# IST-DASLab/gptq-gguf-toolkit

Measured on AMD Instinct MI355X. Metric: Mparams/s GPTQ-quantized, higher is better.
Workload: dtype f32; 1 GPU; llama3-8b-block-q4k: 7 Linears of one block (218.1 M params), 128x2048-token calibration fed per sequence through the package's BlockSchedule, block_size 128, rel_damp 0.01, nstep 20; calib_seqs_per_rank=128, parallelism=calib-dp1+matrix-fanout, owners=rank0

## Files before the change

### gptq-gguf-toolkit_amd/_cabi.py

```python
import ctypes
import os
import subprocess

_HERE = os.path.dirname(os.path.abspath(__file__))
CSRC = os.path.join(_HERE, "csrc")
SO_PATH = os.environ.get("GQ_SO_PATH") or os.path.join(CSRC, "libgptqgguf_hip.so")

ABI_VERSION = 6
F32, F16, BF16 = 0, 1, 2
WS_H_ACCUMULATE, WS_H_PREPARE, WS_GPTQ_QUANTIZE, WS_CHOL_GEMM = 1, 2, 3, 4

EXPORTS = (
    "gq_abi_version", "gq_last_error", "gq_option_count", "gq_option_name", "gq_option_get", "gq_option_default", "gq_option_set", "gq_type_info", "gq_workspace_bytes", "gq_h_accumulate", "gq_h_accumulate_grouped", "gq_h_accumulate_segments", "gq_h_stage", "gq_h_stage_many", "gq_h_prepare", "gq_w_prepare", "gq_h_pack_upper", "gq_h_unpack_upper",
    "gq_scale_search", "gq_group_search", "gq_gptq_quantize", "gq_gptq_quantize_stacked", "gq_gptq_quantize_slice", "gq_gptq_quantize_perm", "gq_gptq_uses_helper_stream", "gq_far_helper_enable", "gq_obq_h_prepare", "gq_obq_quantize", "gq_rtn_quantize", "gq_dequantize", "gq_pack", "gq_unpack", "gq_dequantize_blocks", "gq_trailing_update", "gq_chol_gemm", "gq_stage_to_host", "gq_fwd_rmsnorm", "gq_fwd_rmsnorm_ordered", "gq_fwd_rope", "gq_fwd_silu_mul",
    "gq_eval_nll", "gq_eval_kl", "gq_eval_kl_sparse",
    "gq_prof_enable", "gq_prof_ntags", "gq_prof_name", "gq_prof_collect", "gq_prof_collect2",
)
EXPORTS_ERREST = ("gq_quad_form_workspace_bytes", "gq_quad_form")
EXPORTS_SEARCH = ("gq_level_switch",)
SWITCH_MAX_JOBS = 64
EXPORTS_LEVELS = ("gq_gptq_quantize_bands",)
BANDS_MAX = 64
EXPORTS_LEVELPACK = ("gq_pack_bands",)
PACK_BANDS_ALIGN = 16
EXPORTS_Q8 = ("gq_quantize_q8_0",)
Q8_0 = 8
IQ4_NL, IQ4_XS = 20, 23
EXPORTS_IQ4_ENCODE = ("gq_quantize_iq4",)
EXPORTS_IQ4_GPTQ = ("gq_gptq_quantize_iq4", "gq_pack_iq4")
EXPORTS_QGEMM = ("gq_linear_packed",)
EXPORTS_QGEMV = ("gq_gemv_packed",)
GEMV_MAX_T = 16
EXPORTS_SAMPLE = ("gq_sample_logits",)
SAMPLE_MAX_K = 1024
EXPORTS_MOE = ("gq_gemv_packed_experts",)
MOE_MAX_PAIRS = 64
EXPORTS_MOE_GEMM = ("gq_moe_route", "gq_linear_packed_experts")
MOE_ROUTE_MAX_EXPERTS = 256
MOE_ROUTE_MAX_PAIRS = 131072
EXPORTS_MOE_CALIB = ("gq_fwd_moe_combine",)
MOE_COMBINE_MAX_K = 8
EXPORTS_MOE_SEARCH = ("gq_level_switch_experts",)
SWITCH_EXPERTS_MAX_JOBS = 71


class GQError(RuntimeError):
    pass


class TypeInfo(ctypes.Structure):
    _fields_ = [(n, ctypes.c_int) for n in
                ("bits", "qmin", "qmax", "scale_maxq", "group", "is_signed", "k_search", "type_size")]


class Search(ctypes.Structure):
    _fields_ = [("rmin", ctypes.c_double), ("rdelta", ctypes.c_double), ("nstep", ctypes.c_int),
                ("quant_scale", ctypes.c_int), ("grid", ctypes.c_int), ("maxshrink", ctypes.c_double)]


class SwitchJob(ctypes.Structure):
    _fields_ = [("src", ctypes.c_void_p), ("dst", ctypes.c_void_p), ("row_src", ctypes.c_void_p),
                ("R", ctypes.c_int64), ("C", ctypes.c_int64), ("kind", ctypes.c_int32), ("out_dtype", ctypes.c_int32)]


class SwitchExpertsJob(ctypes.Structure):
    _fields_ = [("src", ctypes.c_void_p), ("dst", ctypes.c_void_p), ("E", ctypes.c_int64), ("R", ctypes.c_int64),
                ("C", ctypes.c_int64), ("dst_expert_stride", ctypes.c_int64), ("kind", ctypes.c_int32),
                ("out_dtype", ctypes.c_int32)]


class Band(ctypes.Structure):
    _fields_ = [("row_end", ctypes.c_int64), ("q_type", ctypes.c_int32)]


def build(force: bool = False) -> str:
    args = ["make", "-C", CSRC, "-s", "-j8"]
    if force:
        args.append("-B")
    subprocess.check_call(args)
    return SO_PATH


_lib = None


def lib():
    global _lib
    if _lib is not None:
        return _lib
    if not os.path.exists(SO_PATH):
        raise GQError(
            f"{SO_PATH} not found: the HIP extension is not built. Run `python -c 'import __graft_entry__ as g; "
            f"g.build()'` (or `make -C {CSRC}`). There is no CPU fallback.")
    import torch
    L = ctypes.CDLL(SO_PATH)
    vp, i64, ci, cf, sz = ctypes.c_void_p, ctypes.c_int64, ctypes.c_int, ctypes.c_float, ctypes.c_size_t
    sp = ctypes.POINTER(Search)
    L.gq_abi_version.restype = ci
    if L.gq_abi_version() != ABI_VERSION:
        raise GQError(f"{SO_PATH} has ABI version {L.gq_abi_version()}, this package binds version {ABI_VERSION}: rebuild "
                      f"(`make -C {CSRC}`)")
    L.gq_last_error.restype = ctypes.c_char_p
    L.gq_option_name.restype = ctypes.c_char_p
    L.gq_option_name.argtypes = [ci]
    L.gq_option_get.argtypes = [ctypes.c_char_p, ctypes.POINTER(i64)]
    L.gq_option_default.argtypes = [ctypes.c_char_p, ctypes.POINTER(i64)]
    L.gq_option_set.argtypes = [ctypes.c_char_p, i64, ctypes.POINTER(i64)]
    L.gq_type_info.argtypes = [ci, ctypes.POINTER(TypeInfo)]
    L.gq_workspace_bytes.argtypes = [ci, i64, i64, i64, ci]
    L.gq_workspace_bytes.restype = sz
    L.gq_h_accumulate.argtypes = [vp, vp, ci, i64, i64, cf, cf, vp, sz, vp]
    L.gq_h_accumulate_grouped.argtypes = [ci, vp, vp, vp, vp, vp, vp, ci, vp, sz, vp]
    L.gq_h_accumulate_segments.argtypes = [ci, vp, vp, vp, vp, vp, vp, vp, ci, vp, sz, vp]
    L.gq_h_stage.argtypes = [vp, vp, i64, vp]
    L.gq_h_stage_many.argtypes = [vp, vp, vp, ci, vp, sz, vp]
    L.gq_h_prepare.argtypes = [vp, vp, i64, i64, cf, vp, vp, vp, vp, sz, vp]
    L.gq_w_prepare.argtypes = [vp, vp, i64, i64, vp, vp]
    L.gq_h_pack_upper.argtypes = [vp, i64, vp, vp]
    L.gq_h_unpack_upper.argtypes = [vp, i64, vp, vp]
    L.gq_scale_search.argtypes = [vp, i64, i64, ci, sp, vp, i64, vp, i64, vp, i64, vp, i64, vp]
    L.gq_group_search.argtypes = [vp, ci, i64, i64, ci, sp, vp, vp, vp, vp, vp, vp, vp]
    L.gq_gptq_quantize.argtypes = [vp, vp, i64, i64, ci, ci, ci, sp, vp, vp, vp, vp, vp, vp, sz, vp]
    L.gq_gptq_quantize_stacked.argtypes = [vp, vp, i64, i64, ci, ci, ci, sp, vp, vp, vp, vp, vp, vp, ci, vp, sz, vp]
    L.gq_gptq_quantize_slice.argtypes = [vp, vp, i64, i64, ci, ci, ci, sp, vp, vp, vp, vp, vp, vp, vp, sz, vp]
    L.gq_gptq_quantize_perm.argtypes = [vp, vp, i64, i64, ci, ci, vp, vp, vp, vp, vp, vp, vp, sz, vp]
    L.gq_gptq_uses_helper_stream.argtypes = [i64, i64, ci]
    L.gq_far_helper_enable.argtypes = [ci]
    L.gq_obq_h_prepare.argtypes = L.gq_h_prepare.argtypes
    L.gq_obq_quantize.argtypes = [vp, vp, i64, i64, ci, ci, ci, ci, vp, vp, vp, vp, sz, vp]
    L.gq_rtn_quantize.argtypes = [vp, ci, i64, i64, ci, sp, vp, vp, vp, vp, vp, vp]
    L.gq_dequantize.argtypes = [ci, vp, vp, vp, vp, vp, i64, i64, vp, ci, vp]
    L.gq_pack.argtypes = [ci, vp, vp, vp, vp, vp, i64, i64, vp, vp]
    L.gq_unpack.argtypes = [ci, vp, i64, i64, vp, vp, vp, vp, vp, vp]
    L.gq_dequantize_blocks.argtypes = [ci, vp, i64, i64, vp, vp, ci, vp]
    L.gq_trailing_update.argtypes = [vp, i64, vp, i64, vp, i64, i64, i64, i64, vp]
    L.gq_chol_gemm.argtypes = [vp, i64, vp, i64, vp, i64, i64, i64, i64, ci, ci, ci, ci, ci, vp, sz, vp]
    L.gq_stage_to_host.argtypes = [vp, vp, i64, vp]
    L.gq_fwd_rmsnorm.argtypes = [vp, vp, vp, i64, i64, cf, ci, vp]
    L.gq_fwd_rmsnorm_ordered.argtypes = [vp, vp, vp, i64, i64, cf, ci, vp, vp]
    L.gq_fwd_rope.argtypes = [vp, vp, vp, vp, i64, ci, ci, ci, vp]
    L.gq_fwd_silu_mul.argtypes = [vp, vp, vp, i64, ci, vp]
    L.gq_eval_nll.argtypes = [vp, ci, i64, i64, i64, vp, i64, vp, vp, vp]
    L.gq_eval_kl.argtypes = [vp, ci, vp, ci, i64, i64, i64, i64, vp, vp]
    L.gq_eval_kl_sparse.argtypes = [vp, ci, i64, i64, i64, vp, ci, vp, i64, vp, vp]
    L.gq_quad_form_workspace_bytes.argtypes = [i64, i64]
    L.gq_quad_form_workspace_bytes.restype = sz
    L.gq_quad_form.argtypes = [vp, ci, i64, vp, ci, i64, vp, i64, i64, vp, vp, sz, vp]
    L.gq_level_switch.argtypes = [ctypes.POINTER(SwitchJob), ci, vp]
    L.gq_gptq_quantize_bands.argtypes = [vp, vp, i64, i64, ctypes.POINTER(Band), ci, ci, sp, vp, vp, vp, vp, vp, vp, sz, vp]
    L.gq_pack_bands.argtypes = [vp, vp, vp, vp, vp, i64, i64, ctypes.POINTER(Band), ci, ctypes.POINTER(vp), ctypes.POINTER(vp), vp]
    L.gq_quantize_q8_0.argtypes = [vp, ci, i64, i64, vp, vp, vp]
    L.gq_quantize_iq4.argtypes = [vp, ci, i64, i64, ci, vp, vp, vp, vp]
    L.gq_gptq_quantize_iq4.argtypes = [vp, vp, i64, i64, ci, ci, vp, vp, vp, vp, vp, vp, vp, sz, vp]
    L.gq_pack_iq4.argtypes = [ci, i64, i64, vp, vp, vp, vp, vp, vp]
    L.gq_linear_packed.argtypes = [ci, vp, vp, i64, i64, vp, i64, ci, vp, vp]
    L.gq_gemv_packed.argtypes = [ci, vp, vp, i64, i64, vp, i64, ci, vp, vp]
    L.gq_sample_logits.argtypes = [vp, ci, i64, i64, i64, ci, cf, cf, vp, vp, vp]
    L.gq_gemv_packed_experts.argtypes = [ci, vp, i64, i64, i64, vp, i64, vp, i64, i64, ci, vp, vp]
    L.gq_moe_route.argtypes = [vp, i64, i64, vp, vp, vp]
    L.gq_linear_packed_experts.argtypes = [ci, vp, i64, i64, i64, vp, i64, i64, vp, vp, i64, ci, vp, vp]
    L.gq_fwd_moe_combine.argtypes = [vp, vp, vp, vp, vp, ci, i64, i64, i64, i64, ci, vp, vp]
    L.gq_level_switch_experts.argtypes = [ctypes.POINTER(SwitchExpertsJob), ci, vp]
    L.gq_prof_enable.argtypes = [ctypes.c_uint]
    L.gq_prof_enable.restype = None
    L.gq_prof_name.argtypes = [ci]
    L.gq_prof_name.restype = ctypes.c_char_p
    L.gq_prof_collect.argtypes = [ctypes.POINTER(ctypes.c_double), ctypes.POINTER(ctypes.c_long)]
    L.gq_prof_collect2.argtypes = [ctypes.POINTER(ctypes.c_double), ctypes.POINTER(ctypes.c_long),
                                   ctypes.POINTER(ctypes.c_double)]
    for name in (EXPORTS + EXPORTS_ERREST + EXPORTS_SEARCH + EXPORTS_LEVELS + EXPORTS_LEVELPACK + EXPORTS_Q8 + EXPORTS_IQ4_ENCODE + EXPORTS_IQ4_GPTQ + EXPORTS_QGEMM +
                 EXPORTS_QGEMV + EXPORTS_SAMPLE + EXPORTS_MOE + EXPORTS_MOE_GEMM + EXPORTS_MOE_CALIB + EXPORTS_MOE_SEARCH):
        getattr(L, name)
    _lib = L
    return L


def check(rc: int, what: str):
    if rc != 0:
        msg = lib().gq_last_error().decode(errors="replace")
        raise GQError(f"{what} failed (status {rc}): {msg}")


def type_info(q_type: int) -> dict:
    t = TypeInfo()
    check(lib().gq_type_info(int(q_type), ctypes.byref(t)), "gq_type_info")
    return {n: getattr(t, n) for n, _ in TypeInfo._fields_}


def prof_enable(tags=None):
    L = lib()
    names = [L.gq_prof_name(i).decode() for i in range(L.gq_prof_ntags())]
    mask = 0
    for i, n in enumerate(names):
        if tags is None or n in tags:
            mask |= 1 << i
    L.gq_prof_enable(mask)
    return names


def prof_collect(busy: bool = False) -> dict:
    L = lib()
    n = L.gq_prof_ntags()
    ms = (ctypes.c_double * n)()
    cnt = (ctypes.c_long * n)()
    bz = (ctypes.c_double * n)()
    check(L.gq_prof_collect2(ms, cnt, bz), "gq_prof_collect2")
    if busy:
        return {L.gq_prof_name(i).decode(): (ms[i], cnt[i], bz[i]) for i in range(n) if cnt[i]}
    return {L.gq_prof_name(i).decode(): (ms[i], cnt[i]) for i in range(n) if cnt[i]}


def option_names():
    L = lib()
    return [L.gq_option_name(i).decode() for i in range(L.gq_option_count())]


def option_get(name: str) -> int:
    v = ctypes.c_int64()
    check(lib().gq_option_get(name.encode(), ctypes.byref(v)), "gq_option_get")
    return int(v.value)


def option_default(name: str) -> int:
    v = ctypes.c_int64()
    check(lib().gq_option_default(name.encode(), ctypes.byref(v)), "gq_option_default")
    return int(v.value)


def option_set(name: str, value: int) -> int:
    prev = ctypes.c_int64()
    check(lib().gq_option_set(name.encode(), int(value), ctypes.byref(prev)), "gq_option_set")
    return int(prev.value)


class options:

    def __init__(self, **kv):
        self.kv, self.prev = kv, {}

    def __enter__(self):
        for k, v in self.kv.items():
            self.prev[k] = option_set(k, option_default(k) if v is None else v)
        return self

    def __exit__(self, *exc):
        for k, v in self.prev.items():
            option_set(k, v)
        return False
```

### gptq-gguf-toolkit_amd/block_schedule.py

```python
import contextlib
import os
import sys
import time
from typing import Any, Callable, Dict, List, Optional, Tuple

import torch
import torch.nn as nn

from . import dist_utils
from . import ops as _ops
from .gptq import GPTQ
from .model_utils import ForwardInterrupt
from .quant_utils import GGML_QUANT_SIZES
from .quant_utils import GGMLQuantizationType, dequantize_linear_weight

_stream_pool: Dict[Any, List["torch.cuda.Stream"]] = {}


def _chain_streams(device, n: int):
    if n <= 0 or torch.device(device).type != "cuda":
        return []
    pool = _stream_pool.setdefault(torch.device(device), [])
    while len(pool) < n:
        pool.append(torch.cuda.Stream(device))
    return pool[:n]


class _Lane:

    def __init__(self, stream, main):
        self.stream, self.main = stream, main

    def wait(self, event):
        if self.stream is not None and event is not None:
            self.stream.wait_event(event)

    def run(self):
        return torch.cuda.stream(self.stream) if self.stream is not None else contextlib.nullcontext()

    def join(self, tensors=()):
        if self.stream is None:
            return
        ev = torch.cuda.Event()
        ev.record(self.stream)
        self.main.wait_event(ev)
        for t in tensors:
            if t is not None and t.is_cuda:
                t.record_stream(self.main)


def _zero_columns(w: torch.Tensor) -> torch.Tensor:
    return (w.detach().reshape(w.shape[0], -1) == 0).all(dim=0)


def _owner_cost(h: GPTQ) -> float:
    return float(h.d_row) * h.d_col * (h.d_col + 128)


def _chain_order_key(hs: List[GPTQ]):
    return (not any(h._row_split_active() for h in hs), -sum(float(h.d_row) * h.d_col ** 2 for h in hs))


def _lane_load(hs: List[GPTQ]) -> float:
    return sum(float(h.d_row) * h.d_col ** 2 + float(h.d_col) ** 3 / 3 for h in hs)


def _plan_lanes(cost: List[float], lanes: int) -> Tuple[List[int], List[int]]:
    n = len(cost)
    lane_of, load = [0] * n, [0.0] * max(lanes, 1)
    for k in range(n):
        lane_of[k] = min(range(lanes), key=lambda i: (load[i], i)) if lanes else 0
        load[lane_of[k]] += cost[k]
    enq = list(range(n))
    if lanes >= 4 and n > 2 * lanes:
        per = [[k for k in range(n) if lane_of[k] == i] for i in range(lanes)]
        for i in range(lanes // 2, lanes):
            per[i].reverse()
        enq = [per[i][j] for j in range(max(len(x) for x in per)) for i in range(lanes) if j < len(per[i])]
    return lane_of, enq


@contextlib.contextmanager
def _far_helper_lease(on: bool):
    was = _ops.far_helper_enable(on)
    try:
        yield
    finally:
        _ops.far_helper_enable(was)


class _Call:

    def __init__(self, qtypes, writeback, extra, own: Dict[str, bool], world: int, rank: int):
        self.qtypes, self.writeback, self.extra, self.own, self.world, self.rank = qtypes, writeback, extra, own, world, rank
        self.results: Dict[str, tuple] = {}
        self.deq: Dict[str, torch.Tensor] = {}


class BlockSchedule:
    unverified: List[torch.Tensor] = []

    def __init__(self, layers: Dict[str, nn.Module], make_handle: Callable[[nn.Module, str], GPTQ],
                 n_streams: Optional[int] = None, verbose: bool = False):
        self.handles: Dict[str, GPTQ] = {n: make_handle(l, n) for n, l in layers.items()}
        self._zero_cols = {n: _zero_columns(l.weight) for n, l in layers.items()}
        self._sharing = None
        for h in self.handles.values():
            h._scheduled = True
        self._seen: Dict[Any, Any] = {}
        self._fired: List[str] = []
        self._last_fired: Optional[str] = None
        self._other_after = False
        self._n_samples = 0
        self.n_streams = int(os.environ.get("GQ_CHAIN_STREAMS", 4)) if n_streams is None else n_streams
        self.stack = os.environ.get("GQ_STACK", "1") != "0"
        self.verbose = verbose
        self.stats = {"syrk_launches": 0, "allreduce_bytes": 0, "reused_U": 0, "own_U": 0, "refactorised": 0}
        self.owners: Dict[str, Any] = {}

    def hook(self, name: str):
        def _hook(_, inp, out):
            self.feed(name, inp[0])
        return _hook

    def pre_hook(self, name: str, interrupt: bool = True):
        def _hook(_, inp):
            self.feed(name, inp[0])
            self._fired.append(name)
            self._other_after = False
            if interrupt and name == self._last_fired and self._all_fired_once():
                self.stats["forward1_interrupts"] = self.stats.get("forward1_interrupts", 0) + 1
                raise ForwardInterrupt
        return _hook

    def _all_fired_once(self) -> bool:
        return len(self._fired) == len(self.handles) and len(set(self._fired)) == len(self._fired)

    def other_pre_hook(self):
        def _hook(_, inp):
            if self._n_samples == 0:
                self._other_after = True
        return _hook

    def feed(self, name: str, x: torch.Tensor) -> None:
        h = self.handles[name]
        key = (x.data_ptr(), tuple(x.shape), tuple(x.stride()), x.dtype, x._version)
        hit = self._seen.get(key)
        if hit is not None and hit[0].d_col == h.d_col and hit[0] is not h:
            leader = hit[0]
            assert h.shared_H_with in (None, leader), "input sharing pattern changed between samples"
            assert h.H is None, "handle switched from own Hessian to a shared one"
            h.shared_H_with = leader
            leader._has_followers = True
        else:
            assert h.shared_H_with is None, "input sharing pattern changed between samples"
            self._seen[key] = (h, x)
        h.update(x)

    def sample_done(self) -> None:
        self._seen.clear()
        if self._n_samples == 0 and self._all_fired_once() and not self._other_after:
            self._last_fired = self._fired[-1]
        self._n_samples += 1
        self._fired = []
        if self._sharing is None:
            self._publish_sharing()
        due = [h for h in self.leaders() if h._fill >= h.flush_tokens]
        if due:
            self.flush(only=due)

    def _publish_sharing(self) -> None:
        name_of = {id(h): n for n, h in self.handles.items()}
        followers = [n for n, h in self.handles.items() if h.shared_H_with is not None]
        host = ev = None
        if followers:
            neq = torch.stack([(self._zero_cols[n] != self._zero_cols[name_of[id(self.handles[n].shared_H_with)]]).any()
                               for n in followers])
            if neq.is_cuda:
                host = torch.empty(len(followers), dtype=torch.bool, pin_memory=True)
                host.copy_(neq, non_blocking=True)
                ev = torch.cuda.Event()
                ev.record(torch.cuda.current_stream(neq.device))
            else:
                host = neq
        self._sharing = (followers, host, ev)

    def _needs_own_factorisation(self) -> Dict[str, bool]:
        if self._sharing is None or not self._sharing[0]:
            return {}
        followers, host, ev = self._sharing
        if ev is not None:
            ev.synchronize()
        return dict(zip(followers, host.tolist()))

    _staged_checks: List[Any] = []

    @classmethod
    def stage_verify(cls) -> None:
        flags, cls.unverified = cls.unverified, []
        if not flags:
            return
        anyf = torch.stack([f.reshape(()) for f in flags]).any().reshape(1)
        if anyf.is_cuda:
            host = torch.empty(1, dtype=torch.bool, pin_memory=True)
            host.copy_(anyf, non_blocking=True)
            ev = torch.cuda.Event()
            ev.record(torch.cuda.current_stream(anyf.device))
            cls._staged_checks.append((host, ev))
        else:
            cls._staged_checks.append((anyf, None))

    @classmethod
    def verify(cls, wait: bool = True) -> None:
        cls.stage_verify()
        keep = []
        for host, ev in cls._staged_checks:
            if ev is not None and not wait and not ev.query():
                keep.append((host, ev))
                continue
            if ev is not None:
                ev.synchronize()
            if bool(host.item()):
                cls._staged_checks = []
                raise RuntimeError("a Linear reused its leader's Cholesky factor although their dead / zero-column sets "
                                   "differ (gq_w_prepare flag)")
        cls._staged_checks = keep

    @classmethod
    def discard_checks(cls) -> None:
        cls.unverified = []
        cls._staged_checks = []

    def leaders(self) -> List[GPTQ]:
        return [h for h in self.handles.values() if h.shared_H_with is None]

    def _fold(self, grids: List[List[GPTQ]]) -> None:
        for grp in grids:
            args = [h._flush_args() for h in grp]
            _ops.h_accumulate_grouped([a[0] for a in args], [a[1] for a in args], [a[2] for a in args],
                                      [a[3] for a in args])
            self.stats["syrk_launches"] += 1
            for h in grp:
                h._flush_done()

    def flush(self, only: Optional[List[GPTQ]] = None) -> None:
        todo = [h for h in self.leaders() if h._fill > 0 and (only is None or any(h is o for o in only))]
        if not todo:
            return
        todo.sort(key=lambda h: (-h.d_col, id(h)))
        grids: List[List[GPTQ]] = []
        if 1 < len(todo) <= 8 and len({(h._pending_dtype(), h._pending_device()) for h in todo}) == 1:
            rest, grids_tail = todo, []
        elif len(todo) > 1 and todo[0].d_col > todo[1].d_col:
            rest, grids_tail = todo[1:], [[todo[0]]]
        else:
            rest, grids_tail = todo, []
        by_kind: Dict[Any, List[GPTQ]] = {}
        for h in rest:
            by_kind.setdefault((h._pending_dtype(), h._pending_device()), []).append(h)
        for grp in by_kind.values():
            grids += [grp[i:i + 8] for i in range(0, len(grp), 8)]
        grids += grids_tail
        self._fold(grids)

    def _agree_on_sharing(self) -> None:
        names = list(self.handles)
        idx = {id(self.handles[n]): i for i, n in enumerate(names)}
        dev = next(iter(self.handles.values())).W_device
        v = torch.full((len(names),), -1, dtype=torch.int64, device=dev)
        for i, n in enumerate(names):
            h = self.handles[n]
            if h.shared_H_with is not None:
                v[i] = idx[id(h.shared_H_with)]
            elif h.H is not None or h._fill > 0:
                v[i] = i
        mine = v.clone()
        dist_utils.collective_calls["small_all_reduce"] += 1
        dist_utils.collective_bytes["small_all_reduce"] += v.numel() * 8
        torch.distributed.all_reduce(v, op=torch.distributed.ReduceOp.MAX)
        got, mine = v.tolist(), mine.tolist()
        for i, n in enumerate(names):
            h = self.handles[n]
            assert mine[i] in (-1, got[i]), f"{n}: ranks observed different input sharing ({mine[i]} vs {got[i]})"
            if mine[i] == -1 and got[i] not in (-1, i):
                leader = self.handles[names[got[i]]]
                h.shared_H_with = leader
                leader._has_followers = True

    @torch.no_grad()
    def quantize(self, qtypes: Dict[str, GGMLQuantizationType], writeback: bool = True,
                 extra: Optional[Callable[[str, GPTQ, tuple], Any]] = None) -> Dict[str, Tuple[torch.Tensor, ...]]:
        handles = self.handles
        world, rank = dist_utils.get_world_size(), dist_utils.get_rank()
        for n, h in handles.items():
            if qtypes[n] == GGMLQuantizationType.Q3_K:
                h.act_order = False
        if world > 1:
            self._assign_ranks(world)
        dev = next(iter(handles.values())).W_device
        on_gpu = torch.device(dev).type == "cuda"
        main = torch.cuda.current_stream(dev) if on_gpu else None
        ready, start = self._reduce_hessians(world, main)

        order = self._chains(rank)
        call = _Call(qtypes, writeback, extra, self._needs_own_factorisation(), world, rank)
        on_main = 1
        lent = 1 if on_gpu and 2 < self.n_streams and len(order) <= self.n_streams and any(
            _ops.uses_helper_stream(h.d_row, h.d_col, h.block_size) for h in handles.values()
            if h.owner_rank == rank and not h._row_split_active()) else 0
        streams = [None] * on_main + _chain_streams(dev, min(self.n_streams - lent, len(order)) - on_main)
        trace = "sched" in os.environ.get("GQ_TRACE", "")
        t_host = time.perf_counter()
        lane_of, enq = _plan_lanes([_lane_load([handles[n] for n in names]) for names in order], len(streams))
        with _far_helper_lease(bool(lent)) if on_gpu else contextlib.nullcontext():
            lanes = []
            for k in enq:
                if trace:
                    print(f"  [sched] +{1e3 * (time.perf_counter() - t_host):7.2f} ms: enqueue chain {k} {order[k]} on lane {lane_of[k]}",
                          file=sys.stderr)
                lane = _Lane(streams[lane_of[k]], main)
                lead = handles[order[k][0]].shared_H_with or handles[order[k][0]]
                lane.wait(ready.get(id(lead), start))
                lanes.append((lane, self._run_chain(call, order[k], lane)))
            for lane, born in lanes:
                lane.join(born)
        if trace:
            print(f"  [sched] +{1e3 * (time.perf_counter() - t_host):7.2f} ms: all chains enqueued", file=sys.stderr)
        self._settle_late_followers(call)
        self.stats["own_U"] = len(call.results) - self.stats["reused_U"]
        return self._exchange_and_write_back(call)

    @torch.no_grad()
    def quantize_levels(self, levels, propagate: Optional[GGMLQuantizationType],
                        extra: Optional[Callable[[str, GPTQ, dict], Any]] = None,
                        pack: Optional[Callable[[tuple, list, list], Any]] = None,
                        before: Optional[Callable[[str, GPTQ], Any]] = None) -> Dict[str, Dict[Any, Tuple[torch.Tensor, ...]]]:
        handles = self.handles
        levels = [GGMLQuantizationType(t) for t in levels]
        if not levels or len(set(levels)) != len(levels):
            raise ValueError("quantize_levels needs a non-empty list of distinct levels")
        if propagate is not None:
            propagate = GGMLQuantizationType(propagate)
            if propagate not in levels:
                raise ValueError(f"propagate={propagate.name} is not one of the levels {[t.name for t in levels]}")
        if dist_utils.get_world_size() > 1:
            raise NotImplementedError("quantize_levels runs on one rank (multi-rank level builds are not built)")
        for n, h in handles.items():
            if h.act_order or h.static_groups:
                raise ValueError(f"{n}: act_order / static_groups handles have no level build")
        dev = next(iter(handles.values())).W_device
        on_gpu = torch.device(dev).type == "cuda"
        main = torch.cuda.current_stream(dev) if on_gpu else None
        ready, start = self._reduce_hessians(1, main)
        order = self._chains(0)
        own = self._needs_own_factorisation()
        lent = 1 if on_gpu and 2 < self.n_streams and len(order) <= self.n_streams and any(
            _ops.uses_helper_stream(len(levels) * h.d_row, h.d_col, h.block_size) for h in handles.values()) else 0
        streams = [None] + _chain_streams(dev, min(self.n_streams - lent, len(order)) - 1)
        lane_of, enq = _plan_lanes([_lane_load([handles[n] for n in names]) for names in order], len(streams))
        results: Dict[str, Dict[Any, tuple]] = {}
        deq: Dict[str, torch.Tensor] = {}
        with _far_helper_lease(bool(lent)) if on_gpu else contextlib.nullcontext():
            lanes = []
            for k in enq:
                lane = _Lane(streams[lane_of[k]], main)
                lane.wait(start)
                lanes.append((lane, self._run_level_chain(order[k], levels, propagate, own, extra, results, deq, lane, pack,
                                                          before)))
            for lane, born in lanes:
                lane.join(born)
        self.stats["own_U"] = len(results) - self.stats["reused_U"]
        for n, h in handles.items():
            if propagate is not None:
                h.layer.weight.data = deq[n]
            h.reset()
        return {n: results[n] for n in handles}

    def _run_level_chain(self, names: List[str], levels, propagate, own: Dict[str, bool], extra, results, deq,
                         lane: _Lane, pack=None, before=None) -> List[torch.Tensor]:
        handles = self.handles
        born: List[torch.Tensor] = []
        names = sorted(names, key=lambda n: handles[n].shared_H_with is not None)
        together = [n for n in names if handles[n].shared_H_with is None or (n in own and not own[n])]
        alone = [n for n in names if n not in together]
        walks = [] if pack is not None else None
        name_of = {handles[n]: n for n in names}
        with lane.run():
            for n in names if before is not None else ():
                out = before(n, handles[n])
                born.extend(t for t in (out if isinstance(out, (tuple, list)) else (out,)) if torch.is_tensor(t))
            for grp in ([together] if self.stack else [[n] for n in together]):
                if not grp:
                    continue
                if self.verbose:
                    print(f"[rank 0] Quantizing {grp} with {[t.name for t in levels]}.")
                hs = [handles[n] for n in grp]
                if len(grp) > 1:
                    self.stats["stacked"] = self.stats.get("stacked", 0) + len(grp)
                res = GPTQ.compute_levels(hs, levels, defer_check=True, walks=walks)
                for n, h in zip(grp, hs):
                    if h._pending_mismatch is not None:
                        BlockSchedule.unverified.append(h._pending_mismatch)
                        h._pending_mismatch = None
                        self.stats["reused_U"] += 1
                    results[n] = res[h]
            for n in alone:
                h = handles[n]
                self.stats["refactorised"] += 1
                results[n] = GPTQ.compute_levels([h], levels, own_U=True, walks=walks)[h]
            for n in names:
                h = handles[n]
                for res in results[n].values():
                    born.extend(res)
                born.extend(t for t in (h._last_U, h._last_cf) if torch.is_tensor(t))
                if propagate is not None:
                    deq[n] = dequantize_linear_weight(propagate, *results[n][propagate], out_dtype=h.layer.weight.data.dtype)
                    born.append(deq[n])
                if extra is not None:
                    out = extra(n, h, results[n])
                    born.extend(t for t in (out if isinstance(out, (tuple, list)) else (out,)) if torch.is_tensor(t))
            for stacked, bands, members in walks or ():
                out = pack(stacked, bands, [None if mem is None else (name_of[mem[0]], mem[1]) for mem in members])
                born.extend(t for t in (out if isinstance(out, (tuple, list)) else (out,)) if torch.is_tensor(t))
        return born

    def _assign_ranks(self, world: int) -> None:
        handles = self.handles
        costs = {n: _owner_cost(h) for n, h in handles.items()}
        split = {n for n in dist_utils.row_split_names(costs, world) if not handles[n].act_order}
        for n in split:
            handles[n].row_split = True
        for n, r in dist_utils.assign_owners({n: c for n, c in costs.items() if n not in split}, world).items():
            handles[n].owner_rank = r
        if any(h.allow_no_samples for h in handles.values()):
            self._agree_on_sharing()
        self.owners = {n: (f"rows/{world}" if h._row_split_active() else h.owner_rank) for n, h in handles.items()}
        need: Dict[int, set] = {}
        for n, h in handles.items():
            lead = h.shared_H_with or h
            need.setdefault(id(lead), set()).update(range(world) if h._row_split_active() else (h.owner_rank,))
        for h in self.leaders():
            ranks = need.get(id(h), set())
            h.reduce_to = next(iter(ranks)) if len(ranks) == 1 else None

    def _reduce_hessians(self, world: int, main):
        ready: Dict[int, Any] = {}
        self.flush()
        for h in sorted(self.leaders(), key=lambda h: -h.d_col):
            h.sync_hessian()
            if world > 1:
                self.stats["allreduce_bytes"] += dist_utils.hessian_payload_bytes(h.d_col)
                if main is not None:
                    ready[id(h)] = torch.cuda.Event()
                    ready[id(h)].record(main)
        for h in self.handles.values():
            h.sync_hessian()
        start = None
        if main is not None and world == 1:
            start = torch.cuda.Event()
            start.record(main)
        return ready, start

    def _chains(self, rank: int) -> List[List[str]]:
        chains: Dict[int, List[str]] = {}
        for n, h in self.handles.items():
            if h.owner_rank == rank or h._row_split_active():
                chains.setdefault(id(h.shared_H_with or h), []).append(n)
        return sorted(chains.values(), key=lambda ns: _chain_order_key([self.handles[n] for n in ns]))

    def _run_chain(self, call: _Call, names: List[str], lane: _Lane) -> List[torch.Tensor]:
        handles, qtypes = self.handles, call.qtypes
        born: List[torch.Tensor] = []
        with lane.run():
            for grp in self._stack_groups(sorted(names, key=lambda n: handles[n].shared_H_with is not None), qtypes, call.own):
                if self.verbose:
                    for n in grp:
                        print(f"[rank {call.rank}] Quantizing {n} with {qtypes[n].name}.")
                if len(grp) > 1:
                    hs = [handles[n] for n in grp]
                    self.stats["stacked"] = self.stats.get("stacked", 0) + len(grp)
                    for n, h, res in zip(grp, hs, GPTQ.compute_stacked(hs, qtypes[grp[0]])):
                        self._computed(call, born, n, h, res)
                    continue
                n = grp[0]
                h = handles[n]
                h.make_working_copy()
                self._computed(call, born, n, h, h.compute(qtypes[n], defer_check=True, own_U=call.own.get(n, False)))
        return born

    def _computed(self, call: _Call, born: List[torch.Tensor], n: str, h: GPTQ, res: tuple) -> None:
        if n in call.own and h._pending_mismatch is not None:
            BlockSchedule.unverified.append(h._pending_mismatch)
            h._pending_mismatch = None
            self.stats["reused_U"] += 1
        elif call.own.get(n, False):
            self.stats["refactorised"] += 1
        call.results[n] = res
        born.extend(res)
        born.extend(t for t in (h._last_U, h._last_cf, getattr(h, "_researches", None), h.W) if torch.is_tensor(t))
        if call.world == 1 and call.writeback:
            call.deq[n] = dequantize_linear_weight(call.qtypes[n], *res, out_dtype=h.layer.weight.data.dtype)
            born.append(call.deq[n])
        if call.extra is not None:
            out = call.extra(n, h, res)
            born.extend(t for t in (out if isinstance(out, (tuple, list)) else (out,)) if torch.is_tensor(t))

    def _settle_late_followers(self, call: _Call) -> None:
        handles = self.handles
        pending = [(n, handles[n]._pending_mismatch) for n in call.results if handles[n]._pending_mismatch is not None]
        if pending:
            flags = torch.cat([f.reshape(1) for _, f in pending]).tolist()
            for (n, _), bad in zip(pending, flags):
                h = handles[n]
                h._pending_mismatch = None
                if bad:
                    self.stats["refactorised"] += 1
                    h.make_working_copy()
                    call.results[n] = h.compute(call.qtypes[n], own_U=True)
                    call.deq.pop(n, None)
                else:
                    self.stats["reused_U"] += 1

    def _exchange_and_write_back(self, call: _Call) -> Dict[str, Tuple[torch.Tensor, ...]]:
        handles, qtypes = self.handles, call.qtypes
        if call.world > 1:
            out = self._exchange_block(handles, qtypes, call.results, call.world, call.rank)
        else:
            out = {n: call.results[n] for n in handles}
        for n, h in handles.items():
            if call.writeback:
                w = call.deq.get(n)
                if w is None:
                    w = dequantize_linear_weight(qtypes[n], *out[n], out_dtype=h.layer.weight.data.dtype)
                h.layer.weight.data = w
            h.reset()
        return out

    def _stack_groups(self, names: List[str], qtypes, own: Dict[str, bool]) -> List[List[str]]:
        if not self.stack:
            return [[n] for n in names]
        groups: List[List[str]] = []
        open_: Dict[Any, List[str]] = {}
        for n in names:
            h = self.handles[n]
            key = h.stack_key(qtypes[n])
            known = (h.shared_H_with is None and h._has_followers) or (n in own and not own[n])
            if key is None or not known:
                groups.append([n])
                continue
            g = open_.get(key)
            if g is None or len(g) >= 8:
                g = open_[key] = []
                groups.append(g)
            g.append(n)
        return groups

    @staticmethod
    def _piece_layout(q_type, rows: int, cols: int):
        bits, clamp, scale_maxq, group_size, supergroup_size, sz_dtype, q_dtype = GGML_QUANT_SIZES[q_type]
        shapes = ((q_dtype, (rows, cols)), (torch.float16, (rows, cols // supergroup_size)),
                  (sz_dtype, (rows, cols // group_size)), (torch.float16, (rows, cols // supergroup_size)),
                  (sz_dtype, (rows, cols // group_size)))
        lay, off = [], 0
        for dt, shp in shapes:
            n = shp[0] * shp[1] * torch.empty(0, dtype=dt).element_size()
            lay.append((dt, shp, off, n))
            off += (n + 255) & ~255
        return lay, off

    def _exchange_block(self, handles, qtypes, results, world: int, rank: int):
        per_rank: List[List[Tuple[str, int, int]]] = [[] for _ in range(world)]
        for n, h in handles.items():
            if h._row_split_active():
                for r in range(world):
                    r0, r1, _ = dist_utils.row_slice(h.d_row, r, world)
                    if r1 > r0:
                        per_rank[r].append((n, r0, r1))
            else:
                per_rank[h.owner_rank].append((n, 0, h.d_row))
        layouts = [[(n, r0, r1) + self._piece_layout(qtypes[n], r1 - r0, handles[n].d_col) for n, r0, r1 in lst]
                   for lst in per_rank]
        sizes = [sum(x[4] for x in lst) for lst in layouts]
        split = [n for n, h in handles.items() if h._row_split_active()]
        tail = (4 * len(split) + 255) & ~255 if split else 0
        body = max(max(sizes), 256)
        nbytes = body + tail
        dev = next(iter(handles.values())).W_device
        buf = torch.empty(nbytes, dtype=torch.uint8, device=dev)
        off = 0
        for n, r0, r1, lay, tot in layouts[rank]:
            for t, (dt, shp, o, k) in zip(results[n], lay):
                buf[off + o:off + o + k].view(dt).view(shp).copy_(t)
            off += tot
        if split:
            buf[body:body + 4 * len(split)].view(torch.int32).copy_(torch.cat([handles[n]._researches for n in split]))
        gathered = dist_utils.all_gather_bytes(buf, nbytes)
        self.stats["allgather_bytes"] = self.stats.get("allgather_bytes", 0) + nbytes
        redo = []
        if split:
            counts = gathered[:, body:body + 4 * len(split)].view(torch.int32).reshape(world, len(split)).sum(dim=0).tolist()
            redo = [n for n, c in zip(split, counts) if c != 0]
        parts: Dict[str, List[List[torch.Tensor]]] = {n: [] for n in handles}
        for r in range(world):
            off = 0
            for n, r0, r1, lay, tot in layouts[r]:
                parts[n].append([gathered[r, off + o:off + o + k].view(dt).view(shp) for dt, shp, o, k in lay])
                off += tot
        out: Dict[str, tuple] = {}
        for n in handles:
            ps = parts[n]
            if n in redo:
                self.stats["row_split_redone"] = self.stats.get("row_split_redone", 0) + 1
                handles[n].row_split_redone = True
                out[n] = handles[n].recompute_whole(qtypes[n])
                continue
            out[n] = tuple(ps[0]) if len(ps) == 1 else tuple(torch.cat([p[i] for p in ps], dim=0) for i in range(5))
        return out
```

### gptq-gguf-toolkit_amd/csrc/gq_cholesky.hip

```cpp
#include <atomic>
#include <stdlib.h>

#include "gq_common.hpp"
#include "gq_gemm32.hpp"
#include "gq_gemm3b.hpp"
#include "gq_gemm3p.hpp"

#include <map>
#include <memory>
#include <mutex>

namespace gq {

constexpr int NB = 128;

__global__ __launch_bounds__(256) void col_flags_kernel(const float* __restrict__ H, const float* __restrict__ W,
                                                        int64_t R, int64_t C, uint8_t* __restrict__ dead,
                                                        uint8_t* __restrict__ zc) {
    const int64_t j = (int64_t)blockIdx.x * 64 + (threadIdx.x & 63);
    const int ty = threadIdx.x >> 6;
    __shared__ int nz[4][64];
    int any = 0;
    if (j < C)
        for (int64_t r = ty; r < R; r += 4) any |= (W[r * C + j] != 0.0f);
    nz[ty][threadIdx.x & 63] = any;
    __syncthreads();
    if (ty == 0 && j < C) {
        int a = nz[0][threadIdx.x] | nz[1][threadIdx.x] | nz[2][threadIdx.x] | nz[3][threadIdx.x];
        uint8_t dd = H[j * C + j] == 0.0f;
        dead[j] = dd;
        zc[j] = dd || !a;
    }
}

__global__ __launch_bounds__(256) void zero_dead_cols_kernel(float* __restrict__ W, int64_t R, int64_t C,
                                                             const uint8_t* __restrict__ dead) {
    const int64_t j = (int64_t)blockIdx.x * 64 + (threadIdx.x & 63);
    const bool dd = j < C && dead[j];
    if (!__syncthreads_or(dd)) return;
    if (dd)
        for (int64_t r = threadIdx.x >> 6; r < R; r += 4) W[r * C + j] = 0.0f;
}

__global__ __launch_bounds__(256) void w_prepare_kernel(float* __restrict__ W, int64_t R, int64_t C,
                                                        const uint8_t* __restrict__ dead,
                                                        const uint8_t* __restrict__ zc, int* __restrict__ mismatch) {
    const int64_t j = (int64_t)blockIdx.x * 64 + (threadIdx.x & 63);
    const int ty = threadIdx.x >> 6;
    __shared__ int nz[4][64];
    int any = 0;
    if (j < C) {
        const bool dd = dead[j];
        for (int64_t r = ty; r < R; r += 4) {
            if (dd) W[r * C + j] = 0.0f;
            else any |= (W[r * C + j] != 0.0f);
        }
    }
    nz[ty][threadIdx.x & 63] = any;
    __syncthreads();
    if (ty == 0 && j < C) {
        int a = nz[0][threadIdx.x] | nz[1][threadIdx.x] | nz[2][threadIdx.x] | nz[3][threadIdx.x];
        uint8_t mine = dead[j] || !a;
        if (mine != zc[j]) atomicOr(mismatch, 1);
    }
}

__global__ __launch_bounds__(256) void col_flags4_kernel(const float* __restrict__ H, const float* __restrict__ W,
                                                         int64_t R, int64_t C, uint8_t* __restrict__ dead,
                                                         uint8_t* __restrict__ zc) {
    const int tx = threadIdx.x & 15, ty = threadIdx.x >> 4;
    const int64_t j = (int64_t)blockIdx.x * 64 + 4 * tx;
    __shared__ int nz[16][64];
    int a0 = 0, a1 = 0, a2 = 0, a3 = 0;
    if (j < C) {
#pragma unroll 8
        for (int64_t r = ty; r < R; r += 16) {
            const float4 v = *reinterpret_cast<const float4*>(W + r * C + j);
            a0 |= (v.x != 0.0f); a1 |= (v.y != 0.0f); a2 |= (v.z != 0.0f); a3 |= (v.w != 0.0f);
        }
    }
    nz[ty][4 * tx] = a0; nz[ty][4 * tx + 1] = a1; nz[ty][4 * tx + 2] = a2; nz[ty][4 * tx + 3] = a3;
    __syncthreads();
    const int64_t jc = (int64_t)blockIdx.x * 64 + threadIdx.x;
    if (threadIdx.x < 64 && jc < C) {
        int a = 0;
#pragma unroll
        for (int t = 0; t < 16; ++t) a |= nz[t][threadIdx.x];
        const uint8_t dd = H[jc * C + jc] == 0.0f;
        dead[jc] = dd;
        zc[jc] = dd || !a;
    }
}
__global__ __launch_bounds__(256) void w_prepare4_kernel(float* __restrict__ W, int64_t R, int64_t C,
                                                         const uint8_t* __restrict__ dead,
                                                         const uint8_t* __restrict__ zc, int* __restrict__ mismatch) {
    const int tx = threadIdx.x & 15, ty = threadIdx.x >> 4;
    const int64_t j = (int64_t)blockIdx.x * 64 + 4 * tx;
    __shared__ int nz[16][64];
    int a0 = 0, a1 = 0, a2 = 0, a3 = 0;
    if (j < C) {
        const bool d0 = dead[j], d1 = dead[j + 1], d2 = dead[j + 2], d3 = dead[j + 3];
        const bool anyd = d0 | d1 | d2 | d3;
#pragma unroll 8
        for (int64_t r = ty; r < R; r += 16) {
            float4 v = *reinterpret_cast<const float4*>(W + r * C + j);
            if (anyd) {
                if (d0) v.x = 0.0f;
                if (d1) v.y = 0.0f;
                if (d2) v.z = 0.0f;
                if (d3) v.w = 0.0f;
                *reinterpret_cast<float4*>(W + r * C + j) = v;
            }
            a0 |= (v.x != 0.0f); a1 |= (v.y != 0.0f); a2 |= (v.z != 0.0f); a3 |= (v.w != 0.0f);
        }
    }
    nz[ty][4 * tx] = a0; nz[ty][4 * tx + 1] = a1; nz[ty][4 * tx + 2] = a2; nz[ty][4 * tx + 3] = a3;
    __syncthreads();
    const int64_t jc = (int64_t)blockIdx.x * 64 + threadIdx.x;
    if (threadIdx.x < 64 && jc < C) {
        int a = 0;
#pragma unroll
        for (int t = 0; t < 16; ++t) a |= nz[t][threadIdx.x];
        const uint8_t mine = dead[jc] || !a;
        if (mine != zc[jc]) atomicOr(mismatch, 1);
    }
}

__global__ __launch_bounds__(256) void mask_h_kernel(float* __restrict__ H, int64_t C, const uint8_t* __restrict__ zc) {
    __shared__ int flagged[64];
    const int64_t i0 = (int64_t)blockIdx.x * 64;
    if (threadIdx.x < 64) flagged[threadIdx.x] = (i0 + threadIdx.x < C) && zc[i0 + threadIdx.x];
    __syncthreads();
    for (int t = 0; t < 64; ++t) {
        if (!flagged[t]) continue;
        const int64_t i = i0 + t;
        for (int64_t j = threadIdx.x; j < C; j += blockDim.x) {
            const float v = (i == j) ? 1.0f : 0.0f;
            H[i * C + j] = v;
            H[j * C + i] = v;
        }
    }
}

__global__ __launch_bounds__(256) void dead_diag_kernel(float* __restrict__ H, int64_t C, const uint8_t* __restrict__ dead) {
    const int64_t j = (int64_t)blockIdx.x * blockDim.x + threadIdx.x;
    if (j < C && dead[j]) H[j * C + j] = 1.0f;
}

__global__ __launch_bounds__(1024) void damp_kernel(float* __restrict__ H, int64_t C, float rel_damp) {
    __shared__ double part[1024];
    double acc = 0.0;
    for (int64_t i = threadIdx.x; i < C; i += 1024) acc += (double)H[i * C + i];
    part[threadIdx.x] = acc;
    __syncthreads();
    for (int o = 512; o > 0; o >>= 1) {
        if ((int)threadIdx.x < o) part[threadIdx.x] += part[threadIdx.x + o];
        __syncthreads();
    }
    const float damp = rel_damp * (float)(part[0] / (double)C);
    for (int64_t i = threadIdx.x; i < C; i += 1024) H[i * C + i] += damp;
}

__global__ __launch_bounds__(256) void equil_kernel(const float* __restrict__ H, int64_t n, float* __restrict__ s) {
    const int64_t j = (int64_t)blockIdx.x * blockDim.x + threadIdx.x;
    if (j >= n) return;
    const float h = H[j * n + j];
    float v = 1.0f;
    if (h > 0.0f && h < 3.0e38f) {
        int e;
        (void)frexpf(h, &e);
        const int half = (e >= 0 ? e : e - 1) / 2;
        v = ldexpf(1.0f, -half);
    }
    s[j] = v;
}
__global__ __launch_bounds__(256) void reverse_copy_kernel(float* __restrict__ A, const float* __restrict__ H,
                                                           int64_t n, const float* __restrict__ s) {
    const int64_t i = blockIdx.x, r = n - 1 - i;
    const int64_t jend = (i / 128 + 1) * 128;
    const float si = s ? s[r] : 1.0f;
    for (int64_t j = 4 * (int64_t)threadIdx.x; j < jend; j += 4 * 256) {
        const float4 h = *reinterpret_cast<const float4*>(H + r * n + (n - 4 - j));
        float4 a = make_float4(h.w, h.z, h.y, h.x);
        if (s) {
            const float4 sc = *reinterpret_cast<const float4*>(s + (n - 4 - j));
            a.x *= si * sc.w; a.y *= si * sc.z; a.z *= si * sc.y; a.w *= si * sc.x;
        }
        *reinterpret_cast<float4*>(A + i * n + j) = a;
    }
}

__global__ __launch_bounds__(256) void finish_u_kernel(float* __restrict__ U, const float* __restrict__ X, int64_t n,
                                                       const int* __restrict__ flag, const float* __restrict__ s) {
    const int64_t i = blockIdx.x, r = n - 1 - i;
    const bool bad = *flag != 0;
    for (int64_t j = 4 * (int64_t)threadIdx.x; j < n; j += 4 * 256) {
        float4 u = make_float4(0.f, 0.f, 0.f, 0.f);
        if (bad) {
            u.x = (j == i) ? 1.0f : 0.0f; u.y = (j + 1 == i) ? 1.0f : 0.0f;
            u.z = (j + 2 == i) ? 1.0f : 0.0f; u.w = (j + 3 == i) ? 1.0f : 0.0f;
        } else if (j + 3 >= i) {
            const float4 x = *reinterpret_cast<const float4*>(X + r * n + (n - 4 - j));
            float4 sc = make_float4(1.f, 1.f, 1.f, 1.f);
            if (s) sc = *reinterpret_cast<const float4*>(s + j);
            u.x = (j >= i) ? x.w * sc.x : 0.0f;
            u.y = (j + 1 >= i) ? x.z * sc.y : 0.0f;
            u.z = (j + 2 >= i) ? x.y * sc.z : 0.0f;
            u.w = x.x * sc.w;
        }
        *reinterpret_cast<float4*>(U + i * n + j) = u;
    }
}

constexpr int LDP = NB + 4;

__global__ __launch_bounds__(256) void diag_potrf_inv_kernel(float* __restrict__ A, int64_t lda,
                                                             float* __restrict__ Xout, int64_t ldx,
                                                             int* __restrict__ flag) {
    extern __shared__ __attribute__((aligned(16))) float smem[];
    float* S = smem;
    float* XT = smem + NB * LDP;
    float* dg = XT + NB * LDP;
    const int tid = threadIdx.x;
    for (int idx = tid; idx < NB * NB; idx += 256) {
        int i = idx / NB, j = idx % NB;
        float v = (j <= i) ? A[i * lda + j] : 0.0f;
        S[i * LDP + j] = v;
        XT[i * LDP + j] = 0.0f;
        if (i == j) dg[i] = v;
    }
    __syncthreads();
    const bool fac = tid < NB;
    const int i = tid & (NB - 1);
    for (int j = 0; j <= NB; ++j) {
        if (fac) {
            if (j < NB && i >= j) {
                const float4* ri = reinterpret_cast<const float4*>(S + i * LDP);
                const float4* rj = reinterpret_cast<const float4*>(S + j * LDP);
                float a0 = 0.f, a1 = 0.f, a2 = 0.f, a3 = 0.f, q0 = 0.f, q1 = 0.f, q2 = 0.f, q3 = 0.f;
                const int n4 = j >> 2;
                int p4 = 0;
                for (; p4 + 4 <= n4; p4 += 4) {
                    float4 a[4], b[4];
#pragma unroll
                    for (int u = 0; u < 4; ++u) { a[u] = ri[p4 + u]; b[u] = rj[p4 + u]; }
#pragma unroll
                    for (int u = 0; u < 4; ++u) {
                        a0 = fmaf(a[u].x, b[u].x, a0); a1 = fmaf(a[u].y, b[u].y, a1);
                        a2 = fmaf(a[u].z, b[u].z, a2); a3 = fmaf(a[u].w, b[u].w, a3);
                        q0 = fmaf(b[u].x, b[u].x, q0); q1 = fmaf(b[u].y, b[u].y, q1);
                        q2 = fmaf(b[u].z, b[u].z, q2); q3 = fmaf(b[u].w, b[u].w, q3);
                    }
                }
                for (; p4 < n4; ++p4) {
                    const float4 a = ri[p4], b = rj[p4];
                    a0 = fmaf(a.x, b.x, a0); a1 = fmaf(a.y, b.y, a1); a2 = fmaf(a.z, b.z, a2); a3 = fmaf(a.w, b.w, a3);
                    q0 = fmaf(b.x, b.x, q0); q1 = fmaf(b.y, b.y, q1); q2 = fmaf(b.z, b.z, q2); q3 = fmaf(b.w, b.w, q3);
                }
                float acc = (a0 + a1) + (a2 + a3), accp = (q0 + q1) + (q2 + q3);
                for (int p = p4 * 4; p < j; ++p) {
                    const float a = S[i * LDP + p], b = S[j * LDP + p];
                    acc = fmaf(a, b, acc);
                    accp = fmaf(b, b, accp);
                }
                float piv = dg[j] - accp;
                const bool bad = !(piv > 0.0f);
                if (bad) piv = 1.0f;
                const float ljj = sqrtf(piv);
                if (i == j) {
                    S[j * LDP + j] = ljj;
                    if (bad) *flag = 1;
                } else {
                    S[i * LDP + j] = (S[i * LDP + j] - acc) / ljj;
                }
            }
        } else if (j >= 1) {
            const int r = j - 1, c = i;
            if (c == r) {
                XT[c * LDP + r] = 1.0f / S[r * LDP + r];
            } else if (c < r) {
                const float4* lr = reinterpret_cast<const float4*>(S + r * LDP);
                const float4* xc = reinterpret_cast<const float4*>(XT + c * LDP);
                float a0 = 0.f, a1 = 0.f, a2 = 0.f, a3 = 0.f;
                int p4 = c >> 2;
                const int e4 = r >> 2;
                for (; p4 + 3 <= e4; p4 += 4) {
                    float4 a[4], b[4];
#pragma unroll
                    for (int u = 0; u < 4; ++u) { a[u] = lr[p4 + u]; b[u] = xc[p4 + u]; }
#pragma unroll
                    for (int u = 0; u < 4; ++u) {
                        a0 = fmaf(a[u].x, b[u].x, a0); a1 = fmaf(a[u].y, b[u].y, a1);
                        a2 = fmaf(a[u].z, b[u].z, a2); a3 = fmaf(a[u].w, b[u].w, a3);
                    }
                }
                for (; p4 <= e4; ++p4) {
                    const float4 a = lr[p4], b = xc[p4];
                    a0 = fmaf(a.x, b.x, a0); a1 = fmaf(a.y, b.y, a1); a2 = fmaf(a.z, b.z, a2); a3 = fmaf(a.w, b.w, a3);
                }
                const float acc = (a0 + a1) + (a2 + a3);
                XT[c * LDP + r] = -acc / S[r * LDP + r];
            }
        }
        __syncthreads();
    }
    for (int idx = tid; idx < NB * NB; idx += 256) {
        int r = idx / NB, c = idx % NB;
        if (c <= r) A[r * lda + c] = S[r * LDP + c];
        Xout[r * ldx + c] = XT[c * LDP + r];
    }
}

constexpr int LDQ = NB + 1;
constexpr int TQ = 33;

__device__ __forceinline__ float rdlane(float v, int l) {
    return __builtin_bit_cast(float, __builtin_amdgcn_readlane(__builtin_bit_cast(int, v), l));
}

template <int C>
__device__ __forceinline__ void d_upd4(float (&a)[32], float aj) {
    int t0, t1, t2, t3;
    asm volatile(
        "v_readlane_b32 %4, %8, %9\n\tv_readlane_b32 %5, %8, %10\n\tv_readlane_b32 %6, %8, %11\n\t"
        "v_readlane_b32 %7, %8, %12\n\t"
        "v_fma_f32 %0, -%8, %4, %0\n\tv_fma_f32 %1, -%8, %5, %1\n\tv_fma_f32 %2, -%8, %6, %2\n\tv_fma_f32 %3, -%8, %7, %3"
        : "+v"(a[C]), "+v"(a[C + 1]), "+v"(a[C + 2]), "+v"(a[C + 3]), "=&s"(t0), "=&s"(t1), "=&s"(t2), "=&s"(t3)
        : "v"(aj), "n"(C), "n"(C + 1), "n"(C + 2), "n"(C + 3));
}
template <int C>
__device__ __forceinline__ void d_upd8(float (&a)[32], float aj) {
    int t0, t1, t2, t3, t4, t5, t6, t7;
    asm volatile(
        "v_readlane_b32 %8, %16, %17\n\tv_readlane_b32 %9, %16, %18\n\tv_readlane_b32 %10, %16, %19\n\t"
        "v_readlane_b32 %11, %16, %20\n\tv_readlane_b32 %12, %16, %21\n\tv_readlane_b32 %13, %16, %22\n\t"
        "v_readlane_b32 %14, %16, %23\n\tv_readlane_b32 %15, %16, %24\n\t"
        "v_fma_f32 %0, -%16, %8, %0\n\tv_fma_f32 %1, -%16, %9, %1\n\tv_fma_f32 %2, -%16, %10, %2\n\t"
        "v_fma_f32 %3, -%16, %11, %3\n\tv_fma_f32 %4, -%16, %12, %4\n\tv_fma_f32 %5, -%16, %13, %5\n\t"
        "v_fma_f32 %6, -%16, %14, %6\n\tv_fma_f32 %7, -%16, %15, %7"
        : "+v"(a[C]), "+v"(a[C + 1]), "+v"(a[C + 2]), "+v"(a[C + 3]), "+v"(a[C + 4]), "+v"(a[C + 5]), "+v"(a[C + 6]),
          "+v"(a[C + 7]), "=&s"(t0), "=&s"(t1), "=&s"(t2), "=&s"(t3), "=&s"(t4), "=&s"(t5), "=&s"(t6), "=&s"(t7)
        : "v"(aj), "n"(C), "n"(C + 1), "n"(C + 2), "n"(C + 3), "n"(C + 4), "n"(C + 5), "n"(C + 6), "n"(C + 7));
}
template <int C>
__device__ __forceinline__ void d_upd1(float (&a)[32], float aj) {
    int t0;
    asm volatile("v_readlane_b32 %1, %2, %3\n\ts_nop 1\n\tv_fma_f32 %0, -%2, %1, %0" : "+v"(a[C]), "=&s"(t0) : "v"(aj), "n"(C));
}
template <int C>
__device__ __forceinline__ void d_updates(float (&a)[32], float aj) {
    if constexpr (C + 7 <= 31) {
        d_upd8<C>(a, aj);
        d_updates<C + 8>(a, aj);
    } else if constexpr (C + 3 <= 31) {
        d_upd4<C>(a, aj);
        d_updates<C + 4>(a, aj);
    } else if constexpr (C <= 31) {
        d_upd1<C>(a, aj);
        d_updates<C + 1>(a, aj);
    }
}
template <int J>
__device__ __forceinline__ void d_factor(float (&a)[32], int i, float& myinv, bool& bad) {
    asm volatile("s_nop 1" : "+v"(a[J]));
    float pj = rdlane(a[J], J);
    if (!(pj > 0.0f)) {
        bad = true;
        pj = 1.0f;
    }
    float inv = __builtin_amdgcn_rsqf(pj);
    inv = fmaf(inv, fmaf(-0.5f * pj * inv, inv, 0.5f), inv);
    const float ljj = pj * inv;
    int ii = i;
    asm volatile("" : "+v"(ii));
    const bool mine = ii == J;
    if (mine) myinv = inv;
    a[J] = mine ? ljj : a[J] * inv;
    asm volatile("s_nop 1" : "+v"(a[J]));
    d_updates<J + 1>(a, a[J]);
    if constexpr (J < 31) d_factor<J + 1>(a, i, myinv, bad);
}
template <int R, int P>
__device__ __forceinline__ void d_dot4(const float (&a)[32], const float (&x)[32], float (&acc)[4]) {
    int t0, t1, t2, t3;
    asm volatile(
        "v_readlane_b32 %4, %8, %16\n\tv_readlane_b32 %5, %9, %16\n\tv_readlane_b32 %6, %10, %16\n\t"
        "v_readlane_b32 %7, %11, %16\n\t"
        "v_fma_f32 %0, %4, %12, %0\n\tv_fma_f32 %1, %5, %13, %1\n\tv_fma_f32 %2, %6, %14, %2\n\tv_fma_f32 %3, %7, %15, %3"
        : "+v"(acc[0]), "+v"(acc[1]), "+v"(acc[2]), "+v"(acc[3]), "=&s"(t0), "=&s"(t1), "=&s"(t2), "=&s"(t3)
        : "v"(a[P]), "v"(a[P + 1]), "v"(a[P + 2]), "v"(a[P + 3]), "v"(x[P]), "v"(x[P + 1]), "v"(x[P + 2]), "v"(x[P + 3]),
          "n"(R));
}
template <int R, int P>
__device__ __forceinline__ void d_dot8(const float (&a)[32], const float (&x)[32], float (&acc)[4]) {
    int t0, t1, t2, t3, t4, t5, t6, t7;
    asm volatile(
        "v_readlane_b32 %4, %12, %28\n\tv_readlane_b32 %5, %13, %28\n\tv_readlane_b32 %6, %14, %28\n\t"
        "v_readlane_b32 %7, %15, %28\n\tv_readlane_b32 %8, %16, %28\n\tv_readlane_b32 %9, %17, %28\n\t"
        "v_readlane_b32 %10, %18, %28\n\tv_readlane_b32 %11, %19, %28\n\t"
        "v_fma_f32 %0, %4, %20, %0\n\tv_fma_f32 %1, %5, %21, %1\n\tv_fma_f32 %2, %6, %22, %2\n\t"
        "v_fma_f32 %3, %7, %23, %3\n\tv_fma_f32 %0, %8, %24, %0\n\tv_fma_f32 %1, %9, %25, %1\n\t"
        "v_fma_f32 %2, %10, %26, %2\n\tv_fma_f32 %3, %11, %27, %3"
        : "+v"(acc[0]), "+v"(acc[1]), "+v"(acc[2]), "+v"(acc[3]), "=&s"(t0), "=&s"(t1), "=&s"(t2), "=&s"(t3), "=&s"(t4),
          "=&s"(t5), "=&s"(t6), "=&s"(t7)
        : "v"(a[P]), "v"(a[P + 1]), "v"(a[P + 2]), "v"(a[P + 3]), "v"(a[P + 4]), "v"(a[P + 5]), "v"(a[P + 6]), "v"(a[P + 7]),
          "v"(x[P]), "v"(x[P + 1]), "v"(x[P + 2]), "v"(x[P + 3]), "v"(x[P + 4]), "v"(x[P + 5]), "v"(x[P + 6]), "v"(x[P + 7]),
          "n"(R));
}
template <int R, int P>
__device__ __forceinline__ void d_dot1(const float (&a)[32], const float (&x)[32], float& acc) {
    int t0;
    asm volatile("v_readlane_b32 %1, %2, %4\n\ts_nop 1\n\tv_fma_f32 %0, %1, %3, %0" : "+v"(acc), "=&s"(t0) : "v"(a[P]), "v"(x[P]), "n"(R));
}
template <int R, int P>
__device__ __forceinline__ void d_dot(const float (&a)[32], const float (&x)[32], float (&acc)[4]) {
    if constexpr (P + 7 < R) {
        d_dot8<R, P>(a, x, acc);
        d_dot<R, P + 8>(a, x, acc);
    } else if constexpr (P + 3 < R) {
        d_dot4<R, P>(a, x, acc);
        d_dot<R, P + 4>(a, x, acc);
    } else if constexpr (P < R) {
        d_dot1<R, P>(a, x, acc[P & 3]);
        d_dot<R, P + 1>(a, x, acc);
    }
}
template <int R>
__device__ __forceinline__ void d_inverse(const float (&a)[32], float (&x)[32], int i, float myinv) {
    const float irr = rdlane(myinv, R);
    float acc[4] = {0.0f, 0.0f, 0.0f, 0.0f};
    d_dot<R, 0>(a, x, acc);
    const float dot = (acc[0] + acc[1]) + (acc[2] + acc[3]);
    int ii = i;
    asm volatile("" : "+v"(ii));
    x[R] = (R < ii) ? 0.0f : ((R == ii) ? irr : -dot * irr);
    if constexpr (R < 31) d_inverse<R + 1>(a, x, i, myinv);
}

__device__ __forceinline__ f32x16 mfma_nt_32(const float* Ap, int lda_, const float* Bp, int ldb_, int lane) {
    f32x16 acc;
#pragma unroll
    for (int e = 0; e < 16; ++e) acc[e] = 0.0f;
    const int li = lane & 31, lk = lane >> 5;
    float av[16], bv[16];
#pragma unroll
    for (int p = 0; p < 16; ++p) {
        av[p] = Ap[li * lda_ + 2 * p + lk];
        bv[p] = Bp[li * ldb_ + 2 * p + lk];
    }
#pragma unroll
    for (int p = 0; p < 16; ++p) acc = __builtin_amdgcn_mfma_f32_32x32x2f32(av[p], bv[p], acc, 0, 0, 0);
    return acc;
}


}
#include "gq_diag5.hpp"
namespace gq {

static int64_t p3_min() { return opt(OPT_chol_3p_min); }
static int p3_planes() { return opt(OPT_chol_planes) == 3 ? 3 : 2; }
static inline bool p3_node(int64_t n1, int64_t n2) {
    return p3_min() > 0 && n1 >= p3_min() && n2 >= p3_min() && n1 % 256 == 0 && n2 % 256 == 0;
}
constexpr int P3_MAX_SLOTS = 1024;
struct P3Gemm {
    size_t table_at, rlist_at;
    int n_reduce;
};
struct P3Plans {
    std::vector<uint32_t> words;
    std::vector<P3Gemm> gemms;
};
static void p3_collect(P3Plans& pl, int64_t lo, int64_t hi) {
    if (hi - lo == 1) return;
    const int64_t mid = (lo + hi) / 2;
    const int64_t n1 = (mid - lo) * NB, n2 = (hi - mid) * NB;
    p3_collect(pl, lo, mid);
    const bool big = p3_node(n1, n2);
    const int gran = p3_planes() == 3 ? 2 : 4;
    auto add = [&](const std::vector<p3::GemmShape>& shs) {
        p3::Plan p = p3::make_plan(shs, gran, P3_MAX_SLOTS);
        P3Gemm g;
        while (pl.words.size() % 4) pl.words.push_back(0u);
        g.table_at = pl.words.size();
        pl.words.insert(pl.words.end(), p.table.begin(), p.table.end());
        g.rlist_at = pl.words.size();
        pl.words.insert(pl.words.end(), p.rlist.begin(), p.rlist.end());
        g.n_reduce = (int)(p.rlist.size() / 2);
        if (p.nslots < 0) fprintf(stderr, "gq: image GEMM plan needs more than %d partial slots\n", P3_MAX_SLOTS), abort();
        pl.gemms.push_back(g);
    };
    if (big) {
        const int t1 = (int)(n1 / 256), t2 = (int)(n2 / 256), k1 = (int)(n1 / 32);
        add({{t2, t1, k1, 1, false}});
        add({{t2, t2, k1, 0, true}, {t2, t1, k1, 2, false}});
    }
    p3_collect(pl, mid, hi);
    if (big) add({{(int)(n2 / 256), (int)(n1 / 256), (int)(n2 / 32), 3, false}});
}
static std::shared_ptr<const P3Plans> p3_plans_for(int64_t nblk) {
    static std::mutex mu;
    static std::map<std::pair<int64_t, int64_t>, std::shared_ptr<const P3Plans>> cache;
    std::lock_guard<std::mutex> lk(mu);
    const std::pair<int64_t, int64_t> key{nblk, p3_min() * 4 + p3_planes()};
    auto it = cache.find(key);
    if (it != cache.end()) return it->second;
    auto pl = std::make_shared<P3Plans>();
    p3_collect(*pl, 0, nblk);
    cache[key] = pl;
    return pl;
}
struct P3Run {
    const P3Plans* plans = nullptr;
    const uint32_t* words_dev = nullptr;
    size_t next = 0;
    unsigned char* img[2] = {nullptr, nullptr};
    float* partial = nullptr;
    unsigned* rmax = nullptr;
    float* inv_scale = nullptr;
};
static size_t p3_image_bytes(int64_t C) { return (size_t)(C / 2) * (size_t)(C / 2) * 2 * (size_t)p3_planes(); }
static bool p3_used(int64_t C) {
    const int64_t nblk = C / NB, mid = nblk / 2;
    return nblk >= 2 && p3_node(mid * NB, (nblk - mid) * NB);
}

size_t h_prepare_workspace_bytes(int64_t R, int64_t C) {
    (void)R;
    const size_t n2 = (size_t)C * (size_t)C * sizeof(float);
    size_t extra = 0;
    if (p3_used(C)) {
        auto pl = p3_plans_for(C / NB);
        extra = 2 * (p3_image_bytes(C) + 256) + (size_t)P3_MAX_SLOTS * p3::TILE * p3::TILE * 4 + pl->words.size() * 4 +
                4 * (size_t)C * 4 + 2048;
    }
    return 2 * n2 + 2 * (size_t)C + 4 * (size_t)C + 1024 + extra;
}

template <int NP>
static p3::Problem p3_problem(P3Run& run, const unsigned char* Aimg, int64_t Ka, const unsigned char* Bimg, int64_t Kb,
                              float* Cm, int64_t ldc, int mode, const float* rs, const float* cs) {
    return p3::Problem{Aimg, Bimg, (uint32_t)(Ka / 32 * NP * p3::BLK), (uint32_t)(Kb / 32 * NP * p3::BLK), Cm, ldc, mode,
                       rs, cs, run.partial};
}
template <int NP>
static int p3_gemm(P3Run& run, const p3::Problem& p0, const p3::Problem* p1, hipStream_t st) {
    const P3Gemm& gm = run.plans->gemms[run.next++];
    p3::Group g;
    g.p[0] = p0;
    g.p[1] = p1 ? *p1 : p0;
    g.table = run.words_dev + gm.table_at;
    return p3::launch_gemm<NP>(g, gm.n_reduce, run.words_dev + gm.rlist_at, st);
}

static int chol_inv_rec(float* A, float* X, float* Tmp, int* flag, int64_t n, int64_t lo, int64_t hi, size_t diag_lds,
                        hipStream_t st, P3Run& run);

template <int NP>
static int chol_node_p3(float* A, float* X, float* Tmp, int* flag, int64_t n, int64_t lo, int64_t mid, int64_t hi,
                        size_t diag_lds, hipStream_t st, P3Run& run) {
    const int64_t n1 = (mid - lo) * NB, n2 = (hi - mid) * NB;
    const int64_t o21 = (mid * NB) * n + lo * NB, o11 = (lo * NB) * n + lo * NB, o22 = (mid * NB) * n + mid * NB;
    unsigned* rm0 = run.rmax, *rm1 = run.rmax ? run.rmax + n / 2 : nullptr;
    float* is0 = run.inv_scale, *is1 = run.inv_scale ? run.inv_scale + n / 2 : nullptr;
    const float* s0 = NP == 2 ? is0 : nullptr;
    const float* s1 = NP == 2 ? is1 : nullptr;
    int rc;
    {
        ProfScope ps(PT_CHOL_GEMM, st);
        if ((rc = p3::launch_split<NP>(false, A + o21, n, n2, n1, 0, 0, run.img[0], rm0, is0, st))) return rc;
        if ((rc = p3::launch_split<NP>(false, X + o11, n, n1, n1, 1, 0, run.img[1], rm1, is1, st))) return rc;
        const p3::Problem g1 = p3_problem<NP>(run, run.img[0], n1, run.img[1], n1, Tmp + o21, n, 1, s0, s1);
        if ((rc = p3_gemm<NP>(run, g1, nullptr, st))) return rc;
        if ((rc = p3::launch_split<NP>(false, Tmp + o21, n, n2, n1, 0, 1, run.img[0], rm0, is0, st))) return rc;
        if ((rc = p3::launch_split<NP>(true, X + o11, n, n1, n1, 2, 1, run.img[1], rm1, is1, st))) return rc;
        const p3::Problem g2 = p3_problem<NP>(run, run.img[0], n1, run.img[0], n1, A + o22, n, 0, s0, s0);
        const p3::Problem g3 = p3_problem<NP>(run, run.img[0], n1, run.img[1], n1, A + o21, n, 1, s0, s1);
        if ((rc = p3_gemm<NP>(run, g2, &g3, st))) return rc;
    }
    if ((rc = chol_inv_rec(A, X, Tmp, flag, n, mid, hi, diag_lds, st, run))) return rc;
    ProfScope ps(PT_TRTRI_GEMM, st);
    if ((rc = p3::launch_split<NP>(false, X + o22, n, n2, n2, 1, 0, run.img[0], rm0, is0, st))) return rc;
    if ((rc = p3::launch_split<NP>(true, A + o21, n, n1, n2, 0, 0, run.img[1], rm1, is1, st))) return rc;
    const p3::Problem g4 = p3_problem<NP>(run, run.img[0], n2, run.img[1], n2, X + o21, n, 2, s0, s1);
    return p3_gemm<NP>(run, g4, nullptr, st);
}

static int chol_inv_rec(float* A, float* X, float* Tmp, int* flag, int64_t n, int64_t lo, int64_t hi, size_t diag_lds,
                        hipStream_t st, P3Run& run) {
    if (hi - lo == 1) {
        ProfScope ps(PT_DIAG_POTRF, st);
        const int64_t o = (lo * NB) * n + lo * NB;
        if (diag_lds == DIAG5_LDS)
            hipLaunchKernelGGL(diag_blk5_kernel, dim3(1), dim3(320), diag_lds, st, A + o, n, X + o, n, flag);
        else
            hipLaunchKernelGGL(diag_potrf_inv_kernel, dim3(1), dim3(256), diag_lds, st, A + o, n, X + o, n, flag);
        GQ_LAUNCH_CHECK();
        return GQ_OK;
    }
    const int64_t mid = (lo + hi) / 2;
    int rc;
    if ((rc = chol_inv_rec(A, X, Tmp, flag, n, lo, mid, diag_lds, st, run))) return rc;
    const int64_t n1 = (mid - lo) * NB, n2 = (hi - mid) * NB;
    if (run.plans && p3_node(n1, n2))
        return p3_planes() == 3 ? chol_node_p3<3>(A, X, Tmp, flag, n, lo, mid, hi, diag_lds, st, run)
                                : chol_node_p3<2>(A, X, Tmp, flag, n, lo, mid, hi, diag_lds, st, run);
    const int64_t o21 = (mid * NB) * n + lo * NB, o11 = (lo * NB) * n + lo * NB, o22 = (mid * NB) * n + mid * NB;
    const int64_t min3b = opt(OPT_chol_fp32) ? (int64_t)1 << 40 : opt(OPT_chol_3b_min);
    const bool big = n1 >= min3b && n2 >= min3b;
#define GQ_CHOL_GEMM(TB, MODE, LOW, KRV, ...) \
    (big ? launch_gemm3b<TB, MODE, LOW, KRV>(__VA_ARGS__) : launch_gemm32<TB, MODE, LOW, KRV>(__VA_ARGS__))
    const bool pair = !big && !opt(OPT_chol_no_pair) && n % 4 == 0 && gemm32_uses_64_full(n2, n2, n1, true) &&
                      gemm32_uses_64_full(n2, n1, n1, false);
    {
        ProfScope ps(PT_CHOL_GEMM, st);
        if ((rc = GQ_CHOL_GEMM(true, 1, false, 1, Tmp + o21, n, A + o21, n, X + o11, n, n2, n1, n1, st))) return rc;
        if (pair) {
            if ((rc = launch_gemm32_pair(A + o22, Tmp + o21, n2, n1, A + o21, Tmp + o21, X + o11, n2, n1, n1, n, st))) return rc;
        } else if ((rc = GQ_CHOL_GEMM(true, 0, true, 0, A + o22, n, Tmp + o21, n, Tmp + o21, n, n2, n2, n1, st))) return rc;
    }
    if ((rc = chol_inv_rec(A, X, Tmp, flag, n, mid, hi, diag_lds, st, run))) return rc;
    ProfScope ps(PT_TRTRI_GEMM, st);
    if (!pair && (rc = GQ_CHOL_GEMM(false, 1, false, 2, A + o21, n, Tmp + o21, n, X + o11, n, n2, n1, n1, st))) return rc;
    return GQ_CHOL_GEMM(false, 2, false, 3, X + o21, n, X + o22, n, A + o21, n, n2, n1, n2, st);
#undef GQ_CHOL_GEMM
}

int w_prepare(const uint8_t* flags, float* W, int64_t R, int64_t C, int* mismatch, hipStream_t st) {
    if (!flags || !W || !mismatch) GQ_FAIL(GQ_E_NULL, "gq_w_prepare: null pointer");
    if (R <= 0 || C <= 0) GQ_FAIL(GQ_E_BAD_SHAPE, "gq_w_prepare: R=%ld C=%ld", (long)R, (long)C);
    GQ_HIP(hipMemsetAsync(mismatch, 0, sizeof(int), st));
    ProfScope ps(PT_PREP_ELEM, st);
    if (C % 4 == 0 && (uintptr_t)W % 16 == 0)
        hipLaunchKernelGGL(w_prepare4_kernel, dim3((unsigned)((C + 63) / 64)), dim3(256), 0, st, W, R, C, flags, flags + C,
                           mismatch);
    else
        hipLaunchKernelGGL(w_prepare_kernel, dim3((unsigned)((C + 63) / 64)), dim3(256), 0, st, W, R, C, flags, flags + C,
                           mismatch);
    GQ_LAUNCH_CHECK();
    return GQ_OK;
}

int h_prepare(float* H, float* W, int64_t R, int64_t C, float rel_damp, float* U, int* not_invertible,
              uint8_t* col_flags_out, void* ws, size_t ws_bytes, hipStream_t st, bool obq_order) {
    if (!H || !W || !U || !not_invertible) GQ_FAIL(GQ_E_NULL, "gq_h_prepare: null pointer");
    if (R <= 0 || C <= 0 || C % NB) GQ_FAIL(GQ_E_BAD_SHAPE, "gq_h_prepare: R=%ld C=%ld (C %% 128 != 0)", (long)R, (long)C);
    const size_t need = h_prepare_workspace_bytes(R, C);
    if (!ws || ws_bytes < need) GQ_FAIL(GQ_E_WORKSPACE, "gq_h_prepare: workspace %zu < %zu bytes", ws_bytes, need);
    const int64_t n = C, nblk = C / NB;
    float* A = reinterpret_cast<float*>(((uintptr_t)ws + 255) & ~(uintptr_t)255);
    float* X = A + (size_t)n * n;
    uint8_t* dead = reinterpret_cast<uint8_t*>(X + (size_t)n * n);
    uint8_t* zc = dead + n;
    int rc;

    P3Run run;
    std::shared_ptr<const P3Plans> plans;
    if (p3_used(C)) {
        plans = p3_plans_for(nblk);
        unsigned char* p = reinterpret_cast<unsigned char*>(zc + n);
        p = reinterpret_cast<unsigned char*>(((uintptr_t)p + 255) & ~(uintptr_t)255) + (((size_t)n * 4 + 255) & ~(size_t)255);
        run.img[0] = p; p += (p3_image_bytes(C) + 255) & ~(size_t)255;
        run.img[1] = p; p += (p3_image_bytes(C) + 255) & ~(size_t)255;
        run.partial = reinterpret_cast<float*>(p); p += (size_t)P3_MAX_SLOTS * p3::TILE * p3::TILE * 4;
        if (p3_planes() == 2) {
            run.rmax = reinterpret_cast<unsigned*>(p); p += (size_t)n * 4;
            run.inv_scale = reinterpret_cast<float*>(p); p += (size_t)n * 4;
        } else {
            p += 2 * (size_t)n * 4;
        }
        p = reinterpret_cast<unsigned char*>(((uintptr_t)p + 255) & ~(uintptr_t)255);
        if (p + plans->words.size() * 4 > reinterpret_cast<unsigned char*>(ws) + ws_bytes)
            GQ_FAIL(GQ_E_WORKSPACE, "gq_h_prepare: workspace too small for the image GEMMs");
        GQ_HIP(hipMemcpyAsync(p, plans->words.data(), plans->words.size() * 4, hipMemcpyHostToDevice, st));
        run.words_dev = reinterpret_cast<const uint32_t*>(p);
        run.plans = plans.get();
    }
    GQ_HIP(hipMemsetAsync(not_invertible, 0, sizeof(int), st));
    float* eq_s = nullptr;
    {
    ProfScope ps(PT_PREP_ELEM, st);
    if ((uintptr_t)W % 16 == 0)
        hipLaunchKernelGGL(col_flags4_kernel, dim3((unsigned)((C + 63) / 64)), dim3(256), 0, st, H, W, R, C, dead, zc);
    else
        hipLaunchKernelGGL(col_flags_kernel, dim3((unsigned)((C + 63) / 64)), dim3(256), 0, st, H, W, R, C, dead, zc);
    GQ_LAUNCH_CHECK();
    hipLaunchKernelGGL(zero_dead_cols_kernel, dim3((unsigned)((C + 63) / 64)), dim3(256), 0, st, W, R, C, dead);
    GQ_LAUNCH_CHECK();
    if (col_flags_out) GQ_HIP(hipMemcpyAsync(col_flags_out, dead, 2 * (size_t)C, hipMemcpyDeviceToDevice, st));
    if (obq_order) {
        hipLaunchKernelGGL(dead_diag_kernel, dim3((unsigned)((C + 255) / 256)), dim3(256), 0, st, H, C, dead);
        hipLaunchKernelGGL(damp_kernel, dim3(1), dim3(1024), 0, st, H, C, rel_damp);
        hipLaunchKernelGGL(mask_h_kernel, dim3((unsigned)((C + 63) / 64)), dim3(256), 0, st, H, C, zc);
    } else {
        hipLaunchKernelGGL(mask_h_kernel, dim3((unsigned)((C + 63) / 64)), dim3(256), 0, st, H, C, zc);
        hipLaunchKernelGGL(damp_kernel, dim3(1), dim3(1024), 0, st, H, C, rel_damp);
    }
    GQ_LAUNCH_CHECK();
    const bool equil = !opt(OPT_chol_no_equil);
    if (equil) {
        eq_s = reinterpret_cast<float*>(((uintptr_t)(zc + n) + 255) & ~(uintptr_t)255);
        hipLaunchKernelGGL(equil_kernel, dim3((unsigned)((n + 255) / 256)), dim3(256), 0, st, H, n, eq_s);
    }
    if (opt(OPT_chol_poison)) GQ_HIP(hipMemsetAsync(A, 0xff, 2 * (size_t)n * n * sizeof(float), st));
    hipLaunchKernelGGL(reverse_copy_kernel, dim3((unsigned)n), dim3(256), 0, st, A, H, n, eq_s);
    GQ_LAUNCH_CHECK();
    }
    static std::atomic<bool> attr_set{false};
    const bool use_ref = opt(OPT_diag_ref) != 0;
    const size_t diag_lds = use_ref ? (2 * NB * LDP + NB) * sizeof(float) : DIAG5_LDS;
    if (!attr_set) {
        GQ_HIP(hipFuncSetAttribute((const void*)diag_potrf_inv_kernel, hipFuncAttributeMaxDynamicSharedMemorySize,
                                   (int)((2 * NB * LDP + NB) * sizeof(float))));
        GQ_HIP(hipFuncSetAttribute((const void*)diag_blk5_kernel, hipFuncAttributeMaxDynamicSharedMemorySize,
                                   (int)DIAG5_LDS));
        attr_set = true;
    }
    if ((rc = chol_inv_rec(A, X, U, not_invertible, n, 0, nblk, diag_lds, st, run))) return rc;
    ProfScope ps(PT_PREP_ELEM, st);
    hipLaunchKernelGGL(finish_u_kernel, dim3((unsigned)n), dim3(256), 0, st, U, X, n, not_invertible, eq_s);
    GQ_LAUNCH_CHECK();
    return GQ_OK;
}

size_t chol_gemm_workspace_bytes(int64_t M, int64_t N, int64_t K) {
    const size_t img = (size_t)3 * 2 * (size_t)K;
    return img * (size_t)M + img * (size_t)N + (size_t)P3_MAX_SLOTS * p3::TILE * p3::TILE * 4 + 2 * (size_t)(M + N) * 4 +
           ((size_t)(M / 256 + 1) * (size_t)(N / 256 + 1) * 6 * 4 + 64) * 4 + 4096;
}
template <int NP>
static int chol_gemm_np(float* Cm, int64_t ldc, const float* A, int64_t lda, const float* B, int64_t ldb, int64_t M, int64_t N,
                        int64_t K, int trans_b, int mode, int kr, int lower, unsigned char* p, unsigned char* end,
                        hipStream_t st) {
    auto take = [&](size_t bytes) {
        unsigned char* q = p;
        p += (bytes + 255) & ~(size_t)255;
        return q;
    };
    unsigned char* ia = take((size_t)NP * 2 * M * K);
    unsigned char* ib = take((size_t)NP * 2 * N * K);
    float* partial = reinterpret_cast<float*>(take((size_t)P3_MAX_SLOTS * p3::TILE * p3::TILE * 4));
    unsigned* rma = reinterpret_cast<unsigned*>(take((size_t)M * 4));
    unsigned* rmb = reinterpret_cast<unsigned*>(take((size_t)N * 4));
    float* isa = reinterpret_cast<float*>(take((size_t)M * 4));
    float* isb = reinterpret_cast<float*>(take((size_t)N * 4));
    const p3::GemmShape sh{(int)(M / 256), (int)(N / 256), (int)(K / 32), kr, lower != 0};
    const p3::Plan pl = p3::make_plan({sh}, NP == 3 ? 2 : 4, P3_MAX_SLOTS);
    if (pl.nslots < 0) GQ_FAIL(GQ_E_UNSUPPORTED, "gq_chol_gemm: the schedule needs more than %d partial slots", P3_MAX_SLOTS);
    std::vector<uint32_t> words(pl.table);
    const size_t rl_at = words.size();
    words.insert(words.end(), pl.rlist.begin(), pl.rlist.end());
    uint32_t* wd = reinterpret_cast<uint32_t*>(take(words.size() * 4));
    if (p > end) GQ_FAIL(GQ_E_WORKSPACE, "gq_chol_gemm: workspace too small");
    GQ_HIP(hipMemcpyAsync(wd, words.data(), words.size() * 4, hipMemcpyHostToDevice, st));
    const int rev = kr == 2;
    int rc;
    if ((rc = p3::launch_split<NP>(false, A, lda, M, K, kr == 3 ? 1 : 0, rev, ia, rma, isa, st))) return rc;
    if (!(lower && A == B && trans_b)) {
        if ((rc = p3::launch_split<NP>(!trans_b, B, ldb, N, K, kr == 1 ? 1 : (kr == 2 ? 2 : 0), rev, ib, rmb, isb, st))) return rc;
    } else {
        ib = ia;
        isb = isa;
    }
    p3::Group g;
    g.p[0] = p3::Problem{ia, ib, (uint32_t)(K / 32 * NP * p3::BLK), (uint32_t)(K / 32 * NP * p3::BLK), Cm, ldc, mode,
                         NP == 2 ? isa : nullptr, NP == 2 ? isb : nullptr, partial};
    g.p[1] = g.p[0];
    g.table = wd;
    return p3::launch_gemm<NP>(g, (int)(pl.rlist.size() / 2), wd + rl_at, st);
}
int chol_gemm(float* Cm, int64_t ldc, const float* A, int64_t lda, const float* B, int64_t ldb, int64_t M, int64_t N, int64_t K,
              int trans_b, int mode, int kr, int lower, int planes, void* ws, size_t ws_bytes, hipStream_t st) {
    if (!Cm || !A || !B || !ws) GQ_FAIL(GQ_E_NULL, "gq_chol_gemm: null pointer");
    if (M <= 0 || N <= 0 || K <= 0 || M % 256 || N % 256 || K % 128 || lda % 4 || ldb % 4 || ldc % 4)
        GQ_FAIL(GQ_E_BAD_SHAPE, "gq_chol_gemm: M=%ld N=%ld (multiples of 256) K=%ld (of 128), ld %% 4 == 0", (long)M, (long)N, (long)K);
    if (mode < 0 || mode > 2 || kr < 0 || kr > 3 || (planes != 2 && planes != 3) || (kr == 1 && !trans_b) || (kr == 2 && trans_b))
        GQ_FAIL(GQ_E_UNSUPPORTED, "gq_chol_gemm: mode=%d kr=%d planes=%d trans_b=%d", mode, kr, planes, trans_b);
    unsigned char* p = reinterpret_cast<unsigned char*>(((uintptr_t)ws + 255) & ~(uintptr_t)255);
    unsigned char* end = reinterpret_cast<unsigned char*>(ws) + ws_bytes;
    return planes == 3 ? chol_gemm_np<3>(Cm, ldc, A, lda, B, ldb, M, N, K, trans_b, mode, kr, lower, p, end, st)
                       : chol_gemm_np<2>(Cm, ldc, A, lda, B, ldb, M, N, K, trans_b, mode, kr, lower, p, end, st);
}

}
```

### gptq-gguf-toolkit_amd/csrc/gq_diag5.hpp

```cpp
#pragma once

namespace gq {

constexpr int D5_ISPLIT = 29;
constexpr int LR5 = 36;
constexpr size_t DIAG5_LDS = (size_t)(2 * NB * LDQ + 5 * 32 * TQ + 32 * 32 + 32 * LR5 + 32 + 4) * sizeof(float);
typedef float d5_f4 __attribute__((ext_vector_type(4)));

template <int OFF>
__device__ __forceinline__ void d5_st(unsigned addr, float v) {
    asm volatile("ds_write_b32 %0, %1 offset:%2" ::"v"(addr), "v"(v), "n"(OFF) : "memory");
}
__device__ __forceinline__ void d5_sti(unsigned addr, int v) { asm volatile("ds_write_b32 %0, %1" ::"v"(addr), "v"(v) : "memory"); }

template <int VOFF>
__device__ __forceinline__ void d5_read_col(unsigned vbase, d5_f4 (&v)[8]) {
    asm volatile("ds_read_b128 %0, %1 offset:%2" : "=v"(v[0]) : "v"(vbase), "n"(VOFF + 0) : "memory");
    asm volatile("ds_read_b128 %0, %1 offset:%2" : "=v"(v[1]) : "v"(vbase), "n"(VOFF + 16) : "memory");
    asm volatile("ds_read_b128 %0, %1 offset:%2" : "=v"(v[2]) : "v"(vbase), "n"(VOFF + 32) : "memory");
    asm volatile("ds_read_b128 %0, %1 offset:%2" : "=v"(v[3]) : "v"(vbase), "n"(VOFF + 48) : "memory");
    asm volatile("ds_read_b128 %0, %1 offset:%2" : "=v"(v[4]) : "v"(vbase), "n"(VOFF + 64) : "memory");
    asm volatile("ds_read_b128 %0, %1 offset:%2" : "=v"(v[5]) : "v"(vbase), "n"(VOFF + 80) : "memory");
    asm volatile("ds_read_b128 %0, %1 offset:%2" : "=v"(v[6]) : "v"(vbase), "n"(VOFF + 96) : "memory");
    asm volatile("ds_read_b128 %0, %1 offset:%2" : "=v"(v[7]) : "v"(vbase), "n"(VOFF + 112) : "memory");
}
template <int VOFF, int Q0>
__device__ __forceinline__ void d5_read_col_from(unsigned vbase, d5_f4 (&v)[8]) {
    if constexpr (Q0 <= 0) asm volatile("ds_read_b128 %0, %1 offset:%2" : "=v"(v[0]) : "v"(vbase), "n"(VOFF + 0) : "memory");
    if constexpr (Q0 <= 1) asm volatile("ds_read_b128 %0, %1 offset:%2" : "=v"(v[1]) : "v"(vbase), "n"(VOFF + 16) : "memory");
    if constexpr (Q0 <= 2) asm volatile("ds_read_b128 %0, %1 offset:%2" : "=v"(v[2]) : "v"(vbase), "n"(VOFF + 32) : "memory");
    if constexpr (Q0 <= 3) asm volatile("ds_read_b128 %0, %1 offset:%2" : "=v"(v[3]) : "v"(vbase), "n"(VOFF + 48) : "memory");
    if constexpr (Q0 <= 4) asm volatile("ds_read_b128 %0, %1 offset:%2" : "=v"(v[4]) : "v"(vbase), "n"(VOFF + 64) : "memory");
    if constexpr (Q0 <= 5) asm volatile("ds_read_b128 %0, %1 offset:%2" : "=v"(v[5]) : "v"(vbase), "n"(VOFF + 80) : "memory");
    if constexpr (Q0 <= 6) asm volatile("ds_read_b128 %0, %1 offset:%2" : "=v"(v[6]) : "v"(vbase), "n"(VOFF + 96) : "memory");
    asm volatile("ds_read_b128 %0, %1 offset:%2" : "=v"(v[7]) : "v"(vbase), "n"(VOFF + 112) : "memory");
}
__device__ __forceinline__ void d5_wait_col(d5_f4 (&v)[8]) {
    asm volatile("s_waitcnt lgkmcnt(0)"
                 : "+v"(v[0]), "+v"(v[1]), "+v"(v[2]), "+v"(v[3]), "+v"(v[4]), "+v"(v[5]), "+v"(v[6]), "+v"(v[7])
                 :: "memory");
}

typedef float d5_f2 __attribute__((ext_vector_type(2)));
template <int C0>
__device__ __forceinline__ void d5_update_from(float (&a)[32], float p, const d5_f4 (&L)[8]) {
    if constexpr (C0 < 32 && (C0 & 1)) {
        a[C0] = fmaf(-p, L[C0 >> 2][C0 & 3], a[C0]);
        asm volatile("" : "+v"(a[C0]));
    }
    const d5_f2 np = {-p, -p};
#pragma unroll
    for (int c = (C0 + 1) & ~1; c < 32; c += 2) {
        d5_f2 t = {a[c], a[c + 1]};
        const d5_f2 l = {L[c >> 2][c & 3], L[c >> 2][(c & 3) + 1]};
        t = __builtin_elementwise_fma(np, l, t);
        asm volatile("" : "+v"(t));
        a[c] = t.x;
        a[c + 1] = t.y;
    }
}

template <int J>
__device__ __forceinline__ void d5_factor(float (&a)[32], int i, bool& bad, unsigned lcol, unsigned lcolb, unsigned lrow,
                                          unsigned invs, unsigned flag, int base, int lane, d5_f4 (&Lp)[8]) {
    asm volatile("s_nop 1" : "+v"(a[J]));
    float pj = rdlane(a[J], J);
    if (!(pj > 0.0f)) {
        bad = true;
        pj = 1.0f;
    }
    float inv = __builtin_amdgcn_rsqf(pj);
    inv = fmaf(inv, fmaf(-0.5f * pj * inv, inv, 0.5f), inv);
    a[J] = a[J] * inv;
    d5_st<J * 32 * 4>(lcol, a[J]);
    d5_st<J * 4>(lrow, a[J]);
    d5_st<J * 4>(invs, inv);
    d5_sti(flag, base + J + 1);
    if constexpr (J < 31) {
        asm volatile("s_nop 1" : "+v"(a[J]));
        const float l = rdlane(a[J], J + 1);
        a[J + 1] = fmaf(-a[J], l, a[J + 1]);
        asm volatile("" : "+v"(a[J + 1]));
    }
    if constexpr (J >= 1 && J < 31) {
        d5_wait_col(Lp);
        d5_update_from<J + 1>(a, a[J - 1], Lp);
    }
    if constexpr (J < 30) {
        d5_read_col_from<J * 32 * 4, (J + 2) / 4>(lcolb, Lp);
        d5_factor<J + 1>(a, i, bad, lcol, lcolb, lrow, invs, flag, base, lane, Lp);
    } else if constexpr (J == 30) {
        d5_factor<J + 1>(a, i, bad, lcol, lcolb, lrow, invs, flag, base, lane, Lp);
    }
}

__device__ __forceinline__ void d5_need(unsigned flag, int need, int& avail) {
    while (avail < need) {
        int f;
        asm volatile("ds_read_b32 %0, %1\n\ts_waitcnt lgkmcnt(0)" : "=v"(f) : "v"(flag) : "memory");
        avail = __builtin_amdgcn_readfirstlane(f);
        if (avail < need) __builtin_amdgcn_s_sleep(2);
    }
}
template <int OFF>
__device__ __forceinline__ void d5_read_f32(unsigned base, float& v) {
    asm volatile("ds_read_b32 %0, %1 offset:%2" : "=v"(v) : "v"(base), "n"(OFF) : "memory");
}
__device__ __forceinline__ void d5_wait_col1(d5_f4 (&v)[8], float& sc) {
    asm volatile("s_waitcnt lgkmcnt(0)"
                 : "+v"(sc), "+v"(v[0]), "+v"(v[1]), "+v"(v[2]), "+v"(v[3]), "+v"(v[4]), "+v"(v[5]), "+v"(v[6]), "+v"(v[7])
                 :: "memory");
}

template <int J>
__device__ __forceinline__ void d5_panel(float (&a)[32], unsigned lcolb, unsigned invs, unsigned flag, int base, int& avail,
                                         d5_f4 (&Lc)[8], float invj, d5_f4 (&Ln)[8]) {
    const float p = a[J] * invj;
    a[J] = p;
    float invn = 0.0f;
    if constexpr (J < 31) {
        d5_need(flag, base + J + 2, avail);
        d5_read_f32<(J + 1) * 4>(invs, invn);
        d5_read_col_from<(J + 1) * 32 * 4, (J + 2) / 4>(lcolb, Ln);
    }
    d5_update_from<J + 1>(a, p, Lc);
    if constexpr (J < 31) {
        d5_wait_col1(Ln, invn);
        d5_panel<J + 1>(a, lcolb, invs, flag, base, avail, Ln, invn, Lc);
    }
}

template <int R, int REND>
__device__ __forceinline__ void d5_inverse(float (&x)[32], int i, unsigned lrowb, unsigned invs, unsigned flag, int base,
                                           int& avail, d5_f4 (&Lc)[8], float irr, d5_f4 (&Ln)[8], float& irr_out) {
    float irn = 0.0f;
    if constexpr (R < 31) {
        d5_need(flag, base + R + 2, avail);
        d5_read_f32<(R + 1) * 4>(invs, irn);
        d5_read_col<(R + 1) * LR5 * 4>(lrowb, Ln);
    }
    d5_f2 acc2[2] = {{0.0f, 0.0f}, {0.0f, 0.0f}};
#pragma unroll
    for (int p = 0; p + 1 < R; p += 2) {
        const d5_f2 l = {Lc[p >> 2][p & 3], Lc[p >> 2][(p & 3) + 1]};
        const d5_f2 xx = {x[p], x[p + 1]};
        acc2[(p >> 1) & 1] = __builtin_elementwise_fma(l, xx, acc2[(p >> 1) & 1]);
    }
    float tail = 0.0f;
    if constexpr (R & 1) tail = Lc[(R - 1) >> 2][(R - 1) & 3] * x[R - 1];
    const float dot = ((acc2[0].x + acc2[0].y) + (acc2[1].x + acc2[1].y)) + tail;
    int ii = i;
    asm volatile("" : "+v"(ii));
    x[R] = (R < ii) ? 0.0f : ((R == ii) ? irr : -dot * irr);
    asm volatile("" : "+v"(x[R]));
    if constexpr (R < 31) {
        d5_wait_col1(Ln, irn);
        if constexpr (R + 1 < REND) d5_inverse<R + 1, REND>(x, i, lrowb, invs, flag, base, avail, Ln, irn, Lc, irr_out);
        else irr_out = irn;
    }
}

#define D5_STAMP(k) (void)0

__global__ __launch_bounds__(320) void diag_blk5_kernel(float* __restrict__ A, int64_t lda, float* __restrict__ Xout,
                                                        int64_t ldx, int* __restrict__ flag_out) {
    extern __shared__ __attribute__((aligned(16))) float smem[];
    float* S = smem;
    float* X = smem + NB * LDQ;
    float* Tw0 = X + NB * LDQ;
    float* Lcol = Tw0 + 5 * 32 * TQ;
    float* Lrow = Lcol + 32 * 32;
    float* Invs = Lrow + 32 * LR5;
    int* Step = reinterpret_cast<int*>(Invs + 32);
    const int tid = threadIdx.x, lane = tid & 63, wid = tid >> 6;
    float* Tw = Tw0 + wid * 32 * TQ;
    if (tid == 0) *Step = 0;
    if (wid == 0) D5_STAMP(0);
    if (tid < 256) {
        float4 v[NB * NB / 4 / 256];
#pragma unroll
        for (int q = 0; q < NB * NB / 4 / 256; ++q) {
            const int idx = tid + q * 256, r = idx / (NB / 4), c = (idx % (NB / 4)) * 4;
            v[q] = (c <= r) ? *reinterpret_cast<const float4*>(A + r * lda + c) : make_float4(0.f, 0.f, 0.f, 0.f);
        }
#pragma unroll
        for (int q = 0; q < NB * NB / 4 / 256; ++q) {
            const int idx = tid + q * 256, r = idx / (NB / 4), c = (idx % (NB / 4)) * 4;
            S[r * LDQ + c + 0] = (c + 0 <= r) ? v[q].x : 0.0f;
            S[r * LDQ + c + 1] = (c + 1 <= r) ? v[q].y : 0.0f;
            S[r * LDQ + c + 2] = (c + 2 <= r) ? v[q].z : 0.0f;
            S[r * LDQ + c + 3] = (c + 3 <= r) ? v[q].w : 0.0f;
        }
    }
    __syncthreads();
    if (wid == 0) D5_STAMP(1);
    const unsigned lcol_b = (unsigned)(uintptr_t)Lcol, lrow_b = (unsigned)(uintptr_t)Lrow;
    const unsigned invs_b = (unsigned)(uintptr_t)Invs, step_b = (unsigned)(uintptr_t)Step;
    const int lc = lane & 31, lh = lane >> 5;
    const int i = lane & 31;
    float xinv[32];
    d5_f4 xL0[8], xL1[8];
    float xirr = 0.0f;
    for (int sb = 0; sb < 4; ++sb) {
        const int c0 = 32 * sb, base = 32 * sb;
        if (wid == sb) {
            float a[32];
#pragma unroll
            for (int c = 0; c < 32; ++c) a[c] = S[(c0 + i) * LDQ + c0 + c];
            bool bad = false;
            d5_f4 Lp[8];
            d5_factor<0>(a, i, bad, lcol_b + (unsigned)(i * 4), lcol_b, lrow_b + (unsigned)(i * LR5 * 4), invs_b, step_b, base, lane, Lp);
            if (lane < 32) {
#pragma unroll
                for (int c = 0; c < 32; ++c) {
                    int ii = i;
                    asm volatile("" : "+v"(ii));
                    S[(c0 + i) * LDQ + c0 + c] = (c <= ii) ? a[c] : 0.0f;
                }
                if (bad && lane == 0) *flag_out = 1;
            }
        } else if (wid > sb && wid < 4) {
            float a[32];
#pragma unroll
            for (int c = 0; c < 32; ++c) a[c] = S[(32 * wid + i) * LDQ + c0 + c];
            int avail = 0;
            d5_f4 L0[8], L1[8];
            float inv0;
            d5_need(step_b, base + 1, avail);
            d5_read_f32<0>(invs_b, inv0);
            d5_read_col<0>(lcol_b, L0);
            d5_wait_col1(L0, inv0);
            d5_panel<0>(a, lcol_b, invs_b, step_b, base, avail, L0, inv0, L1);
            if (lane < 32) {
#pragma unroll
                for (int c = 0; c < 32; ++c) S[(32 * wid + i) * LDQ + c0 + c] = a[c];
            }
        } else if (wid == 4) {
            int avail = 0;
            float inv0;
            d5_need(step_b, base + 1, avail);
            d5_read_f32<0>(invs_b, inv0);
            d5_read_col<0>(lrow_b, xL0);
            d5_wait_col1(xL0, inv0);
            d5_inverse<0, D5_ISPLIT>(xinv, i, lrow_b, invs_b, step_b, base, avail, xL0, inv0, xL1, xirr);
        }
        D5_STAMP(16 + 8 * sb + wid);
        __syncthreads();
        if (wid == 0) D5_STAMP(2 + 2 * sb);
        if (wid == 4) {
            int avail = base + 32;
            d5_inverse<D5_ISPLIT, 32>(xinv, i, lrow_b, invs_b, step_b, base, avail, (D5_ISPLIT & 1) ? xL1 : xL0, xirr,
                                      (D5_ISPLIT & 1) ? xL0 : xL1, xirr);
            if (lane < 32) {
#pragma unroll
                for (int c = 0; c < 32; ++c) X[(c0 + c) * LDQ + c0 + i] = xinv[c];
            }
        }
        int t = 0;
        for (int bi = sb + 1; bi < 4; ++bi)
            for (int bj = sb + 1; bj <= bi; ++bj, ++t) {
                if ((t & 3) != wid) continue;
                f32x16 acc = mfma_nt_32(S + (32 * bi) * LDQ + c0, LDQ, S + (32 * bj) * LDQ + c0, LDQ, lane);
#pragma unroll
                for (int e = 0; e < 16; ++e) {
                    float* p = S + (32 * bi + (e & 3) + 8 * (e >> 2) + 4 * lh) * LDQ + 32 * bj + lc;
                    *p = *p - acc[e];
                }
            }
        __syncthreads();
        if (wid == 0) D5_STAMP(3 + 2 * sb);
    }
    {
        const int li = lane & 31, lk = lane >> 5;
        auto prod = [&](f32x16& acc, const float* PA, int lda_, int ar, int ak, const float* PB, int ldb_, int bk, int bc) {
            float av[16], bv[16];
#pragma unroll
            for (int p = 0; p < 16; ++p) {
                av[p] = PA[(ar + li) * lda_ + ak + 2 * p + lk];
                bv[p] = PB[(bk + 2 * p + lk) * ldb_ + bc + li];
            }
#pragma unroll
            for (int p = 0; p < 16; ++p) acc = __builtin_amdgcn_mfma_f32_32x32x2f32(av[p], bv[p], acc, 0, 0, 0);
        };
        auto zero = [](f32x16& acc) {
#pragma unroll
            for (int e = 0; e < 16; ++e) acc[e] = 0.0f;
        };
        auto put = [&](float* P, int ld_, int r0, int c0_, const f32x16& acc, float sgn) {
#pragma unroll
            for (int e = 0; e < 16; ++e) P[(r0 + (e & 3) + 8 * (e >> 2) + 4 * lh) * ld_ + c0_ + lc] = sgn * acc[e];
        };
        if (wid < 2) {
            const int bi = 2 * wid + 1, bj = 2 * wid;
            f32x16 acc;
            zero(acc);
            prod(acc, S, LDQ, 32 * bi, 32 * bj, X, LDQ, 32 * bj, 32 * bj);
            put(Tw, TQ, 0, 0, acc, 1.0f);
            zero(acc);
            prod(acc, X, LDQ, 32 * bi, 32 * bi, Tw, TQ, 0, 0);
            put(X, LDQ, 32 * bi, 32 * bj, acc, -1.0f);
        }
        __syncthreads();
        const int r = (wid >> 1) & 1, c = wid & 1;
        if (wid < 4) {
            f32x16 acc;
            zero(acc);
            for (int k = c; k < 2; ++k) prod(acc, S, LDQ, 32 * (2 + r), 32 * k, X, LDQ, 32 * k, 32 * c);
            put(Tw, TQ, 0, 0, acc, 1.0f);
        }
        __syncthreads();
        if (wid < 4) {
            f32x16 acc;
            zero(acc);
            for (int k = 0; k <= r; ++k) prod(acc, X, LDQ, 32 * (2 + r), 32 * (2 + k), Tw0 + (2 * k + c) * 32 * TQ, TQ, 0, 0);
            put(X, LDQ, 32 * (2 + r), 32 * c, acc, -1.0f);
        }
        __syncthreads();
    }
    if (wid == 0) D5_STAMP(10);
    for (int idx = tid; idx < NB * NB / 4; idx += 320) {
        const int r = idx / (NB / 4), c = (idx % (NB / 4)) * 4;
        const float* sr = S + r * LDQ + c;
        const float* xr = X + r * LDQ + c;
        *reinterpret_cast<float4*>(Xout + r * ldx + c) =
            (c >> 5) > (r >> 5) ? make_float4(0.f, 0.f, 0.f, 0.f) : make_float4(xr[0], xr[1], xr[2], xr[3]);
        (void)sr;
    }
    if (wid == 0) D5_STAMP(11);
}

}
```

### gptq-gguf-toolkit_amd/csrc/gq_gemm32.hpp

```cpp
#pragma once
#include <atomic>
#include <stdlib.h>

#include <type_traits>

#include "gq_common.hpp"

namespace gq {

typedef float f32x16 __attribute__((ext_vector_type(16)));
constexpr int TM = 128, TN = 128, TK = 32;
constexpr int LDA_S = TK + 1;
constexpr int LDBT_S = TK + 1;
template <int TS> struct G32 {
    static constexpr int NV = TS / 32;
    static constexpr int LDB = TS + 4;
    static constexpr int A_FLOATS = TS * LDA_S;
    static constexpr int B_FLOATS = (TK * LDB > TS * LDBT_S) ? TK * LDB : TS * LDBT_S;
    static constexpr int STAGE_FLOATS = A_FLOATS + B_FLOATS;
    static constexpr int LDS_BYTES = 2 * STAGE_FLOATS * 4;
};
constexpr int LDB_S = G32<128>::LDB;
constexpr int G32_LDS_BYTES = G32<128>::LDS_BYTES;

// ... 488 lines not shown
        by = (id & 7) * (nby / 8) + j / nbx;
        bx = j % nbx;
    } else {
        by = id / nbx;
        bx = id % nbx;
    }
    const int64_t m0 = (int64_t)by * 64, n0 = (int64_t)bx * 64;
    const unsigned lds0 = (unsigned)(uintptr_t)g32_smem;
    const int wm = wid >> 1, wn = wid & 1;
    const int li = lane & 31, lk = lane >> 5;
    f32x16 cv;
    float* cp = Cmat + (m0 + wm * 32 + 4 * lk) * ldc + n0 + wn * 32 + li;
#define GQ_N_DL(vo, sp, ldsaddr) \
    asm volatile("s_mov_b32 m0, %2\n\ts_nop 0\n\tglobal_load_lds_dwordx4 %0, %1" ::"v"(vo), "s"(sp), "s"(ldsaddr) : "memory")
    {
        const float* bp = B + n0;
        const unsigned bvo = (unsigned)(((lane >> 4) * ldb + (lane & 15) * 4) * 4);
        const int arow = lane >> 4;
        const float* ap = A + m0 * lda;
#define GQ_N_QUARTER(q)                                                                                               \
    do {                                                                                                              \
        _Pragma("unroll") for (int r = 0; r < 4; ++r) {                                                               \
            const int j = (q) * 16 + wid * 4 + r;              \
            const float* sp_ = bp + (int64_t)(4 * j) * ldb;                                                           \
            GQ_N_DL(bvo, sp_, lds0 + NEAR_A_BYTES + (unsigned)j * 1024u);                                             \
        }                                                                                                             \
        _Pragma("unroll") for (int r = 0; r < 4; ++r) {                                                               \
            const int row0 = wid * 16 + 4 * r;                      \
            const unsigned avo = (unsigned)((arow * lda + (q) * 64 + (((lane & 15) ^ (4 * r + arow)) << 2)) * 4);     \
            const float* sp_ = ap + (int64_t)row0 * lda;                                                              \
            GQ_N_DL(avo, sp_, lds0 + (unsigned)((q) * 16384 + row0 * 256));                                           \
        }                                                                                                             \
    } while (0)
        GQ_N_QUARTER(0);
#pragma unroll
        for (int e = 0; e < 16; ++e) cv[e] = cp[((e & 3) + 8 * (e >> 2)) * ldc];
        GQ_N_QUARTER(1);
        GQ_N_QUARTER(2);
        GQ_N_QUARTER(3);
#undef GQ_N_QUARTER
    }
#undef GQ_N_DL
    unsigned aaddr[16];
    {
        const int row = wm * 32 + li;
#pragma unroll
        for (int u = 0; u < 16; ++u) aaddr[u] = lds0 + (unsigned)(row * 256 + ((u ^ (row & 15)) << 4));
    }
    const unsigned bbase = lds0 + NEAR_A_BYTES + (unsigned)(lk * 64 + wn * 32 + li) * 4u;
    g32_u32x4 fa[3];
    float fb0[3], fb1[3];
#define GQ_N_READS(g, s)                                                                                              \
    do {                                                                                                              \
        asm volatile("ds_read_b128 %0, %1 offset:%2" : "=v"(fa[s]) : "v"(aaddr[(g) & 15]), "n"(((g) >> 4) * 16384) : "memory"); \
        asm volatile("ds_read_b32 %0, %1 offset:%2" : "=v"(fb0[s]) : "v"(bbase), "n"((g) * 1024) : "memory");         \
        asm volatile("ds_read_b32 %0, %1 offset:%2" : "=v"(fb1[s]) : "v"(bbase), "n"((g) * 1024 + 512) : "memory");   \
    } while (0)
    asm volatile("s_waitcnt vmcnt(40)" ::: "memory");
    __builtin_amdgcn_s_barrier();
    GQ_N_READS(0, 0);
    GQ_N_READS(1, 1);
    const f32x16 zero = {0.f, 0.f, 0.f, 0.f, 0.f, 0.f, 0.f, 0.f, 0.f, 0.f, 0.f, 0.f, 0.f, 0.f, 0.f, 0.f};
    f32x16 acc = zero;
#define GQ_N_GROUP(g)                                                                                            \
    do {                                                                                                         \
        constexpr int s_ = (g) % 3;                                                                              \
        if ((g) % 16 == 14 && (g) < 48) {                                                                        \
            if ((g) == 14) asm volatile("s_waitcnt vmcnt(16)" ::: "memory");                                     \
            else if ((g) == 30) asm volatile("s_waitcnt vmcnt(8)" ::: "memory");                                 \
            else asm volatile("s_waitcnt vmcnt(0)" ::: "memory");                                                \
            __builtin_amdgcn_s_barrier();                                                                        \
        }                                                                                                        \
        if ((g) + 2 < NEAR_K / 4) {                                                                              \
            GQ_N_READS(((g) + 2 < NEAR_K / 4) ? (g) + 2 : 0, ((g) + 2) % 3);                                     \
            asm volatile("s_waitcnt lgkmcnt(6)" : "+v"(fa[s_]), "+v"(fb0[s_]), "+v"(fb1[s_])::"memory");         \
        } else if ((g) + 1 < NEAR_K / 4) {                                                                       \
            asm volatile("s_waitcnt lgkmcnt(3)" : "+v"(fa[s_]), "+v"(fb0[s_]), "+v"(fb1[s_])::"memory");         \
        } else {                                                                                                 \
            asm volatile("s_waitcnt lgkmcnt(0)" : "+v"(fa[s_]), "+v"(fb0[s_]), "+v"(fb1[s_])::"memory");         \
        }                                                                                                        \
        const float a0_ = __builtin_bit_cast(float, lk ? fa[s_].y : fa[s_].x);                                   \
        const float a1_ = __builtin_bit_cast(float, lk ? fa[s_].w : fa[s_].z);                                   \
        acc = __builtin_amdgcn_mfma_f32_32x32x2f32(a0_, fb0[s_], ((g) % 32 == 0) ? zero : acc, 0, 0, 0);         \
        acc = __builtin_amdgcn_mfma_f32_32x32x2f32(a1_, fb1[s_], acc, 0, 0, 0);                                  \
        if ((g) % 32 == 31) {                                                                                    \
            _Pragma("unroll") for (int e = 0; e < 16; ++e) cv[e] = cv[e] - acc[e];                               \
        }                                                                                                        \
    } while (0)
#define GQ_N_G8(g) GQ_N_GROUP(g); GQ_N_GROUP((g) + 1); GQ_N_GROUP((g) + 2); GQ_N_GROUP((g) + 3); \
                   GQ_N_GROUP((g) + 4); GQ_N_GROUP((g) + 5); GQ_N_GROUP((g) + 6); GQ_N_GROUP((g) + 7)
    GQ_N_G8(0); GQ_N_G8(8); GQ_N_G8(16); GQ_N_G8(24); GQ_N_G8(32); GQ_N_G8(40); GQ_N_G8(48); GQ_N_G8(56);
#undef GQ_N_G8
#undef GQ_N_GROUP
#undef GQ_N_READS
#pragma unroll
    for (int e = 0; e < 16; ++e) cp[((e & 3) + 8 * (e >> 2)) * ldc] = cv[e];
}

inline int launch_gemm32_near256(float* Cmat, int64_t ldc, const float* A, int64_t lda, const float* B, int64_t ldb, int64_t M,
                                 int64_t N, hipStream_t st) {
    static std::atomic<bool> attr_set{false};
    if (!attr_set) {
        GQ_HIP(hipFuncSetAttribute((const void*)gemm32_near256_kernel<128>, hipFuncAttributeMaxDynamicSharedMemorySize, NEAR_LDS_BYTES));
        attr_set = true;
    }
    const unsigned nbx = (unsigned)(N / 64), nby = (unsigned)(M / 64);
    hipLaunchKernelGGL(gemm32_near256_kernel<128>, dim3(nbx * nby), dim3(256), NEAR_LDS_BYTES, st, Cmat, ldc, A, lda, B, ldb, nbx, nby);
    GQ_LAUNCH_CHECK();
    return GQ_OK;
}

template <bool TRANS_B, int MODE, bool LOWER, int KR, int CHAIN, int TS, bool FULL>
inline int launch_gemm32_full(float* Cmat, int64_t ldc, const float* A, int64_t lda, const float* B, int64_t ldb, int64_t M,
                            int64_t N, int64_t K, hipStream_t st) {
    constexpr int NW = (CHAIN != 0 && TS == 128) ? 8 : 4;
    static std::atomic<bool> attr_set{false};
    if (!attr_set) {
        GQ_HIP(hipFuncSetAttribute((const void*)gemm32_kernel<TRANS_B, MODE, LOWER, KR, CHAIN, TS, FULL, NW>,
                                   hipFuncAttributeMaxDynamicSharedMemorySize, G32<TS>::LDS_BYTES));
        attr_set = true;
    }
    dim3 grid((unsigned)((N + TS - 1) / TS), (unsigned)((M + TS - 1) / TS)), block(NW * 64);
    hipLaunchKernelGGL((gemm32_kernel<TRANS_B, MODE, LOWER, KR, CHAIN, TS, FULL, NW>), grid, block, G32<TS>::LDS_BYTES, st, Cmat, ldc,
                       A, lda, B, ldb, M, N, K);
    GQ_LAUNCH_CHECK();
    return GQ_OK;
}

template <bool TRANS_B, int MODE, bool LOWER, int KR, int CHAIN, int TS>
inline int launch_gemm32_ts(float* Cmat, int64_t ldc, const float* A, int64_t lda, const float* B, int64_t ldb, int64_t M,
                            int64_t N, int64_t K, hipStream_t st) {
    if constexpr (CHAIN == 128 && TS == 128 && !TRANS_B && MODE == 0 && !LOWER && KR == 0) {
        if (M % TS == 0 && N % TS == 0) return launch_gemm32_chain_full<CHAIN>(Cmat, ldc, A, lda, B, ldb, M, N, K, st);
    }
    if (M % TS == 0 && N % TS == 0 && K % TK == 0 && ldc % 4 == 0)
        return launch_gemm32_full<TRANS_B, MODE, LOWER, KR, CHAIN, TS, true>(Cmat, ldc, A, lda, B, ldb, M, N, K, st);
    return launch_gemm32_full<TRANS_B, MODE, LOWER, KR, CHAIN, TS, false>(Cmat, ldc, A, lda, B, ldb, M, N, K, st);
}

template <bool TRANS_B, int MODE, bool LOWER, int KR = 0, int CHAIN = 0>
inline int launch_gemm32(float* Cmat, int64_t ldc, const float* A, int64_t lda, const float* B, int64_t ldb, int64_t M,
                         int64_t N, int64_t K, hipStream_t st) {
    if (M <= 0 || N <= 0 || K <= 0) return GQ_OK;
    if ((lda % 4) || (ldb % 4) || ((uintptr_t)A % 16) || ((uintptr_t)B % 16))
        GQ_FAIL(GQ_E_BAD_SHAPE, "gemm32: A/B must be 16-byte aligned with ld %% 4 == 0");
    if (CHAIN != 0 && (K % CHAIN)) GQ_FAIL(GQ_E_BAD_SHAPE, "gemm32: K=%ld is not a multiple of the chain length %d", (long)K, CHAIN);
    const int64_t tiles128 = ((M + 127) / 128) * ((N + 127) / 128) / (LOWER ? 2 : 1);
    const int64_t max64 = opt(OPT_gemm32_64_max);
    if (CHAIN == 0 && tiles128 < max64)
        return launch_gemm32_ts<TRANS_B, MODE, LOWER, KR, CHAIN == 0 ? 0 : 0, 64>(Cmat, ldc, A, lda, B, ldb, M, N, K, st);
    return launch_gemm32_ts<TRANS_B, MODE, LOWER, KR, CHAIN, 128>(Cmat, ldc, A, lda, B, ldb, M, N, K, st);
}

}
```

### gptq-gguf-toolkit_amd/gptq.py

```python
import os
from typing import Optional, Sequence, Tuple

import torch
import torch.distributed as dist
import torch.nn as nn
from torch import Tensor
from torch.nn.modules.conv import _ConvNd

from . import dist_utils, model_utils
from . import ops as _ops
from .quant_utils import GGML_QUANT_SIZES, GGMLQuantizationType, QuantizationScale, _check_scale


class GPTQ:
    def __init__(self, layer: nn.Module, rel_damp: float = 1e-2, block_size: Optional[int] = None,
                 act_order: bool = False, quant_scale: str = "absmax", rmin: float = -1.0, rdelta: float = 0.1,
                 nstep: int = 20, grid: int = 100, static_groups: bool = False, verbose: bool = False,
                 allow_no_samples: bool = False):
        if act_order:
            assert static_groups
        assert isinstance(layer, (nn.Linear, _ConvNd)), "OBC supports only linear and convolutional layers."
        self.layer = layer
        self.W = layer.weight
        self.d_row, self.d_col = model_utils.get_number_of_rows_and_cols(layer)
        self.rel_damp = rel_damp
        self.block_size = block_size or self.d_col
        self.act_order = act_order
        self.quant_scale = _check_scale(quant_scale)
        self.static_groups = static_groups
        self.grid, self.rmin, self.rdelta, self.nstep = grid, rmin, rdelta, nstep
        self.W_device, self.W_dtype, self.W_shape = self.W.device, self.W.dtype, self.W.shape
        self.H: Optional[Tensor] = None
        self.num_samples = 0
        self.verbose = verbose
        self.owner_rank = 0
        self.row_split = False
        self.row_split_redone = False
        self._researches = None
        self._last_cf = None
        self.reduce_to = None
        self.allow_no_samples = allow_no_samples
        self.no_samples = False
        self.shared_H_with = None
        self._has_followers = False
        self._scheduled = False
        self._reduced = False
        self._pending_mismatch = None
        self._flag = None
        self._ws = None
        self.flush_tokens = 1 << 16
        self._buf = None
        self._fill = 0
        self._staged = 0
        self._segs = []
        self._rag = []
        self._zero_copy = True
        self._buf_b = 0
        self._U_cache = None
        self._last_U = None

    @torch.no_grad()
    def update(self, input: Tensor) -> None:
        batch_size = input.shape[0]
        if self.shared_H_with is not None:
            self.num_samples += batch_size
            return
        if self.H is None:
            self.H = torch.zeros((self.d_col, self.d_col), device=input.device, dtype=torch.float32)
        if isinstance(self.layer, nn.Linear):
            x = input.reshape(-1, input.shape[-1])
        else:
            unfold = nn.Unfold(self.layer.kernel_size, dilation=self.layer.dilation, padding=self.layer.padding,
                               stride=self.layer.stride)
            x = unfold(input).transpose(1, 2).flatten(0, 1)
        if x.dtype not in (torch.float16, torch.bfloat16, torch.float32):
            x = x.float()
        t = x.shape[0]
        keepable = self._zero_copy and x.is_cuda and x.dtype in (torch.float16, torch.bfloat16) and x.is_contiguous() \
            and x.data_ptr() % 16 == 0 and t > 0
        if keepable and self._staged == 0 and not self._rag and t % 128 == 0 and self.d_col % 256 == 0 \
                and (not self._segs or (self._segs[0][0].shape == x.shape and self._segs[0][0].dtype == x.dtype)):
            self._segs.append((x, x._version, batch_size))
        elif keepable and self.d_col % 8 == 0 and self._pending_dtype() in (None, x.dtype):
            self._rag += [(y, v) for y, v, _ in self._segs]
            self._segs = []
            self._rag.append((x, x._version))
        else:
            self._stage(x)
        self._fill += t
        self._buf_b += batch_size
        if self._fill >= self.flush_tokens and not self._scheduled:
            self.flush()

    def _gather(self) -> None:
        if not self._rag:
            return
        for x, v in self._rag:
            if x._version != v:
                raise RuntimeError("a Linear input was modified in place after its forward hook ran; set the handle's "
                                   "_zero_copy = False to copy activations at hook time")
        xs = [x for x, _ in self._rag]
        need = self._staged + sum(x.shape[0] for x in xs)
        if self._buf is None or self._buf.dtype != xs[0].dtype or self._buf.shape[0] - self._PAD < need:
            assert self._buf is None or self._buf.dtype == xs[0].dtype or self._staged == 0
            bigger = torch.empty((need + self._PAD, self.d_col), device=xs[0].device, dtype=xs[0].dtype)
            if self._staged:
                _ops.h_stage(bigger, 0, self._buf[:self._staged])
            self._buf = bigger
        _ops.h_stage_many(self._buf, self._staged, xs)
        self._staged = need
        self._rag = []

    def _stage(self, x: Tensor) -> None:
        if self._pending_dtype() not in (None, x.dtype):
            self.flush()
        self._gather()
        pend, self._segs = [y for y, _, _ in self._segs], []
        need = self._staged + sum(y.shape[0] for y in pend) + x.shape[0]
        cap = self.flush_tokens + x.shape[0]
        room = self._buf.shape[0] - self._PAD if self._buf is not None else 0
        if self._buf is not None and self._buf.dtype == x.dtype and room < need <= cap:
            bigger = torch.empty((min(cap, max(4 * room, need)) + self._PAD, self.d_col), device=x.device, dtype=x.dtype)
            if self._staged:
                _ops.h_stage(bigger, 0, self._buf[:self._staged])
            self._buf = bigger
        if self._buf is not None and (self._buf.dtype != x.dtype or need > self._buf.shape[0] - self._PAD):
            if self._staged:
                self.flush()
                need = x.shape[0]
            self._buf = None
        if self._buf is None:
            self._buf = torch.empty((max(need, min(cap, 4 * need)) + self._PAD, self.d_col), device=x.device, dtype=x.dtype)
        for y in pend + [x]:
            _ops.h_stage(self._buf, self._staged, y)
            self._staged += y.shape[0]

    def _pending_dtype(self):
        if self._segs or self._rag:
            return (self._segs or self._rag)[0][0].dtype
        return self._buf.dtype if self._buf is not None and self._staged else None

    def _pending_device(self):
        if self._segs or self._rag:
            return (self._segs or self._rag)[0][0].device
        return self._buf.device if self._buf is not None else None

    @torch.no_grad()
    def flush(self) -> None:
        if self._fill == 0:
            return
        H, X, beta, alpha = self._flush_args()
        _ops.h_accumulate(H, X, beta, alpha)
        self._flush_done()

    def _flush_args(self):
        n, b = self.num_samples, self._buf_b
        self._gather()
        if self._segs:
            for x, v, _ in self._segs:
                if x._version != v:
                    raise RuntimeError("a Linear input was modified in place after its forward hook ran; set the handle's "
                                       "_zero_copy = False to copy activations at hook time")
            X = [x for x, _, _ in self._segs]
        else:
            pad = (-self._staged) % self._PAD
            if pad and self._buf.dtype in (torch.float16, torch.bfloat16) and self.d_col % 256 == 0 and self._buf.is_cuda:
                _ops.h_stage(self._buf, self._staged, self._zero_rows(pad))
            else:
                pad = 0
            X = self._buf[:self._staged + pad]
        return self.H, X, n / (n + b), 2.0 / (n + b)

    _PAD = 128
    _zeros: dict = {}

    def _zero_rows(self, n: int) -> Tensor:
        key = (self._buf.device, self._buf.dtype, self.d_col)
        z = GPTQ._zeros.get(key)
        if z is None:
            z = GPTQ._zeros[key] = torch.zeros((self._PAD, self.d_col), device=self._buf.device, dtype=self._buf.dtype)
        return z[:n]

    def _flush_done(self) -> None:
        self.num_samples += self._buf_b
        self._fill = 0
        self._staged = 0
        self._segs = []
        self._rag = []
        self._buf_b = 0

    def reset(self) -> None:
        self.W = self.layer.weight
        self.H = None
        self.num_samples = 0
        self._ws = None
        self._buf = None
        self._fill = 0
        self._staged = 0
        self._segs = []
        self._rag = []
        self._buf_b = 0
        self._reduced = False
        self.shared_H_with = None
        self._has_followers = False
        self._U_cache = None
        self._last_U = None
        self._pending_mismatch = None
        self._flag = None
        self.no_samples = False
        self.owner_rank = 0
        self.row_split = False
        self._researches = None
        self._last_cf = None
        self.reduce_to = None

    @torch.no_grad()
    def quantization_pre_step(self) -> None:
        self.sync_hessian()
        self.make_working_copy()
        self.pre_step_completed = True

    @torch.no_grad()
    def sync_hessian(self) -> None:
        if self.shared_H_with is not None:
            leader = self.shared_H_with
            if not leader._reduced:
                leader.sync_hessian()
            self.H = leader.H
            self._reduced = True
            return
        if self._reduced:
            return
        if not self.allow_no_samples:
            assert self.H is not None, "One has to process at least one sample of calibration data to run pruning"
        if self.H is None:
            self.H = torch.zeros((self.d_col, self.d_col), device=self.W_device, dtype=torch.float32)
        self.flush()
        self._buf = None
        if not self._reduced:
            if self.allow_no_samples:
                total = dist_utils.allreduce_hessian(self.H, self.num_samples, dst=self.reduce_to)
                if total == 0:
                    self.H = torch.eye(self.d_col, device=self.W_device, dtype=torch.float32)
                    self.no_samples = True
            else:
                dist_utils.allreduce_hessian(self.H, dst=self.reduce_to)
            self._reduced = True
            if self.reduce_to is not None and self.reduce_to != dist_utils.get_rank() and dist_utils.get_world_size() > 1:
                self.H = None

    @torch.no_grad()
    def make_working_copy(self, out: Optional[Tensor] = None) -> None:
        W = self.layer.weight.detach()
        if out is not None:
            assert out.shape == (self.d_row, self.d_col) and out.dtype == torch.float32 and out.is_contiguous()
            out.copy_(W.flatten(1, -1) if isinstance(self.layer, _ConvNd) else W)
            self.W = out
            return
        W = W.clone() if W.dtype == torch.float32 else W.float()
        if isinstance(self.layer, _ConvNd):
            W = W.flatten(1, -1)
        self.W = W.contiguous()

    @torch.no_grad()
    def _prepare(self, defer_check: bool = False, own_U: bool = False) -> Tensor:
        leader = self.shared_H_with or self
        shared = self.shared_H_with is not None or self._has_followers
        if shared and leader._U_cache is not None and not own_U:
            U, flag, cf = leader._U_cache
            self._last_cf = cf
            mismatch = _ops.w_prepare(cf, self.W)
            if defer_check:
                self._pending_mismatch, self._flag = mismatch, flag
                return U
            if int(mismatch.item()) == 0:
                self._flag = flag
                return U
        H = self.H.clone() if shared else self.H
        U, self._flag, cf = _ops.h_prepare(H, self.W, self.rel_damp, want_flags=True)
        self._last_cf = cf
        if shared and leader._U_cache is None and not own_U:
            leader._U_cache = (U, self._flag, cf)
        if not shared:
            self.H = H
        return U

    @property
    def issue_non_invertible(self) -> bool:
        return bool(self._flag is not None and int(self._flag.item()) != 0)

    @torch.no_grad()
    def compute(self, q_type: GGMLQuantizationType, defer_check: bool = False, own_U: bool = False):
        if q_type == GGMLQuantizationType.Q3_K:
            self.act_order = False
            self.static_groups = False
        self.row_split_redone = False
        if self.act_order:
            return self._compute_act_order(q_type)
        U = self._prepare(defer_check, own_U)
        self._last_U = U
        W = self.W
        if self._row_split_active():
            r0, r1, _ = dist_utils.row_slice(self.d_row, dist_utils.get_rank(), dist_utils.get_world_size())
            self._researches = torch.zeros(1, dtype=torch.int32, device=self.W.device)
            if r1 <= r0:
                return tuple(t[:0] for t in self._empty_result(q_type))
            W = self.W[r0:r1]
            return _ops.gptq_quantize(W, U, int(q_type), self.block_size, self.static_groups, self.rmin, self.rdelta,
                                      self.nstep, quant_scale=self.quant_scale.value, grid=self.grid,
                                      panel_researches=self._researches)
        return _ops.gptq_quantize(W, U, int(q_type), self.block_size, self.static_groups, self.rmin,
                                  self.rdelta, self.nstep, quant_scale=self.quant_scale.value, grid=self.grid)

    @torch.no_grad()
    def recompute_whole(self, q_type: GGMLQuantizationType):
        assert self._last_U is not None and self._last_cf is not None, "recompute_whole() follows compute()"
        self.make_working_copy()
        _ops.w_prepare(self._last_cf, self.W)
        return _ops.gptq_quantize(self.W, self._last_U, int(q_type), self.block_size, self.static_groups, self.rmin,
                                  self.rdelta, self.nstep, quant_scale=self.quant_scale.value, grid=self.grid)

    def stack_key(self, q_type: GGMLQuantizationType):
        if self.act_order and q_type != GGMLQuantizationType.Q3_K:
            return None
        if self._row_split_active() or self.d_row % 64 or self.layer.weight.dtype not in (torch.float16, torch.bfloat16, torch.float32):
            return None
        return (int(q_type), self.d_col, self.block_size, bool(self.static_groups) and q_type != GGMLQuantizationType.Q3_K,
                self.rmin, self.rdelta, self.nstep, self.quant_scale, self.grid, self.rel_damp, str(self.W_device))

    @staticmethod
    @torch.no_grad()
    def compute_stacked(hs: Sequence["GPTQ"], q_type: GGMLQuantizationType):
        assert len(hs) > 1 and all(h.stack_key(q_type) == hs[0].stack_key(q_type) is not None for h in hs)
        rows = [h.d_row for h in hs]
        ends = [sum(rows[:i + 1]) for i in range(len(rows))]
        Wf = torch.empty((ends[-1], hs[0].d_col), device=hs[0].W_device, dtype=torch.float32)
        U = None
        for h, r1, n in zip(hs, ends, rows):
            if q_type == GGMLQuantizationType.Q3_K:
                h.act_order = False
                h.static_groups = False
            h.make_working_copy(out=Wf[r1 - n:r1])
            Uh = h._prepare(defer_check=True)
            assert U is None or Uh is U, "stacked handles must share one factorisation"
            U = Uh
            h._last_U = U
        h0 = hs[0]
        res = _ops.gptq_quantize(Wf, U, int(q_type), h0.block_size, h0.static_groups, h0.rmin, h0.rdelta, h0.nstep,
                                 quant_scale=h0.quant_scale.value, grid=h0.grid, row_ends=ends)
        for h in hs:
            h.W = None
        return [tuple(t[r1 - n:r1] for t in res) for r1, n in zip(ends, rows)]

    def levels_key(self):
        key = self.stack_key(GGMLQuantizationType.Q4_K)
        return None if key is None else key[1:]

    @staticmethod
    @torch.no_grad()
    def compute_levels(hs: Sequence["GPTQ"], q_types: Sequence[GGMLQuantizationType], own_U: bool = False,
                       defer_check: bool = False, walks: Optional[list] = None):
        q_types = [GGMLQuantizationType(t) for t in q_types]
        if not hs or not q_types or len(set(q_types)) != len(q_types):
            raise ValueError("compute_levels needs at least one handle and distinct levels")
        for h in hs:
            if h.act_order or h.static_groups:
                raise ValueError("compute_levels: act_order / static_groups handles have no level build")
            if h._row_split_active():
                raise NotImplementedError("compute_levels: row-split (multi-rank) handles")
        out = {h: {} for h in hs}
        h0, L = hs[0], len(q_types)
        mq = dict(quant_scale=h0.quant_scale.value, grid=h0.grid)
        banded = [h for h in hs if h.levels_key() is not None]
        assert all(h.levels_key() == banded[0].levels_key() for h in banded), "banded handles must share one grid setup"
        U = None

        def prepare(h):
            nonlocal U
            Uh = h._prepare(defer_check=True, own_U=own_U)
            assert U is None or Uh is U, "the handles of a level build must share one factorisation"
            U = h._last_U = Uh

        per_call = max(1, _ops.BANDS_MAX // L)
        for i in range(0, len(banded), per_call):
            grp = banded[i:i + per_call]
            C = grp[0].d_col
            Wf = torch.empty((L * sum(h.d_row for h in grp), C), device=grp[0].W_device, dtype=torch.float32)
            bands, r0 = [], 0
            for h in grp:
                h.make_working_copy(out=Wf[r0:r0 + h.d_row])
                prepare(h)
                for k, t in enumerate(q_types):
                    if k:
                        Wf[r0 + k * h.d_row:r0 + (k + 1) * h.d_row].copy_(Wf[r0:r0 + h.d_row])
                    bands.append((r0 + (k + 1) * h.d_row, int(t)))
                r0 += L * h.d_row
            if walks is None:
                res = _ops.gptq_quantize_bands(Wf, U, bands, h0.block_size, h0.rmin, h0.rdelta, h0.nstep, **mq)
            else:
                res, stacked = _ops.gptq_quantize_bands(Wf, U, bands, h0.block_size, h0.rmin, h0.rdelta, h0.nstep,
                                                        return_stacked=True, **mq)
                walks.append((stacked, bands, [(h, t) for h in grp for t in q_types]))
            for j, h in enumerate(grp):
                out[h] = {t: res[j * L + k] for k, t in enumerate(q_types)}
                h.W = None
        for h in hs:
            if h.levels_key() is not None:
                continue
            for k, t in enumerate(q_types):
                h.make_working_copy()
                if k == 0:
                    prepare(h)
                else:
                    _ops.w_prepare(h._last_cf, h.W)
                out[h][t] = _ops.gptq_quantize(h.W, U, int(t), h.block_size, False, h.rmin, h.rdelta, h.nstep, **mq)
                if walks is not None:
                    walks.append((out[h][t], [(h.d_row, int(t))], [(h, t)]))
            h.W = None
        if not defer_check:
            pending = [h for h in hs if h._pending_mismatch is not None]
            if pending:
                flags = torch.cat([h._pending_mismatch.reshape(1) for h in pending]).tolist()
                for h, bad in zip(pending, flags):
                    h._pending_mismatch = None
                    if bad:
                        if walks is not None:
                            for _, _, members in walks:
                                members[:] = [None if mem is not None and mem[0] is h else mem for mem in members]
                        out[h] = GPTQ.compute_levels([h], q_types, own_U=True, walks=walks)[h]
        return out

    def _row_split_active(self) -> bool:
        return bool(self.row_split) and not self.act_order and dist_utils.get_world_size() > 1

    @torch.no_grad()
    def _compute_act_order(self, q_type: GGMLQuantizationType):
        H = self.H
        diag = torch.diagonal(H).clone()
        dead = diag == 0
        diag[dead] = 1.0
        self.W[:, dead] = 0
        perm = torch.argsort(diag, descending=True, stable=True)
        _, d, s, dmin, m = _ops.rtn_quantize(self.W, int(q_type), self.rmin, self.rdelta, self.nstep,
                                             quant_scale=self.quant_scale.value, grid=self.grid)
        Wp = self.W[:, perm].contiguous()
        Hp = H[perm][:, perm].contiguous()
        U, self._flag = _ops.h_prepare(Hp, Wp, self.rel_damp)
        qp = _ops.gptq_quantize_perm(Wp, U, int(q_type), perm.to(torch.int32).contiguous(), d, s, dmin, m,
                                     block_size=self.block_size)
        self.W = Wp
        q = qp[:, torch.argsort(perm)].contiguous()
        return q, d, s, dmin, m

    def _empty_result(self, q_type):
        bits, clamp, scale_maxq, group_size, supergroup_size, sz_dtype, q_dtype = GGML_QUANT_SIZES[q_type]
        dev, R, C = self.W_device, self.d_row, self.d_col
        return (torch.empty(R, C, device=dev, dtype=q_dtype),
                torch.empty(R, C // supergroup_size, device=dev, dtype=torch.float16),
                torch.empty(R, C // group_size, device=dev, dtype=sz_dtype),
                torch.empty(R, C // supergroup_size, device=dev, dtype=torch.float16),
                torch.empty(R, C // group_size, device=dev, dtype=sz_dtype))

    @torch.no_grad()
    def exchange(self, result, q_type: GGMLQuantizationType):
        if self._row_split_active():
            _, _, chunk = dist_utils.row_slice(self.d_row, dist_utils.get_rank(), dist_utils.get_world_size())
            q = result[0]
            world = dist_utils.get_world_size()
            padded = torch.zeros((chunk + 1, q.shape[1]), dtype=q.dtype, device=q.device)
            padded[:q.shape[0]] = q
            padded.view(torch.uint8)[chunk, :4] = self._researches.view(torch.uint8)
            gathered = dist_utils.all_gather_rows(padded, (chunk + 1) * world, chunk + 1)
            per = gathered.view(world, chunk + 1, q.shape[1])
            counts = per[:, chunk, :4].contiguous().view(torch.uint8).view(torch.int32)
            if int(counts.sum().item()) != 0:
                self.row_split_redone = True
                return self.recompute_whole(q_type)
            qfull = per[:, :chunk].reshape(world * chunk, q.shape[1])[:self.d_row]
            return (qfull,) + tuple(dist_utils.all_gather_rows(t, self.d_row, chunk) for t in result[1:])
        if result is None:
            result = self._empty_result(q_type)
        if dist_utils.is_dist_available_and_initialized() and dist_utils.get_world_size() > 1:
            for t in result:
                dist_utils.collective_calls["broadcast"] += 1
                dist.broadcast(t, src=self.owner_rank)
        return result

    @torch.no_grad()
    def step(self, q_type: GGMLQuantizationType) -> Tuple[Tensor, Tensor, Tensor, Tensor, Tensor]:
        if q_type == GGMLQuantizationType.Q3_K:
            self.act_order = False
        mine = dist_utils.get_rank() == self.owner_rank or self._row_split_active()
        res = self.compute(q_type) if mine else None
        return self.exchange(res, q_type)

    def quantize(self, q_type: GGMLQuantizationType):
        self.quantization_pre_step()
        return self.step(q_type)
```

### gptq-gguf-toolkit_amd/ops.py

```python
import ctypes
from typing import Optional, Sequence, Tuple

import torch

from . import _cabi
from ._cabi import F16, F32, BF16, Search, check, lib, type_info
from ._cabi import option_get, option_set, options
from .gguf_writer import GGML_QUANT_SIZES, PACKED_TYPES

_DT = {torch.float32: F32, torch.float16: F16, torch.bfloat16: BF16}


def _stream(t: torch.Tensor):
    return ctypes.c_void_p(torch.cuda.current_stream(t.device).cuda_stream)


def _ptr(t: Optional[torch.Tensor]):
    return ctypes.c_void_p(t.data_ptr()) if t is not None else ctypes.c_void_p(0)


def _need_cuda(*ts):
    for t in ts:
        if t is not None and not t.is_cuda:
            raise _cabi.GQError("gptq_gguf_toolkit_amd ops need GPU tensors (no CPU fallback); got a CPU tensor")


def _search(rmin=-1.0, rdelta=0.1, nstep=20, quant_scale="absmax", grid=100, maxshrink=0.8):
    mode = getattr(quant_scale, "value", quant_scale)
    if mode not in ("absmax", "mse"):
        raise ValueError(f"quant_scale must be 'absmax' or 'mse', got {quant_scale!r}")
    return ctypes.byref(Search(float(rmin), float(rdelta), int(nstep), int(mode == "mse"), int(grid), float(maxshrink)))


def _idt(q_type):
    return torch.int8 if type_info(q_type)["is_signed"] else torch.uint8


def _u8(t):
    return t.view(torch.uint8) if t.dtype != torch.uint8 else t


def _u16view(t):
    return t.view(torch.int16) if t.dtype == torch.float16 else t


def _ws(nbytes: int, device) -> torch.Tensor:
    return torch.empty(max(int(nbytes), 256), dtype=torch.uint8, device=device)


def workspace_bytes(op: int, R=0, C=0, T=0, block_size=0) -> int:
    return int(lib().gq_workspace_bytes(op, R, C, T, block_size))


def h_accumulate(H: torch.Tensor, X: torch.Tensor, beta: float, alpha: float, ws: Optional[torch.Tensor] = None):
    if isinstance(X, (list, tuple)):
        return h_accumulate_grouped([H], [X], [beta], [alpha], ws)[0]
    _need_cuda(H, X)
    assert H.dtype == torch.float32 and H.is_contiguous() and X.is_contiguous() and X.dim() == 2
    T, C = X.shape
    assert H.shape == (C, C)
    need = workspace_bytes(_cabi.WS_H_ACCUMULATE, 0, C, T)
    if ws is None or ws.numel() < need:
        ws = _ws(need, X.device)
    check(lib().gq_h_accumulate(_ptr(H), _ptr(X), _DT[X.dtype], T, C, beta, alpha, _ptr(ws), ws.numel(), _stream(X)),
          "gq_h_accumulate")
    return H


def h_accumulate_grouped(Hs, Xs, betas, alphas, ws: Optional[torch.Tensor] = None):
    n = len(Hs)
    assert n == len(Xs) == len(betas) == len(alphas) and 1 <= n <= 8
    blocks = [list(X) if isinstance(X, (list, tuple)) else [X] for X in Xs]
    _need_cuda(*Hs, *[b for bl in blocks for b in bl])
    dt = blocks[0][0].dtype
    for H, bl in zip(Hs, blocks):
        assert H.dtype == torch.float32 and H.is_contiguous()
        for X in bl:
            assert X.is_contiguous() and X.dim() == 2 and X.dtype == dt and X.shape == bl[0].shape
        assert H.shape == (bl[0].shape[1], bl[0].shape[1])
    Ts = [len(bl) * bl[0].shape[0] for bl in blocks]
    need = sum(workspace_bytes(_cabi.WS_H_ACCUMULATE, 0, bl[0].shape[1], T) for bl, T in zip(blocks, Ts))
    if ws is None or ws.numel() < need:
        ws = _ws(need, blocks[0][0].device)
    vp = ctypes.c_void_p
    Hp = (vp * n)(*[H.data_ptr() for H in Hs])
    Cs = (ctypes.c_int64 * n)(*[bl[0].shape[1] for bl in blocks])
    bs = (ctypes.c_float * n)(*[float(b) for b in betas])
    as_ = (ctypes.c_float * n)(*[float(a) for a in alphas])
    if all(len(bl) == 1 for bl in blocks):
        Xp = (vp * n)(*[bl[0].data_ptr() for bl in blocks])
        Tc = (ctypes.c_int64 * n)(*Ts)
        check(lib().gq_h_accumulate_grouped(n, Hp, Xp, Tc, Cs, bs, as_, _DT[dt], _ptr(ws), ws.numel(),
                                            _stream(blocks[0][0])), "gq_h_accumulate_grouped")
        return Hs
    lists = [(vp * len(bl))(*[X.data_ptr() for X in bl]) for bl in blocks]
    Bp = (vp * n)(*[ctypes.cast(l, vp).value for l in lists])
    nb = (ctypes.c_int64 * n)(*[len(bl) for bl in blocks])
    bt = (ctypes.c_int64 * n)(*[bl[0].shape[0] for bl in blocks])
    check(lib().gq_h_accumulate_segments(n, Hp, Bp, nb, bt, Cs, bs, as_, _DT[dt], _ptr(ws), ws.numel(),
                                         _stream(blocks[0][0])), "gq_h_accumulate_segments")
    return Hs


def h_stage(buf: torch.Tensor, fill: int, x: torch.Tensor):
    _need_cuda(buf, x)
    assert buf.is_contiguous() and buf.dtype == x.dtype and x.dim() == 2 and x.shape[1] == buf.shape[1]
    assert fill + x.shape[0] <= buf.shape[0]
    if not x.is_contiguous():
        x = x.contiguous()
    row = buf.shape[1] * buf.element_size()
    check(lib().gq_h_stage(ctypes.c_void_p(buf.data_ptr() + fill * row), _ptr(x), x.shape[0] * row, _stream(buf)),
          "gq_h_stage")


def h_stage_many(buf: torch.Tensor, fill: int, xs: Sequence[torch.Tensor]):
    _need_cuda(buf, *xs)
    row = buf.shape[1] * buf.element_size()
    total = sum(x.shape[0] for x in xs)
    assert buf.is_contiguous() and fill + total <= buf.shape[0] and row % 16 == 0
    assert all(x.dtype == buf.dtype and x.dim() == 2 and x.shape[1] == buf.shape[1] and x.is_contiguous() for x in xs)
    n = len(xs)
    srcs = (ctypes.c_void_p * n)(*[x.data_ptr() for x in xs])
    nb = (ctypes.c_int64 * n)(*[x.shape[0] * row for x in xs])
    ws = _ws((2 * n + 1) * 8 + 512, buf.device)
    check(lib().gq_h_stage_many(ctypes.c_void_p(buf.data_ptr() + fill * row), srcs, nb, n, _ptr(ws), ws.numel(), _stream(buf)),
          "gq_h_stage_many")


def h_prepare(H: torch.Tensor, W: torch.Tensor, rel_damp: float, want_flags: bool = False, obq_order: bool = False):
    _need_cuda(H, W)
    assert H.dtype == torch.float32 and W.dtype == torch.float32 and H.is_contiguous() and W.is_contiguous()
    R, C = W.shape
    U = torch.empty_like(H)
    flag = torch.empty(1, dtype=torch.int32, device=H.device)
    cf = torch.empty(2 * C, dtype=torch.uint8, device=H.device) if want_flags else None
    ws = _ws(workspace_bytes(_cabi.WS_H_PREPARE, R, C), H.device)
    fn = lib().gq_obq_h_prepare if obq_order else lib().gq_h_prepare
    check(fn(_ptr(H), _ptr(W), R, C, rel_damp, _ptr(U), _ptr(flag), _ptr(cf), _ptr(ws), ws.numel(), _stream(H)),
          "gq_obq_h_prepare" if obq_order else "gq_h_prepare")
    return (U, flag, cf) if want_flags else (U, flag)


def w_prepare(col_flags: torch.Tensor, W: torch.Tensor) -> torch.Tensor:
    _need_cuda(col_flags, W)
    assert W.dtype == torch.float32 and W.is_contiguous() and col_flags.numel() == 2 * W.shape[1]
    mm = torch.empty(1, dtype=torch.int32, device=W.device)
    check(lib().gq_w_prepare(_ptr(col_flags), _ptr(W), W.shape[0], W.shape[1], _ptr(mm), _stream(W)), "gq_w_prepare")
    return mm


def h_pack_upper(H: torch.Tensor) -> torch.Tensor:
    _need_cuda(H)
    C = H.shape[0]
    assert H.dtype == torch.float32 and H.is_contiguous() and H.shape == (C, C) and C % 128 == 0
    nt = C // 128
    buf = torch.empty(nt * (nt + 1) // 2, 128, 128, dtype=torch.float32, device=H.device)
    check(lib().gq_h_pack_upper(_ptr(H), C, _ptr(buf), _stream(H)), "gq_h_pack_upper")
    return buf


def h_unpack_upper(buf: torch.Tensor, H: torch.Tensor) -> torch.Tensor:
    _need_cuda(buf, H)
    C = H.shape[0]
    assert H.dtype == torch.float32 and H.is_contiguous() and buf.dtype == torch.float32 and buf.is_contiguous()
    check(lib().gq_h_unpack_upper(_ptr(buf), C, _ptr(H), _stream(H)), "gq_h_unpack_upper")
    return H


def scale_search(x: torch.Tensor, q_type: int, rmin=-1.0, rdelta=0.1, nstep=20, **mq):
    _need_cuda(x)
    assert x.dtype == torch.float32 and x.dim() == 2 and x.shape[1] == 256 and x.stride(1) == 1
    rows = x.shape[0]
    ng = 256 // type_info(q_type)["group"]
    dev = x.device
    d = torch.empty(rows, dtype=torch.float16, device=dev)
    dmin = torch.empty(rows, dtype=torch.float16, device=dev)
    s = torch.empty(rows, ng, dtype=torch.uint8, device=dev)
    m = torch.empty(rows, ng, dtype=torch.uint8, device=dev)
    check(lib().gq_scale_search(_ptr(x), rows, x.stride(0), int(q_type), _search(rmin, rdelta, nstep, **mq), _ptr(d), 1,
                                _ptr(s), ng, _ptr(dmin), 1, _ptr(m), ng, _stream(x)), "gq_scale_search")
    t = _idt(q_type)
    return d, s.view(t), dmin, m.view(t)


def _alloc_outs(R, C, q_type, dev):
    G = type_info(q_type)["group"]
    return (torch.empty(R, C, dtype=torch.uint8, device=dev), torch.empty(R, C // 256, dtype=torch.float16, device=dev),
            torch.empty(R, C // G, dtype=torch.uint8, device=dev),
            torch.empty(R, C // 256, dtype=torch.float16, device=dev),
            torch.empty(R, C // G, dtype=torch.uint8, device=dev))


def _walk_ws(ws: Optional[torch.Tensor], R, C, bs, device) -> torch.Tensor:
    need = workspace_bytes(_cabi.WS_GPTQ_QUANTIZE, R, C, 0, bs)
    return ws if ws is not None and ws.numel() >= need else _ws(need, device)


def _kquant_outs(q_type, q, d, s, dmin, m):
    t = _idt(q_type)
    return q.view(t), d, s.view(t), dmin, m.view(t)


_side_streams = {}


def _streams(device, n):
    pool = _side_streams.setdefault(device, [])
    while len(pool) < n:
        pool.append(torch.cuda.Stream(device))
    return pool[:n]


def gptq_quantize(W: torch.Tensor, U: torch.Tensor, q_type: int, block_size=128, static_groups=False, rmin=-1.0,
                  rdelta=0.1, nstep=20, ws: Optional[torch.Tensor] = None, row_chunks: Optional[int] = None,
                  row_ends: Optional[Sequence[int]] = None, panel_researches: Optional[torch.Tensor] = None, **mq):
    _need_cuda(W, U)
    assert W.dtype == torch.float32 and U.dtype == torch.float32 and W.is_contiguous() and U.is_contiguous()
    R, C = W.shape
    q, d, s, dmin, m = _alloc_outs(R, C, q_type, W.device)
    bs = int(block_size or 0)
    if row_chunks is None:
        row_chunks = 1
    if row_chunks > 1 and (R % (64 * row_chunks) or ws is not None):
        row_chunks = 1

    def one(r0, r1, wsbuf, entry="gq_gptq_quantize", extra=()):
        n = r1 - r0
        wsbuf = _walk_ws(wsbuf, n, C, bs, W.device)
        check(getattr(lib(), entry)(_ptr(W[r0:r1]), _ptr(U), n, C, int(q_type), bs, int(bool(static_groups)),
                                    _search(rmin, rdelta, nstep, **mq), _ptr(q[r0:r1]), _ptr(d[r0:r1]), _ptr(s[r0:r1]),
                                    _ptr(dmin[r0:r1]), _ptr(m[r0:r1]), *extra, _ptr(wsbuf), wsbuf.numel(), _stream(W)), entry)
        return wsbuf

    if row_ends is not None and len(row_ends) > 1:
        ends = (ctypes.c_int64 * len(row_ends))(*[int(e) for e in row_ends])
        one(0, R, ws, "gq_gptq_quantize_stacked", (ends, len(row_ends)))
    elif panel_researches is not None:
        assert panel_researches.dtype == torch.int32 and panel_researches.is_cuda and panel_researches.numel() >= 1
        one(0, R, ws, "gq_gptq_quantize_slice", (_ptr(panel_researches),))
    elif row_chunks == 1:
        one(0, R, ws)
    else:
        cur = torch.cuda.current_stream(W.device)
        fork = torch.cuda.Event()
        fork.record(cur)
        step = R // row_chunks
        keep = []
        for k, st in enumerate(_streams(W.device, row_chunks)):
            st.wait_event(fork)
            with torch.cuda.stream(st):
                keep.append(one(k * step, (k + 1) * step, None))
            ev = torch.cuda.Event()
            ev.record(st)
            cur.wait_event(ev)
        for b in keep:
            b.record_stream(cur)
    return _kquant_outs(q_type, q, d, s, dmin, m)


BANDS_MAX = _cabi.BANDS_MAX
_K_GROUP = {10: 16, 11: 16, 12: 32, 13: 32, 14: 16}
_K_SIGNED = {10: False, 11: True, 12: False, 13: False, 14: True}


def band_layout(bands: Sequence[Tuple[int, int]], C: int):
    if not 1 <= len(bands) <= BANDS_MAX:
        raise ValueError(f"{len(bands)} bands (1..{BANDS_MAX})")
    out, r0, off = [], 0, 0
    for k, (r1, t) in enumerate(bands):
        r1, t = int(r1), int(t)
        if t not in _K_GROUP:
            raise ValueError(f"band {k} has unknown q_type {t}")
        if r1 % 64 or r1 <= r0:
            raise ValueError(f"band {k} ends at row {r1} (ascending multiples of 64)")
        g = _K_GROUP[t]
        out.append((r0, r1, t, g, off))
        off += (r1 - r0) * (C // g)
        r0 = r1
    return out, off


def gptq_quantize_bands(W: torch.Tensor, U: torch.Tensor, bands: Sequence[Tuple[int, int]], block_size=128, rmin=-1.0,
                        rdelta=0.1, nstep=20, ws: Optional[torch.Tensor] = None, return_stacked: bool = False, **mq):
    _need_cuda(W, U)
    assert W.dtype == torch.float32 and U.dtype == torch.float32 and W.is_contiguous() and U.is_contiguous()
    R, C = W.shape
    n = len(bands)
    tbl = (_cabi.Band * max(n, 1))(*[_cabi.Band(int(e), int(t)) for e, t in bands])
    dev = W.device
    q = torch.empty(R, C, dtype=torch.uint8, device=dev)
    d = torch.empty(R, C // 256, dtype=torch.float16, device=dev)
    dmin = torch.empty(R, C // 256, dtype=torch.float16, device=dev)
    s = torch.empty(R * (C // 16), dtype=torch.uint8, device=dev)
# ... 809 lines not shown
```

Baseline: 2505 Mparams/s.

## Batch Hessian preparation and Cholesky factorisation across same-width chains

Adds a batched h_prepare path that runs column flagging, damping, equilibration and the blocked Cholesky/inverse for up to eight Hessians of equal width in one set of launches, with the batch index carried in blockIdx.y. The block schedule groups eligible chain leaders by width, factorises them together on one lane ahead of the per-chain work, and hands the resulting U back to each handle. The aim is to cut per-matrix launch overhead and fill the GPU better on the small per-matrix factorisation kernels. In exchange, independent chains now serialise behind one batched prepare, adding a dependency event and extra bookkeeping for stacked buffers, plus an H clone for leaders that have followers.

```diff
diff --git a/gptq-gguf-toolkit_amd/_cabi.py b/gptq-gguf-toolkit_amd/_cabi.py
--- a/gptq-gguf-toolkit_amd/_cabi.py
+++ b/gptq-gguf-toolkit_amd/_cabi.py
@@ -42,6 +42,8 @@
 MOE_COMBINE_MAX_K = 8
 EXPORTS_MOE_SEARCH = ("gq_level_switch_experts",)
 SWITCH_EXPERTS_MAX_JOBS = 71
+EXPORTS_PREPARE_BATCH = ("gq_h_prepare_batch_workspace_bytes", "gq_h_prepare_batch")
+PREPARE_BATCH_MAX = 8
 
 
 class GQError(RuntimeError):
@@ -161,6 +163,9 @@
     L.gq_linear_packed_experts.argtypes = [ci, vp, i64, i64, i64, vp, i64, i64, vp, vp, i64, ci, vp, vp]
     L.gq_fwd_moe_combine.argtypes = [vp, vp, vp, vp, vp, ci, i64, i64, i64, i64, ci, vp, vp]
     L.gq_level_switch_experts.argtypes = [ctypes.POINTER(SwitchExpertsJob), ci, vp]
+    L.gq_h_prepare_batch_workspace_bytes.argtypes = [ci, vp, i64]
+    L.gq_h_prepare_batch_workspace_bytes.restype = sz
+    L.gq_h_prepare_batch.argtypes = [ci, vp, vp, vp, i64, cf, vp, vp, vp, vp, sz, vp]
     L.gq_prof_enable.argtypes = [ctypes.c_uint]
     L.gq_prof_enable.restype = None
     L.gq_prof_name.argtypes = [ci]
@@ -169,7 +174,7 @@
     L.gq_prof_collect2.argtypes = [ctypes.POINTER(ctypes.c_double), ctypes.POINTER(ctypes.c_long),
                                    ctypes.POINTER(ctypes.c_double)]
     for name in (EXPORTS + EXPORTS_ERREST + EXPORTS_SEARCH + EXPORTS_LEVELS + EXPORTS_LEVELPACK + EXPORTS_Q8 + EXPORTS_IQ4_ENCODE + EXPORTS_IQ4_GPTQ + EXPORTS_QGEMM +
-                 EXPORTS_QGEMV + EXPORTS_SAMPLE + EXPORTS_MOE + EXPORTS_MOE_GEMM + EXPORTS_MOE_CALIB + EXPORTS_MOE_SEARCH):
+                 EXPORTS_QGEMV + EXPORTS_SAMPLE + EXPORTS_MOE + EXPORTS_MOE_GEMM + EXPORTS_MOE_CALIB + EXPORTS_MOE_SEARCH + EXPORTS_PREPARE_BATCH):
         getattr(L, name)
     _lib = L
     return L
diff --git a/gptq-gguf-toolkit_amd/block_schedule.py b/gptq-gguf-toolkit_amd/block_schedule.py
--- a/gptq-gguf-toolkit_amd/block_schedule.py
+++ b/gptq-gguf-toolkit_amd/block_schedule.py
@@ -80,6 +80,20 @@
     return lane_of, enq
 
 
+def _plan_prepare_batches(widths: List[int], eligible: List[bool], cap: int = 8) -> List[List[int]]:
+    groups: List[List[int]] = []
+    open_: Dict[int, List[int]] = {}
+    for k, (c, ok) in enumerate(zip(widths, eligible)):
+        if not ok:
+            continue
+        g = open_.get(c)
+        if g is None or len(g) >= cap:
+            g = open_[c] = []
+            groups.append(g)
+        g.append(k)
+    return [g for g in groups if len(g) > 1]
+
+
 @contextlib.contextmanager
 def _far_helper_lease(on: bool):
     was = _ops.far_helper_enable(on)
@@ -95,6 +109,7 @@
         self.qtypes, self.writeback, self.extra, self.own, self.world, self.rank = qtypes, writeback, extra, own, world, rank
         self.results: Dict[str, tuple] = {}
         self.deq: Dict[str, torch.Tensor] = {}
+        self.stacked: Dict[str, torch.Tensor] = {}
 
 
 class BlockSchedule:
@@ -117,6 +132,7 @@
         self.verbose = verbose
         self.stats = {"syrk_launches": 0, "allreduce_bytes": 0, "reused_U": 0, "own_U": 0, "refactorised": 0}
         self.owners: Dict[str, Any] = {}
+        self.prepare_batches: List[List[str]] = []
 
     def hook(self, name: str):
         def _hook(_, inp, out):
@@ -314,6 +330,7 @@
         lane_of, enq = _plan_lanes([_lane_load([handles[n] for n in names]) for names in order], len(streams))
         with _far_helper_lease(bool(lent)) if on_gpu else contextlib.nullcontext():
             lanes = []
+            released = self._prepare_batched(call, order, lane_of, enq, streams, main, ready, start, lanes)
             for k in enq:
                 if trace:
                     print(f"  [sched] +{1e3 * (time.perf_counter() - t_host):7.2f} ms: enqueue chain {k} {order[k]} on lane {lane_of[k]}",
@@ -321,6 +338,7 @@
                 lane = _Lane(streams[lane_of[k]], main)
                 lead = handles[order[k][0]].shared_H_with or handles[order[k][0]]
                 lane.wait(ready.get(id(lead), start))
+                lane.wait(released.get(k))
                 lanes.append((lane, self._run_chain(call, order[k], lane)))
             for lane, born in lanes:
                 lane.join(born)
@@ -329,6 +347,71 @@
         self._settle_late_followers(call)
         self.stats["own_U"] = len(call.results) - self.stats["reused_U"]
         return self._exchange_and_write_back(call)
+
+    def _batch_leader(self, call: _Call, names: List[str]) -> Optional[str]:
+        if not hasattr(_ops, "h_prepare_batch"):
+            return None
+        for n in names:
+            h = self.handles[n]
+            if h.shared_H_with is None:
+                ok = (not h.act_order and h.H is not None and h.H.is_cuda and not h.no_samples and h.d_col % 128 == 0
+                      and h.layer.weight.dtype in (torch.float16, torch.bfloat16, torch.float32))
+                return n if ok else None
+        return None
+
+    def _prepare_batched(self, call: _Call, order, lane_of, enq, streams, main, ready, start, lanes) -> Dict[int, Any]:
+        handles = self.handles
+        self.prepare_batches = []
+        if main is None:
+            return {}
+        leaders = [self._batch_leader(call, names) for names in order]
+        widths = [handles[names[0]].d_col for names in order]
+        damp: Dict[int, float] = {}
+        for k, n in enumerate(leaders):
+            if n is not None and damp.setdefault(widths[k], handles[n].rel_damp) != handles[n].rel_damp:
+                leaders[k] = None
+        groups = _plan_prepare_batches(widths, [n is not None for n in leaders])
+        released: Dict[int, Any] = {}
+        pos = {k: i for i, k in enumerate(enq)}
+        for grp in sorted(groups, key=lambda g: min(pos[k] for k in g)):
+            first = min(grp, key=lambda k: pos[k])
+            lane = _Lane(streams[lane_of[first]], main)
+            for k in grp:
+                lane.wait(ready.get(id(handles[leaders[k]]), start))
+            born: List[torch.Tensor] = []
+            with lane.run():
+                hs = [handles[leaders[k]] for k in grp]
+                for k, h in zip(grp, hs):
+                    n = leaders[k]
+                    stack = next(g for g in self._stack_groups(sorted(order[k], key=lambda m: handles[m].shared_H_with is not None),
+                                                               call.qtypes, call.own) if n in g)
+                    if len(stack) > 1:
+                        assert stack[0] == n
+                        Wf = call.stacked[n] = GPTQ.stacked_buffer([handles[m] for m in stack])
+                        h.make_working_copy(out=Wf[:h.d_row])
+                        born.append(Wf)
+                    else:
+                        h.make_working_copy()
+                ops_ = [h.prepare_operands() for h in hs]
+                out = _ops.h_prepare_batch([o[0] for o in ops_], [o[1] for o in ops_], hs[0].rel_damp)
+                flags = out[0][1]._base if out[0][1]._base is not None else out[0][1]
+                mine: Dict[int, List[torch.Tensor]] = {}
+                for k, h, (H, _), (U, flag, cf) in zip(grp, hs, ops_, out):
+                    h.adopt_factorisation(U, flag, cf, H)
+                    mine[k] = [U, cf, call.stacked.get(leaders[k], h.W), flags]
+                    born.extend(mine[k][:2] if leaders[k] in call.stacked else mine[k][:3])
+                born.append(flags)
+                ev = torch.cuda.Event()
+                ev.record(torch.cuda.current_stream(main.device))
+            for k in grp:
+                released[k] = ev
+                if streams[lane_of[k]] is not streams[lane_of[first]]:
+                    other = main if streams[lane_of[k]] is None else streams[lane_of[k]]
+                    for t in mine[k]:
+                        t.record_stream(other)
+            lanes.append((lane, born))
+            self.prepare_batches.append([leaders[k] for k in grp])
+        return released
 
     @torch.no_grad()
     def quantize_levels(self, levels, propagate: Optional[GGMLQuantizationType],
@@ -479,12 +562,14 @@
                 if len(grp) > 1:
                     hs = [handles[n] for n in grp]
                     self.stats["stacked"] = self.stats.get("stacked", 0) + len(grp)
-                    for n, h, res in zip(grp, hs, GPTQ.compute_stacked(hs, qtypes[grp[0]])):
+                    kw = {"Wf": call.stacked.pop(grp[0])} if grp[0] in call.stacked else {}
+                    for n, h, res in zip(grp, hs, GPTQ.compute_stacked(hs, qtypes[grp[0]], **kw)):
                         self._computed(call, born, n, h, res)
                     continue
                 n = grp[0]
                 h = handles[n]
-                h.make_working_copy()
+                if h._adopted is None:
+                    h.make_working_copy()
                 self._computed(call, born, n, h, h.compute(qtypes[n], defer_check=True, own_U=call.own.get(n, False)))
         return born
 
diff --git a/gptq-gguf-toolkit_amd/csrc/gq_cholesky.hip b/gptq-gguf-toolkit_amd/csrc/gq_cholesky.hip
--- a/gptq-gguf-toolkit_amd/csrc/gq_cholesky.hip
+++ b/gptq-gguf-toolkit_amd/csrc/gq_cholesky.hip
@@ -5,6 +5,7 @@
 #include "gq_gemm32.hpp"
 #include "gq_gemm3b.hpp"
 #include "gq_gemm3p.hpp"
+#include "../../include/gptq_gguf_prepare_batch.h"
 
 #include <map>
 #include <memory>
@@ -14,7 +15,7 @@
 
 constexpr int NB = 128;
 
-__global__ __launch_bounds__(256) void col_flags_kernel(const float* __restrict__ H, const float* __restrict__ W,
+__device__ __forceinline__ void col_flags_body(const float* __restrict__ H, const float* __restrict__ W,
                                                         int64_t R, int64_t C, uint8_t* __restrict__ dead,
                                                         uint8_t* __restrict__ zc) {
     const int64_t j = (int64_t)blockIdx.x * 64 + (threadIdx.x & 63);
@@ -33,7 +34,7 @@
     }
 }
 
-__global__ __launch_bounds__(256) void zero_dead_cols_kernel(float* __restrict__ W, int64_t R, int64_t C,
+__device__ __forceinline__ void zero_dead_cols_body(float* __restrict__ W, int64_t R, int64_t C,
                                                              const uint8_t* __restrict__ dead) {
     const int64_t j = (int64_t)blockIdx.x * 64 + (threadIdx.x & 63);
     const bool dd = j < C && dead[j];
@@ -65,7 +66,7 @@
     }
 }
 
-__global__ __launch_bounds__(256) void col_flags4_kernel(const float* __restrict__ H, const float* __restrict__ W,
+__device__ __forceinline__ void col_flags4_body(const float* __restrict__ H, const float* __restrict__ W,
                                                          int64_t R, int64_t C, uint8_t* __restrict__ dead,
                                                          uint8_t* __restrict__ zc) {
     const int tx = threadIdx.x & 15, ty = threadIdx.x >> 4;
@@ -126,7 +127,7 @@
     }
 }
 
-__global__ __launch_bounds__(256) void mask_h_kernel(float* __restrict__ H, int64_t C, const uint8_t* __restrict__ zc) {
+__device__ __forceinline__ void mask_h_body(float* __restrict__ H, int64_t C, const uint8_t* __restrict__ zc) {
     __shared__ int flagged[64];
     const int64_t i0 = (int64_t)blockIdx.x * 64;
     if (threadIdx.x < 64) flagged[threadIdx.x] = (i0 + threadIdx.x < C) && zc[i0 + threadIdx.x];
@@ -147,7 +148,7 @@
     if (j < C && dead[j]) H[j * C + j] = 1.0f;
 }
 
-__global__ __launch_bounds__(1024) void damp_kernel(float* __restrict__ H, int64_t C, float rel_damp) {
+__device__ __forceinline__ void damp_body(float* __restrict__ H, int64_t C, float rel_damp) {
     __shared__ double part[1024];
     double acc = 0.0;
     for (int64_t i = threadIdx.x; i < C; i += 1024) acc += (double)H[i * C + i];
@@ -161,7 +162,7 @@
     for (int64_t i = threadIdx.x; i < C; i += 1024) H[i * C + i] += damp;
 }
 
-__global__ __launch_bounds__(256) void equil_kernel(const float* __restrict__ H, int64_t n, float* __restrict__ s) {
+__device__ __forceinline__ void equil_body(const float* __restrict__ H, int64_t n, float* __restrict__ s) {
     const int64_t j = (int64_t)blockIdx.x * blockDim.x + threadIdx.x;
     if (j >= n) return;
     const float h = H[j * n + j];
@@ -174,7 +175,7 @@
     }
     s[j] = v;
 }
-__global__ __launch_bounds__(256) void reverse_copy_kernel(float* __restrict__ A, const float* __restrict__ H,
+__device__ __forceinline__ void reverse_copy_body(float* __restrict__ A, const float* __restrict__ H,
                                                            int64_t n, const float* __restrict__ s) {
     const int64_t i = blockIdx.x, r = n - 1 - i;
     const int64_t jend = (i / 128 + 1) * 128;
@@ -190,7 +191,7 @@
     }
 }
 
-__global__ __launch_bounds__(256) void finish_u_kernel(float* __restrict__ U, const float* __restrict__ X, int64_t n,
+__device__ __forceinline__ void finish_u_body(float* __restrict__ U, const float* __restrict__ X, int64_t n,
                                                        const int* __restrict__ flag, const float* __restrict__ s) {
     const int64_t i = blockIdx.x, r = n - 1 - i;
     const bool bad = *flag != 0;
@@ -214,7 +215,7 @@
 
 constexpr int LDP = NB + 4;
 
-__global__ __launch_bounds__(256) void diag_potrf_inv_kernel(float* __restrict__ A, int64_t lda,
+__device__ __forceinline__ void diag_potrf_inv_body(float* __restrict__ A, int64_t lda,
                                                              float* __restrict__ Xout, int64_t ldx,
                                                              int* __restrict__ flag) {
     extern __shared__ __attribute__((aligned(16))) float smem[];
@@ -311,6 +312,91 @@
     }
 }
 
+__global__ __launch_bounds__(256) void col_flags_kernel(const float* __restrict__ H, const float* __restrict__ W,
+                                                        int64_t R, int64_t C, uint8_t* __restrict__ dead,
+                                                        uint8_t* __restrict__ zc) {
+    col_flags_body(H, W, R, C, dead, zc);
+}
+__global__ __launch_bounds__(256) void col_flags4_kernel(const float* __restrict__ H, const float* __restrict__ W,
+                                                         int64_t R, int64_t C, uint8_t* __restrict__ dead,
+                                                         uint8_t* __restrict__ zc) {
+    col_flags4_body(H, W, R, C, dead, zc);
+}
+__global__ __launch_bounds__(256) void zero_dead_cols_kernel(float* __restrict__ W, int64_t R, int64_t C,
+                                                             const uint8_t* __restrict__ dead) {
+    zero_dead_cols_body(W, R, C, dead);
+}
+__global__ __launch_bounds__(256) void mask_h_kernel(float* __restrict__ H, int64_t C, const uint8_t* __restrict__ zc) {
+    mask_h_body(H, C, zc);
+}
+__global__ __launch_bounds__(1024) void damp_kernel(float* __restrict__ H, int64_t C, float rel_damp) {
+    damp_body(H, C, rel_damp);
+}
+__global__ __launch_bounds__(256) void equil_kernel(const float* __restrict__ H, int64_t n, float* __restrict__ s) {
+    equil_body(H, n, s);
+}
+__global__ __launch_bounds__(256) void reverse_copy_kernel(float* __restrict__ A, const float* __restrict__ H,
+                                                           int64_t n, const float* __restrict__ s) {
+    reverse_copy_body(A, H, n, s);
+}
+__global__ __launch_bounds__(256) void finish_u_kernel(float* __restrict__ U, const float* __restrict__ X, int64_t n,
+                                                       const int* __restrict__ flag, const float* __restrict__ s) {
+    finish_u_body(U, X, n, flag, s);
+}
+__global__ __launch_bounds__(256) void diag_potrf_inv_kernel(float* __restrict__ A, int64_t lda,
+                                                             float* __restrict__ Xout, int64_t ldx,
+                                                             int* __restrict__ flag) {
+    diag_potrf_inv_body(A, lda, Xout, ldx, flag);
+}
+
+constexpr int PREP_BATCH_MAX = 8;
+struct PrepBatch {
+    float* H[PREP_BATCH_MAX];
+    float* W[PREP_BATCH_MAX];
+    int64_t R[PREP_BATCH_MAX];
+    uint8_t* dead[PREP_BATCH_MAX];
+    float* A[PREP_BATCH_MAX];
+    float* X[PREP_BATCH_MAX];
+    float* U[PREP_BATCH_MAX];
+    float* eq_s[PREP_BATCH_MAX];
+    int* flag[PREP_BATCH_MAX];
+};
+__global__ __launch_bounds__(256) void col_flags_batch_kernel(const PrepBatch b, int64_t C) {
+    const unsigned z = blockIdx.y;
+    col_flags_body(b.H[z], b.W[z], b.R[z], C, b.dead[z], b.dead[z] + C);
+}
+__global__ __launch_bounds__(256) void col_flags4_batch_kernel(const PrepBatch b, int64_t C) {
+    const unsigned z = blockIdx.y;
+    col_flags4_body(b.H[z], b.W[z], b.R[z], C, b.dead[z], b.dead[z] + C);
+}
+__global__ __launch_bounds__(256) void zero_dead_cols_batch_kernel(const PrepBatch b, int64_t C) {
+    const unsigned z = blockIdx.y;
+    zero_dead_cols_body(b.W[z], b.R[z], C, b.dead[z]);
+}
+__global__ __launch_bounds__(256) void mask_h_batch_kernel(const PrepBatch b, int64_t C) {
+    const unsigned z = blockIdx.y;
+    mask_h_body(b.H[z], C, b.dead[z] + C);
+}
+__global__ __launch_bounds__(1024) void damp_batch_kernel(const PrepBatch b, int64_t C, float rel_damp) {
+    damp_body(b.H[blockIdx.y], C, rel_damp);
+}
+__global__ __launch_bounds__(256) void equil_batch_kernel(const PrepBatch b, int64_t n) {
+    const unsigned z = blockIdx.y;
+    equil_body(b.H[z], n, b.eq_s[z]);
+}
+__global__ __launch_bounds__(256) void reverse_copy_batch_kernel(const PrepBatch b, int64_t n) {
+    const unsigned z = blockIdx.y;
+    reverse_copy_body(b.A[z], b.H[z], n, b.eq_s[z]);
+}
+__global__ __launch_bounds__(256) void finish_u_batch_kernel(const PrepBatch b, int64_t n) {
+    const unsigned z = blockIdx.y;
+    finish_u_body(b.U[z], b.X[z], n, b.flag[z], b.eq_s[z]);
+}
+__global__ __launch_bounds__(256) void diag_potrf_inv_batch_kernel(const PrepBatch b, int64_t off, int64_t ld) {
+    const unsigned z = blockIdx.y;
+    diag_potrf_inv_body(b.A[z] + off, ld, b.X[z] + off, ld, b.flag[z]);
+}
+
 constexpr int LDQ = NB + 1;
 constexpr int TQ = 33;
 
@@ -557,16 +643,18 @@
 static int chol_inv_rec(float* A, float* X, float* Tmp, int* flag, int64_t n, int64_t lo, int64_t hi, size_t diag_lds,
                         hipStream_t st, P3Run& run);
 
+#define GQ_P3_NODE_LOCALS                                                                                             \
+    const int64_t n1 = (mid - lo) * NB, n2 = (hi - mid) * NB;                                                         \
+    const int64_t o21 = (mid * NB) * n + lo * NB, o11 = (lo * NB) * n + lo * NB, o22 = (mid * NB) * n + mid * NB;     \
+    unsigned* rm0 = run.rmax, *rm1 = run.rmax ? run.rmax + n / 2 : nullptr;                                           \
+    float* is0 = run.inv_scale, *is1 = run.inv_scale ? run.inv_scale + n / 2 : nullptr;                               \
+    const float* s0 = NP == 2 ? is0 : nullptr;                                                                        \
+    const float* s1 = NP == 2 ? is1 : nullptr;                                                                        \
+    int rc
 template <int NP>
-static int chol_node_p3(float* A, float* X, float* Tmp, int* flag, int64_t n, int64_t lo, int64_t mid, int64_t hi,
-                        size_t diag_lds, hipStream_t st, P3Run& run) {
-    const int64_t n1 = (mid - lo) * NB, n2 = (hi - mid) * NB;
-    const int64_t o21 = (mid * NB) * n + lo * NB, o11 = (lo * NB) * n + lo * NB, o22 = (mid * NB) * n + mid * NB;
-    unsigned* rm0 = run.rmax, *rm1 = run.rmax ? run.rmax + n / 2 : nullptr;
-    float* is0 = run.inv_scale, *is1 = run.inv_scale ? run.inv_scale + n / 2 : nullptr;
-    const float* s0 = NP == 2 ? is0 : nullptr;
-    const float* s1 = NP == 2 ? is1 : nullptr;
-    int rc;
+static int chol_node_p3_front(float* A, float* X, float* Tmp, int64_t n, int64_t lo, int64_t mid, int64_t hi, hipStream_t st,
+                              P3Run& run) {
+    GQ_P3_NODE_LOCALS;
     {
         ProfScope ps(PT_CHOL_GEMM, st);
         if ((rc = p3::launch_split<NP>(false, A + o21, n, n2, n1, 0, 0, run.img[0], rm0, is0, st))) return rc;
@@ -579,12 +667,27 @@
         const p3::Problem g3 = p3_problem<NP>(run, run.img[0], n1, run.img[1], n1, A + o21, n, 1, s0, s1);
         if ((rc = p3_gemm<NP>(run, g2, &g3, st))) return rc;
     }
-    if ((rc = chol_inv_rec(A, X, Tmp, flag, n, mid, hi, diag_lds, st, run))) return rc;
+    (void)o22; (void)n2;
+    return GQ_OK;
+}
+template <int NP>
+static int chol_node_p3_back(float* A, float* X, int64_t n, int64_t lo, int64_t mid, int64_t hi, hipStream_t st, P3Run& run) {
+    GQ_P3_NODE_LOCALS;
+    (void)o11; (void)rc;
     ProfScope ps(PT_TRTRI_GEMM, st);
     if ((rc = p3::launch_split<NP>(false, X + o22, n, n2, n2, 1, 0, run.img[0], rm0, is0, st))) return rc;
     if ((rc = p3::launch_split<NP>(true, A + o21, n, n1, n2, 0, 0, run.img[1], rm1, is1, st))) return rc;
     const p3::Problem g4 = p3_problem<NP>(run, run.img[0], n2, run.img[1], n2, X + o21, n, 2, s0, s1);
     return p3_gemm<NP>(run, g4, nullptr, st);
+}
+#undef GQ_P3_NODE_LOCALS
+template <int NP>
+static int chol_node_p3(float* A, float* X, float* Tmp, int* flag, int64_t n, int64_t lo, int64_t mid, int64_t hi,
+                        size_t diag_lds, hipStream_t st, P3Run& run) {
+    int rc;
+    if ((rc = chol_node_p3_front<NP>(A, X, Tmp, n, lo, mid, hi, st, run))) return rc;
+    if ((rc = chol_inv_rec(A, X, Tmp, flag, n, mid, hi, diag_lds, st, run))) return rc;
+    return chol_node_p3_back<NP>(A, X, n, lo, mid, hi, st, run);
 }
 
 static int chol_inv_rec(float* A, float* X, float* Tmp, int* flag, int64_t n, int64_t lo, int64_t hi, size_t diag_lds,
@@ -642,23 +745,24 @@
     return GQ_OK;
 }
 
-int h_prepare(float* H, float* W, int64_t R, int64_t C, float rel_damp, float* U, int* not_invertible,
-              uint8_t* col_flags_out, void* ws, size_t ws_bytes, hipStream_t st, bool obq_order) {
-    if (!H || !W || !U || !not_invertible) GQ_FAIL(GQ_E_NULL, "gq_h_prepare: null pointer");
-    if (R <= 0 || C <= 0 || C % NB) GQ_FAIL(GQ_E_BAD_SHAPE, "gq_h_prepare: R=%ld C=%ld (C %% 128 != 0)", (long)R, (long)C);
-    const size_t need = h_prepare_workspace_bytes(R, C);
-    if (!ws || ws_bytes < need) GQ_FAIL(GQ_E_WORKSPACE, "gq_h_prepare: workspace %zu < %zu bytes", ws_bytes, need);
-    const int64_t n = C, nblk = C / NB;
-    float* A = reinterpret_cast<float*>(((uintptr_t)ws + 255) & ~(uintptr_t)255);
-    float* X = A + (size_t)n * n;
-    uint8_t* dead = reinterpret_cast<uint8_t*>(X + (size_t)n * n);
-    uint8_t* zc = dead + n;
-    int rc;
-
+struct PrepArea {
+    float* A = nullptr;
+    float* X = nullptr;
+    uint8_t* dead = nullptr;
+    float* eq_s = nullptr;
     P3Run run;
     std::shared_ptr<const P3Plans> plans;
+};
+static int prep_carve(void* ws, size_t ws_bytes, int64_t C, PrepArea& ar, hipStream_t st, const char* who) {
+    const int64_t n = C, nblk = C / NB;
+    ar.A = reinterpret_cast<float*>(((uintptr_t)ws + 255) & ~(uintptr_t)255);
+    ar.X = ar.A + (size_t)n * n;
+    ar.dead = reinterpret_cast<uint8_t*>(ar.X + (size_t)n * n);
+    uint8_t* zc = ar.dead + n;
+    ar.eq_s = reinterpret_cast<float*>(((uintptr_t)(zc + n) + 255) & ~(uintptr_t)255);
+    P3Run& run = ar.run;
     if (p3_used(C)) {
-        plans = p3_plans_for(nblk);
+        ar.plans = p3_plans_for(nblk);
         unsigned char* p = reinterpret_cast<unsigned char*>(zc + n);
         p = reinterpret_cast<unsigned char*>(((uintptr_t)p + 255) & ~(uintptr_t)255) + (((size_t)n * 4 + 255) & ~(size_t)255);
         run.img[0] = p; p += (p3_image_bytes(C) + 255) & ~(size_t)255;
@@ -671,12 +775,28 @@
             p += 2 * (size_t)n * 4;
         }
         p = reinterpret_cast<unsigned char*>(((uintptr_t)p + 255) & ~(uintptr_t)255);
-        if (p + plans->words.size() * 4 > reinterpret_cast<unsigned char*>(ws) + ws_bytes)
-            GQ_FAIL(GQ_E_WORKSPACE, "gq_h_prepare: workspace too small for the image GEMMs");
-        GQ_HIP(hipMemcpyAsync(p, plans->words.data(), plans->words.size() * 4, hipMemcpyHostToDevice, st));
+        if (p + ar.plans->words.size() * 4 > reinterpret_cast<unsigned char*>(ws) + ws_bytes)
+            GQ_FAIL(GQ_E_WORKSPACE, "%s: workspace too small for the image GEMMs", who);
+        GQ_HIP(hipMemcpyAsync(p, ar.plans->words.data(), ar.plans->words.size() * 4, hipMemcpyHostToDevice, st));
         run.words_dev = reinterpret_cast<const uint32_t*>(p);
-        run.plans = plans.get();
-    }
+        run.plans = ar.plans.get();
+    }
+    return GQ_OK;
+}
+
+int h_prepare(float* H, float* W, int64_t R, int64_t C, float rel_damp, float* U, int* not_invertible,
+              uint8_t* col_flags_out, void* ws, size_t ws_bytes, hipStream_t st, bool obq_order) {
+    if (!H || !W || !U || !not_invertible) GQ_FAIL(GQ_E_NULL, "gq_h_prepare: null pointer");
+    if (R <= 0 || C <= 0 || C % NB) GQ_FAIL(GQ_E_BAD_SHAPE, "gq_h_prepare: R=%ld C=%ld (C %% 128 != 0)", (long)R, (long)C);
+    const size_t need = h_prepare_workspace_bytes(R, C);
+    if (!ws || ws_bytes < need) GQ_FAIL(GQ_E_WORKSPACE, "gq_h_prepare: workspace %zu < %zu bytes", ws_bytes, need);
+    const int64_t n = C, nblk = C / NB;
+    PrepArea ar;
+    int rc;
+    if ((rc = prep_carve(ws, ws_bytes, C, ar, st, "gq_h_prepare"))) return rc;
+    float* A = ar.A, *X = ar.X;
+    uint8_t* dead = ar.dead, *zc = ar.dead + n;
+    P3Run& run = ar.run;
     GQ_HIP(hipMemsetAsync(not_invertible, 0, sizeof(int), st));
     float* eq_s = nullptr;
     {
@@ -700,7 +820,7 @@
     GQ_LAUNCH_CHECK();
     const bool equil = !opt(OPT_chol_no_equil);
     if (equil) {
-        eq_s = reinterpret_cast<float*>(((uintptr_t)(zc + n) + 255) & ~(uintptr_t)255);
+        eq_s = ar.eq_s;
         hipLaunchKernelGGL(equil_kernel, dim3((unsigned)((n + 255) / 256)), dim3(256), 0, st, H, n, eq_s);
     }
     if (opt(OPT_chol_poison)) GQ_HIP(hipMemsetAsync(A, 0xff, 2 * (size_t)n * n * sizeof(float), st));
@@ -720,6 +840,174 @@
     if ((rc = chol_inv_rec(A, X, U, not_invertible, n, 0, nblk, diag_lds, st, run))) return rc;
     ProfScope ps(PT_PREP_ELEM, st);
     hipLaunchKernelGGL(finish_u_kernel, dim3((unsigned)n), dim3(256), 0, st, U, X, n, not_invertible, eq_s);
+    GQ_LAUNCH_CHECK();
+    return GQ_OK;
+}
+
+struct CholBatch {
+    int n = 0;
+    float* A[PREP_BATCH_MAX];
+    float* X[PREP_BATCH_MAX];
+    float* Tmp[PREP_BATCH_MAX];
+    int* flag[PREP_BATCH_MAX];
+    PrepArea area[PREP_BATCH_MAX];
+};
+static_assert(PREP_BATCH_MAX == G32_BATCH_MAX && PREP_BATCH_MAX == DIAG_BATCH_MAX, "one batch limit");
+
+size_t h_prepare_batch_workspace_bytes(int n, const int64_t* R, int64_t C) {
+    if (n <= 0 || n > PREP_BATCH_MAX || !R || C <= 0 || C % NB) return 0;
+    size_t total = 0;
+    for (int i = 0; i < n; ++i) total += (h_prepare_workspace_bytes(R[i], C) + 255) & ~(size_t)255;
+    return total;
+}
+
+template <bool TB, int MODE, bool LOW, int KR>
+static int chol_gemm_batch(bool big, const CholBatch& b, float* const* Cm, int64_t oc, float* const* Am, int64_t oa,
+                           float* const* Bm, int64_t ob, int64_t ld, int64_t M, int64_t N, int64_t K, hipStream_t st) {
+    if (big) {
+        for (int i = 0; i < b.n; ++i)
+            if (int rc = launch_gemm3b<TB, MODE, LOW, KR>(Cm[i] + oc, ld, Am[i] + oa, ld, Bm[i] + ob, ld, M, N, K, st)) return rc;
+        return GQ_OK;
+    }
+    G32Batch g;
+    for (int i = 0; i < PREP_BATCH_MAX; ++i) {
+        const int j = i < b.n ? i : 0;
+        g.C[i] = Cm[j] + oc; g.A[i] = Am[j] + oa; g.B[i] = Bm[j] + ob;
+    }
+    return launch_gemm32_batch<TB, MODE, LOW, KR>(b.n, g, ld, ld, ld, M, N, K, st);
+}
+
+static int chol_inv_rec_batch(CholBatch& b, int64_t n, int64_t lo, int64_t hi, size_t diag_lds, hipStream_t st) {
+    if (hi - lo == 1) {
+        ProfScope ps(PT_DIAG_POTRF, st);
+        const int64_t o = (lo * NB) * n + lo * NB;
+        if (diag_lds == DIAG5_LDS) {
+            DiagBatch d;
+            for (int i = 0; i < PREP_BATCH_MAX; ++i) {
+                const int j = i < b.n ? i : 0;
+                d.A[i] = b.A[j]; d.X[i] = b.X[j]; d.flag[i] = b.flag[j];
+            }
+            hipLaunchKernelGGL(diag_blk5_batch_kernel, dim3(1, (unsigned)b.n), dim3(320), diag_lds, st, d, o, n);
+        } else {
+            PrepBatch d = {};
+            for (int i = 0; i < b.n; ++i) { d.A[i] = b.A[i]; d.X[i] = b.X[i]; d.flag[i] = b.flag[i]; }
+            hipLaunchKernelGGL(diag_potrf_inv_batch_kernel, dim3(1, (unsigned)b.n), dim3(256), diag_lds, st, d, o, n);
+        }
+        GQ_LAUNCH_CHECK();
+        return GQ_OK;
+    }
+    const int64_t mid = (lo + hi) / 2;
+    int rc;
+    if ((rc = chol_inv_rec_batch(b, n, lo, mid, diag_lds, st))) return rc;
+    const int64_t n1 = (mid - lo) * NB, n2 = (hi - mid) * NB;
+    if (b.area[0].run.plans && p3_node(n1, n2)) {
+        const bool p3x = p3_planes() == 3;
+        for (int i = 0; i < b.n; ++i) {
+            P3Run& run = b.area[i].run;
+            if ((rc = p3x ? chol_node_p3_front<3>(b.A[i], b.X[i], b.Tmp[i], n, lo, mid, hi, st, run)
+                          : chol_node_p3_front<2>(b.A[i], b.X[i], b.Tmp[i], n, lo, mid, hi, st, run)))
+                return rc;
+        }
+        if ((rc = chol_inv_rec_batch(b, n, mid, hi, diag_lds, st))) return rc;
+        for (int i = 0; i < b.n; ++i) {
+            P3Run& run = b.area[i].run;
+            if ((rc = p3x ? chol_node_p3_back<3>(b.A[i], b.X[i], n, lo, mid, hi, st, run)
+                          : chol_node_p3_back<2>(b.A[i], b.X[i], n, lo, mid, hi, st, run)))
+                return rc;
+        }
+        return GQ_OK;
+    }
+    const int64_t o21 = (mid * NB) * n + lo * NB, o11 = (lo * NB) * n + lo * NB, o22 = (mid * NB) * n + mid * NB;
+    const int64_t min3b = opt(OPT_chol_fp32) ? (int64_t)1 << 40 : opt(OPT_chol_3b_min);
+    const bool big = n1 >= min3b && n2 >= min3b;
+    const bool pair = !big && !opt(OPT_chol_no_pair) && n % 4 == 0 && gemm32_uses_64_full(n2, n2, n1, true) &&
+                      gemm32_uses_64_full(n2, n1, n1, false);
+    {
+        ProfScope ps(PT_CHOL_GEMM, st);
+        if ((rc = chol_gemm_batch<true, 1, false, 1>(big, b, b.Tmp, o21, b.A, o21, b.X, o11, n, n2, n1, n1, st))) return rc;
+        if (pair) {
+            G32PairBatch pb;
+            for (int i = 0; i < PREP_BATCH_MAX; ++i) {
+                const int j = i < b.n ? i : 0;
+                pb.Ca[i] = b.A[j] + o22; pb.Aa[i] = b.Tmp[j] + o21;
+                pb.Cb[i] = b.A[j] + o21; pb.Ab[i] = b.Tmp[j] + o21; pb.Bb[i] = b.X[j] + o11;
+            }
+            if ((rc = launch_gemm32_pair_batch(b.n, pb, n2, n1, n2, n1, n1, n, st))) return rc;
+        } else if ((rc = chol_gemm_batch<true, 0, true, 0>(big, b, b.A, o22, b.Tmp, o21, b.Tmp, o21, n, n2, n2, n1, st))) return rc;
+    }
+    if ((rc = chol_inv_rec_batch(b, n, mid, hi, diag_lds, st))) return rc;
+    ProfScope ps(PT_TRTRI_GEMM, st);
+    if (!pair && (rc = chol_gemm_batch<false, 1, false, 2>(big, b, b.A, o21, b.Tmp, o21, b.X, o11, n, n2, n1, n1, st))) return rc;
+    return chol_gemm_batch<false, 2, false, 3>(big, b, b.X, o21, b.X, o22, b.A, o21, n, n2, n1, n2, st);
+}
+
+int h_prepare_batch(int n, float* const* H, float* const* W, const int64_t* R, int64_t C, float rel_damp, float* const* U,
+                    int* not_invertible, uint8_t* const* col_flags_out, void* ws, size_t ws_bytes, hipStream_t st) {
+    if (!H || !W || !R || !U || !not_invertible) GQ_FAIL(GQ_E_NULL, "gq_h_prepare_batch: null pointer");
+    if (n <= 0 || n > PREP_BATCH_MAX) GQ_FAIL(GQ_E_BAD_SHAPE, "gq_h_prepare_batch: n=%d not in 1..%d", n, PREP_BATCH_MAX);
+    if (C <= 0 || C % NB) GQ_FAIL(GQ_E_BAD_SHAPE, "gq_h_prepare_batch: C=%ld (C %% 128 != 0)", (long)C);
+    for (int i = 0; i < n; ++i) {
+        if (!H[i] || !W[i] || !U[i]) GQ_FAIL(GQ_E_NULL, "gq_h_prepare_batch: null pointer (problem %d)", i);
+        if (R[i] <= 0) GQ_FAIL(GQ_E_BAD_SHAPE, "gq_h_prepare_batch: R[%d]=%ld", i, (long)R[i]);
+        for (int j = 0; j < i; ++j)
+            if (H[i] == H[j] || U[i] == U[j])
+                GQ_FAIL(GQ_E_BAD_SHAPE, "gq_h_prepare_batch: problems %d and %d share %s", j, i, H[i] == H[j] ? "H" : "U");
+    }
+    const size_t need = h_prepare_batch_workspace_bytes(n, R, C);
+    if (!ws || ws_bytes < need) GQ_FAIL(GQ_E_WORKSPACE, "gq_h_prepare_batch: workspace %zu < %zu bytes", ws_bytes, need);
+    const int64_t nblk = C / NB;
+    const size_t nn = (size_t)C * (size_t)C;
+    CholBatch b;
+    b.n = n;
+    PrepBatch e = {};
+    int rc;
+    bool w16 = true;
+    const bool equil = !opt(OPT_chol_no_equil);
+    const bool poison = opt(OPT_chol_poison) != 0;
+    size_t at = 0;
+    for (int i = 0; i < n; ++i) {
+        const size_t bytes = (h_prepare_workspace_bytes(R[i], C) + 255) & ~(size_t)255;
+        if (at + bytes > ws_bytes) GQ_FAIL(GQ_E_WORKSPACE, "gq_h_prepare_batch: the area of problem %d ends at %zu > %zu bytes", i, at + bytes, ws_bytes);
+        if ((rc = prep_carve(reinterpret_cast<unsigned char*>(ws) + at, bytes, C, b.area[i], st, "gq_h_prepare_batch"))) return rc;
+        at += bytes;
+        b.A[i] = b.area[i].A; b.X[i] = b.area[i].X; b.Tmp[i] = U[i]; b.flag[i] = not_invertible + i;
+        e.H[i] = H[i]; e.W[i] = W[i]; e.R[i] = R[i]; e.dead[i] = b.area[i].dead; e.A[i] = b.A[i]; e.X[i] = b.X[i];
+        e.U[i] = U[i]; e.eq_s[i] = equil ? b.area[i].eq_s : nullptr; e.flag[i] = b.flag[i];
+        w16 = w16 && (uintptr_t)W[i] % 16 == 0;
+    }
+    GQ_HIP(hipMemsetAsync(not_invertible, 0, (size_t)n * sizeof(int), st));
+    const dim3 g64((unsigned)((C + 63) / 64), (unsigned)n), grow((unsigned)C, (unsigned)n);
+    {
+    ProfScope ps(PT_PREP_ELEM, st);
+    if (w16) hipLaunchKernelGGL(col_flags4_batch_kernel, g64, dim3(256), 0, st, e, C);
+    else hipLaunchKernelGGL(col_flags_batch_kernel, g64, dim3(256), 0, st, e, C);
+    GQ_LAUNCH_CHECK();
+    hipLaunchKernelGGL(zero_dead_cols_batch_kernel, g64, dim3(256), 0, st, e, C);
+    GQ_LAUNCH_CHECK();
+    if (col_flags_out)
+        for (int i = 0; i < n; ++i)
+            if (col_flags_out[i]) GQ_HIP(hipMemcpyAsync(col_flags_out[i], e.dead[i], 2 * (size_t)C, hipMemcpyDeviceToDevice, st));
+    hipLaunchKernelGGL(mask_h_batch_kernel, g64, dim3(256), 0, st, e, C);
+    hipLaunchKernelGGL(damp_batch_kernel, dim3(1, (unsigned)n), dim3(1024), 0, st, e, C, rel_damp);
+    GQ_LAUNCH_CHECK();
+    if (equil) hipLaunchKernelGGL(equil_batch_kernel, dim3((unsigned)((C + 255) / 256), (unsigned)n), dim3(256), 0, st, e, C);
+    if (poison)
+        for (int i = 0; i < n; ++i) GQ_HIP(hipMemsetAsync(b.A[i], 0xff, 2 * nn * sizeof(float), st));
+    hipLaunchKernelGGL(reverse_copy_batch_kernel, grow, dim3(256), 0, st, e, C);
+    GQ_LAUNCH_CHECK();
+    }
+    static std::atomic<bool> attr_set{false};
+    const bool use_ref = opt(OPT_diag_ref) != 0;
+    const size_t diag_lds = use_ref ? (2 * NB * LDP + NB) * sizeof(float) : DIAG5_LDS;
+    if (!attr_set) {
+        GQ_HIP(hipFuncSetAttribute((const void*)diag_potrf_inv_batch_kernel, hipFuncAttributeMaxDynamicSharedMemorySize,
+                                   (int)((2 * NB * LDP + NB) * sizeof(float))));
+        GQ_HIP(hipFuncSetAttribute((const void*)diag_blk5_batch_kernel, hipFuncAttributeMaxDynamicSharedMemorySize, (int)DIAG5_LDS));
+        attr_set = true;
+    }
+    if ((rc = chol_inv_rec_batch(b, C, 0, nblk, diag_lds, st))) return rc;
+    ProfScope ps(PT_PREP_ELEM, st);
+    hipLaunchKernelGGL(finish_u_batch_kernel, grow, dim3(256), 0, st, e, C);
     GQ_LAUNCH_CHECK();
     return GQ_OK;
 }
@@ -784,3 +1072,16 @@
 }
 
 }
+
+extern "C" {
+size_t gq_h_prepare_batch_workspace_bytes(int n, const int64_t* R_host, int64_t C) {
+    return gq::h_prepare_batch_workspace_bytes(n, R_host, C);
+}
+int gq_h_prepare_batch(int n, float* const* H_host, float* const* W_host, const int64_t* R_host, int64_t C, float rel_damp,
+                       float* const* U_host, int* not_invertible, uint8_t* const* col_flags_out_host, void* ws, size_t ws_bytes,
+                       void* stream) {
+    if (int rc = gq::options_ok()) return rc;
+    return gq::h_prepare_batch(n, H_host, W_host, R_host, C, rel_damp, U_host, not_invertible, col_flags_out_host, ws, ws_bytes,
+                               (hipStream_t)stream);
+}
+}
diff --git a/gptq-gguf-toolkit_amd/csrc/gq_diag5.hpp b/gptq-gguf-toolkit_amd/csrc/gq_diag5.hpp
--- a/gptq-gguf-toolkit_amd/csrc/gq_diag5.hpp
+++ b/gptq-gguf-toolkit_amd/csrc/gq_diag5.hpp
@@ -162,8 +162,8 @@
 
 #define D5_STAMP(k) (void)0
 
-__global__ __launch_bounds__(320) void diag_blk5_kernel(float* __restrict__ A, int64_t lda, float* __restrict__ Xout,
-                                                        int64_t ldx, int* __restrict__ flag_out) {
+__device__ __forceinline__ void diag_blk5_body(float* __restrict__ A, int64_t lda, float* __restrict__ Xout, int64_t ldx,
+                                               int* __restrict__ flag_out) {
     extern __shared__ __attribute__((aligned(16))) float smem[];
     float* S = smem;
     float* X = smem + NB * LDQ;
@@ -329,4 +329,19 @@
     if (wid == 0) D5_STAMP(11);
 }
 
-}
+__global__ __launch_bounds__(320) void diag_blk5_kernel(float* __restrict__ A, int64_t lda, float* __restrict__ Xout,
+                                                        int64_t ldx, int* __restrict__ flag_out) {
+    diag_blk5_body(A, lda, Xout, ldx, flag_out);
+}
+constexpr int DIAG_BATCH_MAX = 8;
+struct DiagBatch {
+    float* A[DIAG_BATCH_MAX];
+    float* X[DIAG_BATCH_MAX];
+    int* flag[DIAG_BATCH_MAX];
+};
+__global__ __launch_bounds__(320) void diag_blk5_batch_kernel(const DiagBatch b, int64_t off, int64_t ld) {
+    const unsigned z = blockIdx.y;
+    diag_blk5_body(b.A[z] + off, ld, b.X[z] + off, ld, b.flag[z]);
+}
+
+}
diff --git a/gptq-gguf-toolkit_amd/csrc/gq_gemm32.hpp b/gptq-gguf-toolkit_amd/csrc/gq_gemm32.hpp
--- a/gptq-gguf-toolkit_amd/csrc/gq_gemm32.hpp
+++ b/gptq-gguf-toolkit_amd/csrc/gq_gemm32.hpp
@@ -664,4 +664,96 @@
     return launch_gemm32_ts<TRANS_B, MODE, LOWER, KR, CHAIN, 128>(Cmat, ldc, A, lda, B, ldb, M, N, K, st);
 }
 
-}
+constexpr int G32_BATCH_MAX = 8;
+struct G32Batch {
+    float* C[G32_BATCH_MAX];
+    const float* A[G32_BATCH_MAX];
+    const float* B[G32_BATCH_MAX];
+};
+template <bool TRANS_B, int MODE, bool LOWER, int KR, int TS, bool FULL>
+__global__ __launch_bounds__(256, 2) void gemm32_batch_kernel(const G32Batch b, int64_t ldc, int64_t lda, int64_t ldb, int64_t M,
+                                                              int64_t N, int64_t K) {
+    const unsigned z = blockIdx.z;
+    gemm32_tile<TRANS_B, MODE, LOWER, KR, 0, TS, FULL, 4>(b.C[z], ldc, b.A[z], lda, b.B[z], ldb, M, N, K, blockIdx.x, blockIdx.y,
+                                                          gridDim.x, gridDim.y);
+}
+template <bool TRANS_B, int MODE, bool LOWER, int KR, int TS, bool FULL>
+inline int launch_gemm32_batch_full(int n, const G32Batch& b, int64_t ldc, int64_t lda, int64_t ldb, int64_t M, int64_t N,
+                                    int64_t K, hipStream_t st) {
+    static std::atomic<bool> attr_set{false};
+    if (!attr_set) {
+        GQ_HIP(hipFuncSetAttribute((const void*)gemm32_batch_kernel<TRANS_B, MODE, LOWER, KR, TS, FULL>,
+                                   hipFuncAttributeMaxDynamicSharedMemorySize, G32<TS>::LDS_BYTES));
+        attr_set = true;
+    }
+    dim3 grid((unsigned)((N + TS - 1) / TS), (unsigned)((M + TS - 1) / TS), (unsigned)n), block(256);
+    hipLaunchKernelGGL((gemm32_batch_kernel<TRANS_B, MODE, LOWER, KR, TS, FULL>), grid, block, G32<TS>::LDS_BYTES, st, b, ldc, lda,
+                       ldb, M, N, K);
+    GQ_LAUNCH_CHECK();
+    return GQ_OK;
+}
+template <bool TRANS_B, int MODE, bool LOWER, int KR>
+inline int launch_gemm32_batch(int n, const G32Batch& b, int64_t ldc, int64_t lda, int64_t ldb, int64_t M, int64_t N, int64_t K,
+                               hipStream_t st) {
+    if (M <= 0 || N <= 0 || K <= 0) return GQ_OK;
+    if (n <= 0 || n > G32_BATCH_MAX) GQ_FAIL(GQ_E_BAD_SHAPE, "gemm32 batch: n=%d not in 1..%d", n, G32_BATCH_MAX);
+    for (int i = 0; i < n; ++i)
+        if ((lda % 4) || (ldb % 4) || ((uintptr_t)b.A[i] % 16) || ((uintptr_t)b.B[i] % 16))
+            GQ_FAIL(GQ_E_BAD_SHAPE, "gemm32: A/B must be 16-byte aligned with ld %% 4 == 0");
+    const int64_t tiles128 = ((M + 127) / 128) * ((N + 127) / 128) / (LOWER ? 2 : 1);
+    const bool t64 = tiles128 < opt(OPT_gemm32_64_max);
+    const int64_t ts = t64 ? 64 : 128;
+    const bool full = M % ts == 0 && N % ts == 0 && K % TK == 0 && ldc % 4 == 0;
+    if (t64)
+        return full ? launch_gemm32_batch_full<TRANS_B, MODE, LOWER, KR, 64, true>(n, b, ldc, lda, ldb, M, N, K, st)
+                    : launch_gemm32_batch_full<TRANS_B, MODE, LOWER, KR, 64, false>(n, b, ldc, lda, ldb, M, N, K, st);
+    return full ? launch_gemm32_batch_full<TRANS_B, MODE, LOWER, KR, 128, true>(n, b, ldc, lda, ldb, M, N, K, st)
+                : launch_gemm32_batch_full<TRANS_B, MODE, LOWER, KR, 128, false>(n, b, ldc, lda, ldb, M, N, K, st);
+}
+
+struct G32PairBatch {
+    G32Pair shape;
+    float* Ca[G32_BATCH_MAX]; const float* Aa[G32_BATCH_MAX];
+    float* Cb[G32_BATCH_MAX]; const float* Ab[G32_BATCH_MAX]; const float* Bb[G32_BATCH_MAX];
+};
+template <int TS>
+__global__ __launch_bounds__(256, 2) void gemm32_pair_batch_kernel(const G32PairBatch pb) {
+    const G32Pair& p = pb.shape;
+    const unsigned z = blockIdx.y;
+    unsigned id = blockIdx.x;
+    if (id < p.n_a) {
+        unsigned by = (unsigned)((__fsqrt_rn(8.0f * (float)id + 1.0f) - 1.0f) * 0.5f);
+        while ((by + 1) * (by + 2) / 2 <= id) ++by;
+        while (by * (by + 1) / 2 > id) --by;
+        const unsigned bx = id - by * (by + 1) / 2;
+        gemm32_tile<true, 0, true, 0, 0, TS, true, 4>(pb.Ca[z], p.ld, pb.Aa[z], p.ld, pb.Aa[z], p.ld, p.Ma, p.Ma, p.Ka, bx, by, p.gxa,
+                                                      p.gxa);
+    } else {
+        id -= p.n_a;
+        gemm32_tile<false, 1, false, 2, 0, TS, true, 4>(pb.Cb[z], p.ld, pb.Ab[z], p.ld, pb.Bb[z], p.ld, p.Mb, p.Nb, p.Kb, id % p.gxb,
+                                                        id / p.gxb, p.gxb, p.gyb);
+    }
+}
+inline int launch_gemm32_pair_batch(int n, G32PairBatch& pb, int64_t Ma, int64_t Ka, int64_t Mb, int64_t Nb, int64_t Kb, int64_t ld,
+                                    hipStream_t st) {
+    if (n <= 0 || n > G32_BATCH_MAX) GQ_FAIL(GQ_E_BAD_SHAPE, "gemm32 pair batch: n=%d not in 1..%d", n, G32_BATCH_MAX);
+    static std::atomic<bool> attr_set{false};
+    if (!attr_set) {
+        GQ_HIP(hipFuncSetAttribute((const void*)gemm32_pair_batch_kernel<64>, hipFuncAttributeMaxDynamicSharedMemorySize,
+                                   G32<64>::LDS_BYTES));
+        attr_set = true;
+    }
+    G32Pair& p = pb.shape;
+    p.Ca = nullptr; p.Aa = nullptr; p.Cb = nullptr; p.Ab = nullptr; p.Bb = nullptr;
+    p.Ma = Ma; p.Ka = Ka; p.Mb = Mb; p.Nb = Nb; p.Kb = Kb;
+    p.ld = ld;
+    p.gxa = (unsigned)(Ma / 64);
+    p.n_a = p.gxa * (p.gxa + 1) / 2;
+    p.gxb = (unsigned)(Nb / 64);
+    p.gyb = (unsigned)(Mb / 64);
+    hipLaunchKernelGGL(gemm32_pair_batch_kernel<64>, dim3(p.n_a + p.gxb * p.gyb, (unsigned)n), dim3(256), G32<64>::LDS_BYTES, st, pb);
+    GQ_LAUNCH_CHECK();
+    return GQ_OK;
+}
+
+}
diff --git a/gptq-gguf-toolkit_amd/gptq.py b/gptq-gguf-toolkit_amd/gptq.py
--- a/gptq-gguf-toolkit_amd/gptq.py
+++ b/gptq-gguf-toolkit_amd/gptq.py
@@ -57,6 +57,7 @@
         self._zero_copy = True
         self._buf_b = 0
         self._U_cache = None
+        self._adopted = None
         self._last_U = None
 
     @torch.no_grad()
@@ -204,6 +205,7 @@
         self.shared_H_with = None
         self._has_followers = False
         self._U_cache = None
+        self._adopted = None
         self._last_U = None
         self._pending_mismatch = None
         self._flag = None
@@ -266,6 +268,9 @@
     def _prepare(self, defer_check: bool = False, own_U: bool = False) -> Tensor:
         leader = self.shared_H_with or self
         shared = self.shared_H_with is not None or self._has_followers
+        if self._adopted is not None and not own_U:
+            U, self._adopted = self._adopted, None
+            return U
         if shared and leader._U_cache is not None and not own_U:
             U, flag, cf = leader._U_cache
             self._last_cf = cf
@@ -284,6 +289,20 @@
         if not shared:
             self.H = H
         return U
+
+    def prepare_operands(self) -> Tuple[Tensor, Tensor]:
+        assert self.shared_H_with is None and not self.act_order, "only a leader without act_order factorises elsewhere"
+        return (self.H.clone() if self._has_followers else self.H), self.W
+
+    def adopt_factorisation(self, U: Tensor, flag: Tensor, cf: Tensor, H: Tensor) -> None:
+        assert self.shared_H_with is None and self._adopted is None
+        self._flag, self._last_cf = flag, cf
+        if self._has_followers:
+            if self._U_cache is None:
+                self._U_cache = (U, flag, cf)
+        else:
+            self.H = H
+        self._adopted = U
 
     @property
     def issue_non_invertible(self) -> bool:
@@ -330,17 +349,23 @@
 
     @staticmethod
     @torch.no_grad()
-    def compute_stacked(hs: Sequence["GPTQ"], q_type: GGMLQuantizationType):
+    def compute_stacked(hs: Sequence["GPTQ"], q_type: GGMLQuantizationType, Wf: Optional[Tensor] = None):
         assert len(hs) > 1 and all(h.stack_key(q_type) == hs[0].stack_key(q_type) is not None for h in hs)
         rows = [h.d_row for h in hs]
         ends = [sum(rows[:i + 1]) for i in range(len(rows))]
-        Wf = torch.empty((ends[-1], hs[0].d_col), device=hs[0].W_device, dtype=torch.float32)
+        have = Wf is not None
+        if not have:
+            Wf = GPTQ.stacked_buffer(hs)
+        assert Wf.shape == (ends[-1], hs[0].d_col) and Wf.dtype == torch.float32
         U = None
         for h, r1, n in zip(hs, ends, rows):
             if q_type == GGMLQuantizationType.Q3_K:
                 h.act_order = False
                 h.static_groups = False
-            h.make_working_copy(out=Wf[r1 - n:r1])
+            if not (have and h is hs[0]):
+                h.make_working_copy(out=Wf[r1 - n:r1])
+            else:
+                assert h._adopted is not None and h.W.data_ptr() == Wf.data_ptr()
             Uh = h._prepare(defer_check=True)
             assert U is None or Uh is U, "stacked handles must share one factorisation"
             U = Uh
@@ -351,6 +376,10 @@
         for h in hs:
             h.W = None
         return [tuple(t[r1 - n:r1] for t in res) for r1, n in zip(ends, rows)]
+
+    @staticmethod
+    def stacked_buffer(hs: Sequence["GPTQ"]) -> Tensor:
+        return torch.empty((sum(h.d_row for h in hs), hs[0].d_col), device=hs[0].W_device, dtype=torch.float32)
 
     def levels_key(self):
         key = self.stack_key(GGMLQuantizationType.Q4_K)
diff --git a/gptq-gguf-toolkit_amd/ops.py b/gptq-gguf-toolkit_amd/ops.py
--- a/gptq-gguf-toolkit_amd/ops.py
+++ b/gptq-gguf-toolkit_amd/ops.py
@@ -139,6 +139,30 @@
     check(fn(_ptr(H), _ptr(W), R, C, rel_damp, _ptr(U), _ptr(flag), _ptr(cf), _ptr(ws), ws.numel(), _stream(H)),
           "gq_obq_h_prepare" if obq_order else "gq_h_prepare")
     return (U, flag, cf) if want_flags else (U, flag)
+
+
+def h_prepare_batch(Hs, Ws, rel_damp: float, want_flags: bool = True):
+    n = len(Hs)
+    assert n == len(Ws) and 1 <= n <= _cabi.PREPARE_BATCH_MAX
+    _need_cuda(*Hs, *Ws)
+    C = Hs[0].shape[0]
+    for H, W in zip(Hs, Ws):
+        assert H.dtype == torch.float32 and W.dtype == torch.float32 and H.is_contiguous() and W.is_contiguous()
+        assert H.shape == (C, C) and W.dim() == 2 and W.shape[1] == C and H.device == Hs[0].device == W.device
+    dev = Hs[0].device
+    Us = [torch.empty_like(H) for H in Hs]
+    flags = torch.empty(n, dtype=torch.int32, device=dev)
+    cfs = [torch.empty(2 * C, dtype=torch.uint8, device=dev) if want_flags else None for _ in range(n)]
+    vp = ctypes.c_void_p
+    Rs = (ctypes.c_int64 * n)(*[W.shape[0] for W in Ws])
+    ws = _ws(int(lib().gq_h_prepare_batch_workspace_bytes(n, Rs, C)), dev)
+    Hp = (vp * n)(*[H.data_ptr() for H in Hs])
+    Wp = (vp * n)(*[W.data_ptr() for W in Ws])
+    Up = (vp * n)(*[U.data_ptr() for U in Us])
+    Fp = (vp * n)(*[cf.data_ptr() for cf in cfs]) if want_flags else None
+    check(lib().gq_h_prepare_batch(n, Hp, Wp, Rs, C, rel_damp, Up, _ptr(flags), Fp, _ptr(ws), ws.numel(), _stream(Hs[0])),
+          "gq_h_prepare_batch")
+    return [(Us[i], flags[i:i + 1], cfs[i]) for i in range(n)]
 
 
 def w_prepare(col_flags: torch.Tensor, W: torch.Tensor) -> torch.Tensor:
diff --git a/include/gptq_gguf_prepare_batch.h b/include/gptq_gguf_prepare_batch.h
--- /dev/null
+++ b/include/gptq_gguf_prepare_batch.h
@@ -0,0 +1,21 @@
+#ifndef GPTQ_GGUF_PREPARE_BATCH_H
+#define GPTQ_GGUF_PREPARE_BATCH_H
+
+#include "gptq_gguf.h"
+
+#ifdef __cplusplus
+extern "C" {
+#endif
+
+#define GQ_PREPARE_BATCH_MAX 8
+
+size_t gq_h_prepare_batch_workspace_bytes(int n, const int64_t* R_host, int64_t C);
+
+int gq_h_prepare_batch(int n, float* const* H_host, float* const* W_host, const int64_t* R_host, int64_t C, float rel_damp,
+                       float* const* U_host, int* not_invertible, uint8_t* const* col_flags_out_host, void* ws, size_t ws_bytes,
+                       void* stream);
+
+#ifdef __cplusplus
+}
+#endif
+#endif
diff --git a/profiles/prepare_batch_probe.py b/profiles/prepare_batch_probe.py
--- /dev/null
+++ b/profiles/prepare_batch_probe.py
@@ -0,0 +1,70 @@
+#!/usr/bin/env python3
+import json, os, statistics, sys
+import torch
+sys.path.insert(0, os.path.dirname(os.path.dirname(os.path.abspath(__file__))))
+from gptq_gguf_toolkit_amd import ops, _cabi
+
+N = int(os.environ.get("N", 9))
+ROWS = (4096, 4096, 14336)
+TAGS = ("diag_potrf_inv", "potrf_gemm32", "trtri_gemm32", "prepare_elementwise", "chol_image_split", "chol_image_gemm")
+
+
+def problems(C):
+    out = []
+    for i, R in enumerate(ROWS):
+        g = torch.Generator(device="cuda").manual_seed(100 * C + i)
+        T = 2 * C
+        X = (torch.randn(T, C, device="cuda", generator=g) * torch.exp(torch.randn(C, device="cuda", generator=g) * 0.5)).half()
+        H = torch.zeros(C, C, device="cuda")
+        ops.h_accumulate(H, X, 0.0, 2.0 / T)
+        out.append((H, torch.randn(R, C, device="cuda", generator=g) * 0.02))
+    return out
+
+
+def single(ps):
+    return [ops.h_prepare(H, W, 0.01, want_flags=True) for H, W in ps]
+
+
+def batch(ps):
+    return ops.h_prepare_batch([H for H, _ in ps], [W for _, W in ps], 0.01)
+
+
+def timed(fn, ps0):
+    ps = [(H.clone(), W.clone()) for H, W in ps0]
+    a, b = torch.cuda.Event(enable_timing=True), torch.cuda.Event(enable_timing=True)
+    torch.cuda.synchronize()
+    a.record()
+    out = fn(ps)
+    b.record()
+    torch.cuda.synchronize()
+    return a.elapsed_time(b), ps, out
+
+
+def launches(fn, ps0):
+    _cabi.prof_enable(None)
+    _cabi.prof_collect()
+    timed(fn, ps0)
+    got = _cabi.prof_collect()
+    _cabi.prof_enable([])
+    return {t: got[t][1] for t in TAGS if t in got}
+
+
+for C in [int(a) for a in sys.argv[1:]] or [4096, 8192]:
+    ps0 = problems(C)
+    _cabi.prof_enable([])
+    for fn in (single, batch):
+        timed(fn, ps0)
+    ts, tb = [], []
+    for _ in range(N):
+        t, p1, o1 = timed(single, ps0)
+        ts.append(t)
+        t, p2, o2 = timed(batch, ps0)
+        tb.append(t)
+    same = all(torch.equal(x, y) for (a, b) in zip(o1, o2) for x, y in zip(a, b)) and \
+        all(torch.equal(x, y) for (a, b) in zip(p1, p2) for x, y in zip(a, b))
+    print(json.dumps({"C": C, "rows": ROWS, "n": N, "three_single_ms": [round(t, 3) for t in ts],
+                      "one_batch_ms": [round(t, 3) for t in tb], "single_median": round(statistics.median(ts), 3),
+                      "batch_median": round(statistics.median(tb), 3), "bit_identical": same,
+                      "launches_single": launches(single, ps0), "launches_batch": launches(batch, ps0)}), flush=True)
+    del ps0, p1, p2, o1, o2
+    torch.cuda.empty_cache()
```

New measurement: 2468 Mparams/s. -1.5%, worse.
